# sThalham/PyraPose

Hardware: AMD Instinct MI355X
Metric: images/sec 640x480 fwd+bwd (train step: fwd + losses + bwd + clipnorm-Adam) (higher is better)
Workload: dtype bf16x3+f16c8

## Files before the change

### include/pyrapose_hip.h

```cpp
#ifndef PYRAPOSE_HIP_H
#define PYRAPOSE_HIP_H

#include <stddef.h>
#include <stdint.h>

#ifdef __cplusplus
extern "C" {
#endif

#define PP_OK 0
#define PP_ERR_ARG (-1)
#define PP_ERR_SHAPE (-2)
#define PP_ERR_ALIGN (-3)
#define PP_ERR_NOCTX (-4)
#define PP_ERR_UNSUPPORTED (-5)
#define PP_ERR_COMM (-6)

#define PP_MAX_SEG 5

typedef struct pp_ctx pp_ctx;

int pp_ctx_create(pp_ctx** out, int device, void* hip_stream);
void pp_ctx_destroy(pp_ctx* ctx);
int pp_ctx_set_stream(pp_ctx* ctx, void* hip_stream);
int pp_ctx_set_workspace(pp_ctx* ctx, void* device_buffer, size_t bytes);
int pp_row_block_list(pp_ctx* ctx, const float* x, int rows, int ld, int cols, unsigned char* flags, int* list);
int pp_row_block_list_planes(pp_ctx* ctx, const void* x_hi, const void* x_lo, int rows, int ld, int cols, unsigned char* flags, int* list);
int pp_row_block_list_planes_within(pp_ctx* ctx, const void* x_hi, const void* x_lo, int rows, int ld, int cols, const unsigned char* within,
                                    unsigned char* flags, int* list);
const char* pp_last_error_string(pp_ctx* ctx);
const char* pp_version(void);
int pp_device_info(pp_ctx* ctx, int* n_cu, char* name_host, int name_len);

typedef struct {
  int n_img;
  int n_seg;
  int h[PP_MAX_SEG];
  int w[PP_MAX_SEG];
} pp_rowspace;

typedef struct {
  pp_rowspace in;
  pp_rowspace out;
  int cin, cout;
  int kh, kw, stride;
  int pad_t, pad_l;
  int ld_x, ld_y, ld_w;
} pp_conv_desc;

int pp_conv2d_nhwc_fwd(pp_ctx* ctx, const pp_conv_desc* d, const float* x, const float* w,
                       const float* bias, const float* residual, int ld_res, int relu, float* y);

int pp_conv2d_nhwc_bwd_data(pp_ctx* ctx, const pp_conv_desc* d, const float* dy, const float* w,
                            const float* addend, int ld_add, const float* relu_src, int ld_rs, float* dx);

int pp_conv2d_nhwc_bwd_weight(pp_ctx* ctx, const pp_conv_desc* d, const float* x, const float* dy,
                              float* dw, float* dbias);

int pp_conv_split_weights_bf16x3(pp_ctx* ctx, const pp_conv_desc* d, const float* w, void* fwd_hi, void* fwd_lo,
                                 void* dgrad_hi, void* dgrad_lo);
typedef struct pp_split_job {
  const float* w;
  void* fwd_hi; void* fwd_lo; void* dg_hi; void* dg_lo;
  int taps, cin, cout, ld_w;
  int tile_begin, reserved;
} pp_split_job;
int pp_conv_split_weights_bf16x3_batch(pp_ctx* ctx, int n_jobs, const pp_split_job* jobs_dev, int total_tiles);
int pp_positive_row_blocks(pp_ctx* ctx, const pp_rowspace* rs, int A, int stride, const float* y_true, unsigned char* flags);
int pp_row_block_dilate(pp_ctx* ctx, const pp_conv_desc* d, const unsigned char* in_flags, unsigned char* out_flags);
int pp_split_planes_bf16x3(pp_ctx* ctx, size_t n, const float* src, void* hi, void* lo);
int pp_ctx_set_planes_format(pp_ctx* ctx, int fmt);
int pp_convert_planes(pp_ctx* ctx, size_t n, const void* src_hi, const void* src_lo, int src_fmt, void* dst_hi, void* dst_lo, int dst_fmt,
                      const float* scale2_dev, int scale_index, const void* relu_src_hi);
int pp_grad_scale_from_counts(pp_ctx* ctx, const int* counts_dev, int n_counts, float* scale2_dev);
int pp_grad_scale_from_counts_adj(pp_ctx* ctx, const int* counts_dev, int n_counts, float* scale2_dev, int log2_adjust);
int pp_split_planes_scaled_bf16x3(pp_ctx* ctx, size_t n, const float* src, void* hi, void* lo, const float* scale_dev);
int pp_ctx_set_grad_scale(pp_ctx* ctx, const float* scale2_dev);

typedef struct pp_conv_opts {
  void* capture_hi;
  void* capture_lo;
  const void* add_hi;
  const void* add_lo;
  const void* mask_hi;
  unsigned char* skip_flags;
  int* skip_list;
  const unsigned char* out_flags;
  int* out_list;
  int lazy_out;
  int lazy_in;
} pp_conv_opts;
#ifdef __cplusplus
static_assert(sizeof(pp_conv_opts) == 9 * sizeof(void*) + 2 * sizeof(int), "pp_conv_opts: pointers, then ints, no padding");
#else
_Static_assert(sizeof(pp_conv_opts) == 9 * sizeof(void*) + 2 * sizeof(int), "pp_conv_opts: pointers, then ints, no padding");
#endif

int pp_conv2d_nhwc_fwd_bf16x3(pp_ctx* ctx, const pp_conv_desc* d, const float* x, const void* x_hi, const void* x_lo,
                              const void* w_fwd_hi, const void* w_fwd_lo, const float* bias, const float* residual,
                              int ld_res, int relu, float* y, void* y_hi, void* y_lo, const pp_conv_opts* opts);
int pp_conv2d_nhwc_bwd_data_bf16x3(pp_ctx* ctx, const pp_conv_desc* d, const float* dy, const void* dy_hi,
                                   const void* dy_lo, const void* w_dgrad_hi, const void* w_dgrad_lo,
                                   const float* addend, int ld_add, const float* relu_src, int ld_rs, float* dx,
                                   void* dx_hi, void* dx_lo, const pp_conv_opts* opts);
int pp_conv2d_nhwc_bwd_data_s2_bf16x3(pp_ctx* ctx, const pp_conv_desc* d, const float* dy, const void* dy_hi,
                                      const void* dy_lo, const void* w_dgrad_hi, const void* w_dgrad_lo,
                                      const float* addend, int ld_add, const float* relu_src, int ld_rs, float* dx,
                                      void* dx_hi, void* dx_lo, const pp_conv_opts* opts);
int pp_conv_s2_merged(void);
int pp_conv2d_nhwc_bwd_weight_bf16x3(pp_ctx* ctx, const pp_conv_desc* d, const float* x, const float* dy,
                                     const void* x_hi, const void* x_lo, const void* dy_hi, const void* dy_lo,
                                     float* dw, float* dbias, const pp_conv_opts* opts);

#define PP_PLAN_FWD 0
#define PP_PLAN_BWD_DATA 1
#define PP_PLAN_BWD_WEIGHT 2
#define PP_PLAN_BWD_DATA_S2 3
#define PP_PLAN_PLANES_IN 1u
#define PP_PLAN_PLANES_OUT 2u
#define PP_PLAN_F32_OUT 4u
#define PP_PLAN_CAPTURE 8u
#define PP_PLAN_LIST 16u
#define PP_PLAN_LAZY_IN 32u
#define PP_PLAN_LAZY_OUT 64u
int pp_conv_plan_text(const pp_conv_desc* d, int pass, unsigned forms, int planes_fmt, int n_cu, size_t ws_bytes, char* buf,
                      int buf_bytes);

typedef struct pp_comm pp_comm;
int pp_comm_available(void);
int pp_comm_unique_id(pp_ctx* ctx, void* id128);
int pp_comm_init(pp_ctx* ctx, int world, int rank, const void* id128, pp_comm** out);
int pp_comm_destroy(pp_comm* comm);
int pp_allreduce_bucket(pp_ctx* ctx, pp_comm* comm, float* buf, size_t count);
int pp_allreduce_counts(pp_ctx* ctx, pp_comm* comm, int* counts, int n);

int pp_maxpool3x3s2_fwd(pp_ctx* ctx, int n_img, int h, int w, int c, const float* x, int oh, int ow, float* y);
int pp_upsample_nearest_add_fwd(pp_ctx* ctx, int n_img, int sh, int sw, int th, int tw, int c,
                                const float* src, const float* other, float* out);
int pp_upsample_nearest_add_bwd(pp_ctx* ctx, int n_img, int sh, int sw, int th, int tw, int c,
                                const float* dtarget, const float* base, float* dsrc);
int pp_add_n(pp_ctx* ctx, size_t n, const float* a, const float* b, const float* c, float* out);
int pp_relu_fwd(pp_ctx* ctx, size_t n, const float* x, float* y);
typedef struct pp_tview {
  const float* f32;
  const void* hi;
  const void* lo;
} pp_tview;
int pp_add_n_v(pp_ctx* ctx, size_t n, const pp_tview* a, const pp_tview* b, const pp_tview* c, const pp_tview* out);
int pp_relu_fwd_v(pp_ctx* ctx, size_t n, const pp_tview* x, const pp_tview* y);
int pp_upsample_nearest_add_fwd_v(pp_ctx* ctx, int n_img, int sh, int sw, int th, int tw, int c, const pp_tview* src,
                                  const pp_tview* other, const pp_tview* out);
int pp_upsample_nearest_add_bwd_v(pp_ctx* ctx, int n_img, int sh, int sw, int th, int tw, int c, const pp_tview* dtarget,
                                  const pp_tview* base, const pp_tview* dsrc);
int pp_merge_planes_bf16x3(pp_ctx* ctx, size_t n, const void* hi, const void* lo, float* dst);
int pp_planes_stats(pp_ctx* ctx, const void* hi, const void* lo, long long rows, int ld, int cols, const unsigned char* within,
                    unsigned long long* stats5_dev);
int pp_pack_rgb_to_4(pp_ctx* ctx, size_t n_pixels, const float* x3, float* x4);
int pp_preprocess_caffe_u8(pp_ctx* ctx, int n_img, int H, int W, const int* sizes_hw_host, const unsigned char* images_u8,
                           float* x4);
int pp_warp_affine_u8(pp_ctx* ctx, int n_img, int H, int W, int channels, const double* mats_host, int interpolation, int border,
                      int cval, const unsigned char* src, unsigned char* dst);
int pp_resize_scale(int rows, int cols, int min_side, int max_side, double* scale);
int pp_resize_linear_u8(pp_ctx* ctx, int n_img, int SH, int SW, int channels, double scale, int DH, int DW, const unsigned char* src,
                        unsigned char* dst);
enum { PP_PHOTO_NONE = 0, PP_PHOTO_LUT = 1, PP_PHOTO_GRAY = 2, PP_PHOTO_HUESAT = 3, PP_PHOTO_BLEND = 4, PP_PHOTO_CONV = 5, PP_PHOTO_MEDIAN = 6,
       PP_PHOTO_BILATERAL = 7 };
typedef struct pp_photo_op {
  int kind;
  int k;
  int off0, off1;
  float f0, f1;
} pp_photo_op;
size_t pp_photo_workspace_bytes(int n_img, int H, int W);
int pp_photo_augment_u8(pp_ctx* ctx, int n_img, int H, int W, int channels, const int* op_offsets_host, const pp_photo_op* ops_host,
                        const unsigned char* pool_host, size_t pool_bytes, const unsigned char* pool_dev, const unsigned char* src,
                        unsigned char* dst, void* workspace, size_t workspace_bytes);
int pp_pack_rgb_to_4_padded(pp_ctx* ctx, int n_img, int H, int W, int Hp, int Wp, int pad, const float* x3, float* x4p);
int pp_preprocess_caffe_u8_padded(pp_ctx* ctx, int n_img, int H, int W, int Hp, int Wp, int pad, const int* sizes_hw_host,
                                  const unsigned char* images_u8, float* x4p);
int pp_stem7x7s2_fwd_bf16x3(pp_ctx* ctx, int n_img, int H, int W, int Hp, int Wp, const float* x4p, const void* w_hi,
                            const void* w_lo, int cout, const float* bias, int relu, float* y, int ld_y);

int pp_export_head(pp_ctx* ctx, const pp_rowspace* rs, int n_anchor, int n_val, const float* src, int ld,
                   int apply_sigmoid, float* out);

int pp_count_positives(pp_ctx* ctx, size_t rows_box, const float* y_box, size_t rows_cls, int c_cls,
                       const float* y_cls, size_t rows_mask, int c_mask, const float* y_mask, int* counts);
int pp_sigmoid_focal_fwd_bwd(pp_ctx* ctx, const pp_rowspace* rs, int n_anchor, int n_class,
                             const float* logits, int ld, const float* y_true, float alpha, float gamma,
                             const int* count, float loss_weight, float* loss_sum, float* dlogits);
int pp_orth_smoothl1_fwd_bwd(pp_ctx* ctx, const pp_rowspace* rs, int n_anchor, const float* pred, int ld,
                             const float* y_true, float weight, float sigma, const int* count,
                             float loss_weight, float* loss_sum, float* dpred);

typedef struct {
  long long offset;
  long long count;
  int ld;
  int trainable;
  long long scale_off;
  float l2;
} pp_param_desc;

typedef struct pp_optimizer pp_optimizer;
int pp_optimizer_create(pp_ctx* ctx, pp_optimizer** out, const pp_param_desc* descs_host, int n_desc,
                        long long total);
void pp_optimizer_destroy(pp_optimizer* opt);
int pp_grad_global_norm(pp_ctx* ctx, pp_optimizer* opt, const float* w_master, const float* g_eff,
                        const float* scales, float* gnorm_sq, float* l2_loss);
int pp_adam_step_clipnorm(pp_ctx* ctx, pp_optimizer* opt, float* w_master, float* w_eff, const float* g_eff,
                          const float* scales, float* m, float* v, const float* gnorm_sq, float lr,
                          float beta1, float beta2, float eps, float clipnorm, long long step);

int pp_generate_base_anchors_host(int base_size, const float* ratios_host, int n_ratios,
                                  const float* scales_host, int n_scales, double* out_host);
int pp_anchors_shift_f64(pp_ctx* ctx, int n_levels, const int* feat_h_host, const int* feat_w_host,
                         const int* strides_host, int n_anchor, const double* base_anchors_host,
                         double* anchors_out);
int pp_anchors_shift_f32(pp_ctx* ctx, int n_levels, const int* feat_h_host, const int* feat_w_host,
                         const int* strides_host, int n_anchor, const double* base_anchors_host,
                         float* anchors_out);
int pp_compute_overlap_f64(pp_ctx* ctx, int n, const double* boxes, int k, const double* query, double* overlaps);
int pp_compute_gt_annotations(pp_ctx* ctx, int n, const double* anchors, int k, const double* gt_boxes,
                              double negative_overlap, double positive_overlap, int* argmax, signed char* state);

int pp_anchor_targets(pp_ctx* ctx, int n_anchor_total, const double* anchors, int batch,
                      const int* gt_offset_host, const double* gt_boxes, const int* gt_labels,
                      const double* gt_box3d, const int* gt_mask_ids, const unsigned char* id_masks,
                      int mask_h, int mask_w, const int* mask_hw_host, const int* image_hw_host, int num_classes,
                      double negative_overlap, double positive_overlap, int out_mh, int out_mw,
                      float* regression, float* labels, float* mask);
int pp_project_box3d_host(const double* pose7_host, const double* box8x3_host, const double* cam4_host,
                          double* out16_host);
int pp_pil_nearest_index_host(int n_in, int n_out, int* out_host);

int pp_box3d_decode(pp_ctx* ctx, int batch, int n, const float* anchors, const float* regression, float* boxes3d);
int pp_score_threshold_compact(pp_ctx* ctx, int batch, int n, int n_class, const float* scores, float thr,
                               int cap, int* idx_out, int* counts);
size_t pp_filter_workspace_bytes(int n, int n_class, int max_det);
int pp_filter_detections(pp_ctx* ctx, int n, int n_class, const float* boxes, const float* boxes3d,
                         const float* scores, float score_thr, float iou_thr, int max_det, void* workspace,
                         float* out_boxes, float* out_boxes3d, float* out_scores, int* out_labels);
int pp_filter_detections_batch(pp_ctx* ctx, int n_img, int n, int n_class, const float* boxes, const float* boxes3d,
                               const float* scores, float score_thr, float iou_thr, int max_det, void* workspace,
                               float* out_boxes, float* out_boxes3d, float* out_scores, int* out_labels);

size_t pp_pose_error_workspace_bytes(int n_pose, int n_pts);
int pp_pose_add_f64(pp_ctx* ctx, int n_pose, int n_pts, const double* pts, const double* R_est, const double* t_est,
                    const double* R_gt, const double* t_gt, void* workspace, double* out);
int pp_pose_adi_f64(pp_ctx* ctx, int n_pose, int n_pts, const double* pts, const double* R_est, const double* t_est,
                    const double* R_gt, const double* t_gt, void* workspace, double* out);

size_t pp_render_workspace_bytes(int n_pose, int n_vert, int n_tri, int width, int height);
int pp_render_depth_f32(pp_ctx* ctx, int n_pose, int n_vert, const double* verts, int n_tri, const int* faces, const double* R,
                        const double* t, const double* K4, int width, int height, double clip_near, double clip_far, void* workspace,
                        size_t workspace_bytes, float* depth);
size_t pp_render_rgbd_workspace_bytes(int n_pose, int n_vert, int n_tri, int width, int height);
int pp_render_rgbd(pp_ctx* ctx, int n_pose, int n_vert, const double* verts, const double* colors, const double* normals, int n_tri,
                   const int* faces, const double* R, const double* t, const double* K4, int width, int height, double clip_near,
                   double clip_far, int shading, double ambient_weight, const double* light_cam_pos, const double* bg_color,
                   void* workspace, size_t workspace_bytes, float* depth, int* tri_id, float* rgb_f32, unsigned char* rgb_u8);
size_t pp_render_rgbd_tex_workspace_bytes(int n_pose, int n_vert, int n_tri, int width, int height, int tex_w, int tex_h);
int pp_render_rgbd_tex(pp_ctx* ctx, int n_pose, int n_vert, const double* verts, const double* uv, const unsigned char* tex, int tex_w,
                       int tex_h, int filter, int wrap, const double* normals, int n_tri, const int* faces, const double* R,
                       const double* t, const double* K4, int width, int height, double clip_near, double clip_far, int shading,
                       double ambient_weight, const double* light_cam_pos, const double* bg_color, void* workspace,
                       size_t workspace_bytes, float* depth, int* tri_id, float* rgb_f32, unsigned char* rgb_u8);
size_t pp_vsd_workspace_bytes(int n, int width, int height);
int pp_vsd_f64(pp_ctx* ctx, int n, int width, int height, const float* depth_test, long long test_stride, const float* depth_est,
               const float* depth_gt, const double* K4, double delta, double tau, int cost_type, void* workspace, double* e,
               long long* inter, long long* uni);
size_t pp_vsd_multi_workspace_bytes(int n, int width, int height, int n_tau);
int pp_vsd_multi_f64(pp_ctx* ctx, int n, int width, int height, const float* depth_test, long long test_stride,
                     const float* depth_est, const float* depth_gt, const double* K4, double delta, int n_tau, const double* taus,
                     int cost_type, int visib_mode, void* workspace, double* e, long long* inter, long long* uni,
                     long long* visib_gt, long long* px_gt);
size_t pp_scene_gt_workspace_bytes(int n_inst, int canvas_w, int canvas_h);
// ... 163 lines not shown
```

### pyrapose_amd/_lib.py

```python
import ctypes as C
import os

_HERE = os.path.dirname(os.path.abspath(__file__))
LIB_PATH = os.path.join(_HERE, os.environ.get("PP_LIB") or "libpyrapose_hip.so")

PP_MAX_SEG = 5


class RowSpace(C.Structure):
    _fields_ = [("n_img", C.c_int), ("n_seg", C.c_int), ("h", C.c_int * PP_MAX_SEG), ("w", C.c_int * PP_MAX_SEG)]

    @classmethod
    def make(cls, n_img, shapes):
        rs = cls()
        rs.n_img = int(n_img)
        rs.n_seg = len(shapes)
        for i, (h, w) in enumerate(shapes):
            rs.h[i] = int(h)
            rs.w[i] = int(w)
        return rs

    def rows(self):
        return sum(self.n_img * self.h[i] * self.w[i] for i in range(self.n_seg))

    def shapes(self):
        return [(self.h[i], self.w[i]) for i in range(self.n_seg)]


class ConvDesc(C.Structure):
    _fields_ = [("in_", RowSpace), ("out", RowSpace), ("cin", C.c_int), ("cout", C.c_int), ("kh", C.c_int),
                ("kw", C.c_int), ("stride", C.c_int), ("pad_t", C.c_int), ("pad_l", C.c_int), ("ld_x", C.c_int),
                ("ld_y", C.c_int), ("ld_w", C.c_int)]


class ParamDesc(C.Structure):
    _fields_ = [("offset", C.c_longlong), ("count", C.c_longlong), ("ld", C.c_int), ("trainable", C.c_int),
                ("scale_off", C.c_longlong), ("l2", C.c_float)]


class SplitJob(C.Structure):
    _fields_ = [("w", C.c_void_p), ("fwd_hi", C.c_void_p), ("fwd_lo", C.c_void_p), ("dg_hi", C.c_void_p), ("dg_lo", C.c_void_p),
                ("taps", C.c_int), ("cin", C.c_int), ("cout", C.c_int), ("ld_w", C.c_int), ("tile_begin", C.c_int), ("reserved", C.c_int)]


class TView(C.Structure):
    _fields_ = [("f32", C.c_void_p), ("hi", C.c_void_p), ("lo", C.c_void_p)]


class ConvOpts(C.Structure):
    _fields_ = [("capture_hi", C.c_void_p), ("capture_lo", C.c_void_p), ("add_hi", C.c_void_p), ("add_lo", C.c_void_p),
                ("mask_hi", C.c_void_p), ("skip_flags", C.c_void_p), ("skip_list", C.c_void_p), ("out_flags", C.c_void_p),
                ("out_list", C.c_void_p), ("lazy_out", C.c_int), ("lazy_in", C.c_int)]


def _load():
    if not os.path.exists(LIB_PATH):
        raise ImportError(
            "pyrapose_amd: %s not found. Build it with `python -c 'import __graft_entry__ as g; g.build()'` "
            "or `make -C pyrapose_amd/csrc`. There is no CPU fallback." % LIB_PATH)
    try:
        return C.CDLL(LIB_PATH)
    except OSError as e:
        raise ImportError("pyrapose_amd: cannot load %s: %s" % (LIB_PATH, e))


lib = _load()
if hasattr(lib, "pp_ctx_set_split_capture"):
    raise ImportError("pyrapose_amd: %s predates pp_conv_opts (it still exports pp_ctx_set_split_capture): rebuild it" % LIB_PATH)

_p = C.c_void_p
_i = C.c_int
_f = C.c_float
_d = C.c_double
_ll = C.c_longlong
_sz = C.c_size_t

_SIGS = {
    "pp_ctx_create": (_i, [C.POINTER(_p), _i, _p]),
    "pp_ctx_destroy": (None, [_p]),
    "pp_ctx_set_stream": (_i, [_p, _p]),
    "pp_last_error_string": (C.c_char_p, [_p]),
    "pp_version": (C.c_char_p, []),
    "pp_device_info": (_i, [_p, C.POINTER(_i), C.c_char_p, _i]),
    "pp_conv2d_nhwc_fwd": (_i, [_p, C.POINTER(ConvDesc), _p, _p, _p, _p, _i, _i, _p]),
    "pp_conv2d_nhwc_bwd_data": (_i, [_p, C.POINTER(ConvDesc), _p, _p, _p, _i, _p, _i, _p]),
    "pp_conv2d_nhwc_bwd_weight": (_i, [_p, C.POINTER(ConvDesc), _p, _p, _p, _p]),
    "pp_conv_split_weights_bf16x3": (_i, [_p, C.POINTER(ConvDesc), _p, _p, _p, _p, _p]),
    "pp_split_planes_bf16x3": (_i, [_p, _sz, _p, _p, _p]),
    "pp_ctx_set_planes_format": (_i, [_p, _i]),
    "pp_convert_planes": (_i, [_p, _sz, _p, _p, _i, _p, _p, _i, _p, _i, _p]),
    "pp_split_planes_scaled_bf16x3": (_i, [_p, _sz, _p, _p, _p, _p]),
    "pp_grad_scale_from_counts": (_i, [_p, _p, _i, _p]),
    "pp_grad_scale_from_counts_adj": (_i, [_p, _p, _i, _p, _i]),
    "pp_ctx_set_grad_scale": (_i, [_p, _p]),
    "pp_planes_stats": (_i, [_p, _p, _p, _ll, _i, _i, _p, _p]),
    "pp_comm_available": (_i, []),
    "pp_comm_unique_id": (_i, [_p, _p]),
    "pp_comm_init": (_i, [_p, _i, _i, _p, C.POINTER(_p)]),
    "pp_comm_destroy": (_i, [_p]),
    "pp_allreduce_bucket": (_i, [_p, _p, _p, C.c_size_t]),
    "pp_allreduce_counts": (_i, [_p, _p, _p, _i]),
    "pp_ctx_set_workspace": (_i, [_p, _p, C.c_size_t]),
    "pp_row_block_list": (_i, [_p, _p, _i, _i, _i, _p, _p]),
    "pp_positive_row_blocks": (_i, [_p, _p, _i, _i, _p, _p]),
    "pp_row_block_dilate": (_i, [_p, _p, _p, _p]),
    "pp_row_block_list_planes": (_i, [_p, _p, _p, _i, _i, _i, _p, _p]),
    "pp_row_block_list_planes_within": (_i, [_p, _p, _p, _i, _i, _i, _p, _p, _p]),
    "pp_add_n_v": (_i, [_p, _sz, C.POINTER(TView), C.POINTER(TView), C.POINTER(TView), C.POINTER(TView)]),
    "pp_relu_fwd_v": (_i, [_p, _sz, C.POINTER(TView), C.POINTER(TView)]),
    "pp_upsample_nearest_add_fwd_v": (_i, [_p, _i, _i, _i, _i, _i, _i, C.POINTER(TView), C.POINTER(TView), C.POINTER(TView)]),
    "pp_upsample_nearest_add_bwd_v": (_i, [_p, _i, _i, _i, _i, _i, _i, C.POINTER(TView), C.POINTER(TView), C.POINTER(TView)]),
    "pp_merge_planes_bf16x3": (_i, [_p, _sz, _p, _p, _p]),
    "pp_warp_affine_u8": (_i, [_p, _i, _i, _i, _i, C.POINTER(_d), _i, _i, _i, _p, _p]),
    "pp_photo_workspace_bytes": (_sz, [_i, _i, _i]),
    "pp_photo_augment_u8": (_i, [_p, _i, _i, _i, _i, _p, _p, _p, _sz, _p, _p, _p, _p, _sz]),
    "pp_resize_scale": (_i, [_i, _i, _i, _i, C.POINTER(_d)]),
    "pp_resize_linear_u8": (_i, [_p, _i, _i, _i, _i, _d, _i, _i, _p, _p]),
    "pp_conv_split_weights_bf16x3_batch": (_i, [_p, _i, _p, _i]),
    "pp_conv2d_nhwc_fwd_bf16x3": (_i, [_p, C.POINTER(ConvDesc), _p, _p, _p, _p, _p, _p, _p, _i, _i, _p, _p, _p, C.POINTER(ConvOpts)]),
    "pp_conv2d_nhwc_bwd_data_bf16x3": (_i, [_p, C.POINTER(ConvDesc), _p, _p, _p, _p, _p, _p, _i, _p, _i, _p, _p, _p, C.POINTER(ConvOpts)]),
    "pp_conv2d_nhwc_bwd_data_s2_bf16x3": (_i, [_p, C.POINTER(ConvDesc), _p, _p, _p, _p, _p, _p, _i, _p, _i, _p, _p, _p, C.POINTER(ConvOpts)]),
    "pp_conv_s2_merged": (_i, []),
    "pp_conv2d_nhwc_bwd_weight_bf16x3": (_i, [_p, C.POINTER(ConvDesc), _p, _p, _p, _p, _p, _p, _p, _p, C.POINTER(ConvOpts)]),
    "pp_conv_plan_text": (_i, [C.POINTER(ConvDesc), _i, C.c_uint, _i, _i, _sz, C.c_char_p, _i]),
    "pp_maxpool3x3s2_fwd": (_i, [_p, _i, _i, _i, _i, _p, _i, _i, _p]),
    "pp_upsample_nearest_add_fwd": (_i, [_p, _i, _i, _i, _i, _i, _i, _p, _p, _p]),
    "pp_upsample_nearest_add_bwd": (_i, [_p, _i, _i, _i, _i, _i, _i, _p, _p, _p]),
    "pp_add_n": (_i, [_p, _sz, _p, _p, _p, _p]),
    "pp_relu_fwd": (_i, [_p, C.c_size_t, _p, _p]),
    "pp_preprocess_caffe_u8": (_i, [_p, _i, _i, _i, C.POINTER(C.c_int), _p, _p]),
    "pp_preprocess_caffe_u8_padded": (_i, [_p, _i, _i, _i, _i, _i, _i, C.POINTER(C.c_int), _p, _p]),
    "pp_pack_rgb_to_4_padded": (_i, [_p, _i, _i, _i, _i, _i, _i, _p, _p]),
    "pp_stem7x7s2_fwd_bf16x3": (_i, [_p, _i, _i, _i, _i, _i, _p, _p, _p, _i, _p, _i, _p, _i]),
    "pp_pack_rgb_to_4": (_i, [_p, _sz, _p, _p]),
    "pp_export_head": (_i, [_p, C.POINTER(RowSpace), _i, _i, _p, _i, _i, _p]),
    "pp_count_positives": (_i, [_p, _sz, _p, _sz, _i, _p, _sz, _i, _p, _p]),
    "pp_sigmoid_focal_fwd_bwd": (_i, [_p, C.POINTER(RowSpace), _i, _i, _p, _i, _p, _f, _f, _p, _f, _p, _p]),
    "pp_orth_smoothl1_fwd_bwd": (_i, [_p, C.POINTER(RowSpace), _i, _p, _i, _p, _f, _f, _p, _f, _p, _p]),
    "pp_optimizer_create": (_i, [_p, C.POINTER(_p), C.POINTER(ParamDesc), _i, _ll]),
    "pp_optimizer_destroy": (None, [_p]),
    "pp_grad_global_norm": (_i, [_p, _p, _p, _p, _p, _p, _p]),
    "pp_adam_step_clipnorm": (_i, [_p, _p, _p, _p, _p, _p, _p, _p, _p, _f, _f, _f, _f, _f, _ll]),
    "pp_generate_base_anchors_host": (_i, [_i, C.POINTER(_f), _i, C.POINTER(_f), _i, C.POINTER(_d)]),
    "pp_anchors_shift_f64": (_i, [_p, _i, C.POINTER(_i), C.POINTER(_i), C.POINTER(_i), _i, C.POINTER(_d), _p]),
    "pp_anchors_shift_f32": (_i, [_p, _i, C.POINTER(_i), C.POINTER(_i), C.POINTER(_i), _i, C.POINTER(_d), _p]),
    "pp_compute_overlap_f64": (_i, [_p, _i, _p, _i, _p, _p]),
    "pp_compute_gt_annotations": (_i, [_p, _i, _p, _i, _p, _d, _d, _p, _p]),
    "pp_anchor_targets": (_i, [_p, _i, _p, _i, C.POINTER(_i), _p, _p, _p, _p, _p, _i, _i, C.POINTER(_i), C.POINTER(_i), _i, _d, _d,
                               _i, _i, _p, _p, _p]),
    "pp_project_box3d_host": (_i, [C.POINTER(_d), C.POINTER(_d), C.POINTER(_d), C.POINTER(_d)]),
    "pp_pil_nearest_index_host": (_i, [_i, _i, C.POINTER(_i)]),
    "pp_box3d_decode": (_i, [_p, _i, _i, _p, _p, _p]),
    "pp_score_threshold_compact": (_i, [_p, _i, _i, _i, _p, _f, _i, _p, _p]),
    "pp_filter_workspace_bytes": (_sz, [_i, _i, _i]),
    "pp_pose_error_workspace_bytes": (_sz, [_i, _i]),
    "pp_filter_detections": (_i, [_p, _i, _i, _p, _p, _p, _f, _f, _i, _p, _p, _p, _p, _p]),
    "pp_pose_add_f64": (_i, [_p, _i, _i, _p, _p, _p, _p, _p, _p, _p]),
    "pp_pose_adi_f64": (_i, [_p, _i, _i, _p, _p, _p, _p, _p, _p, _p]),
    "pp_filter_detections_batch": (_i, [_p, _i, _i, _i, _p, _p, _p, _f, _f, _i, _p, _p, _p, _p, _p]),
    "pp_render_workspace_bytes": (_sz, [_i, _i, _i, _i, _i]),
    "pp_render_depth_f32": (_i, [_p, _i, _i, _p, _i, _p, _p, _p, _p, _i, _i, _d, _d, _p, _sz, _p]),
    "pp_render_rgbd_workspace_bytes": (_sz, [_i, _i, _i, _i, _i]),
    "pp_render_rgbd": (_i, [_p, _i, _i, _p, _p, _p, _i, _p, _p, _p, _p, _i, _i, _d, _d, _i, _d, C.POINTER(_d), C.POINTER(_d), _p, _sz,
                            _p, _p, _p, _p]),
    "pp_render_rgbd_tex_workspace_bytes": (_sz, [_i, _i, _i, _i, _i, _i, _i]),
    "pp_render_rgbd_tex": (_i, [_p, _i, _i, _p, _p, _p, _i, _i, _i, _i, _p, _i, _p, _p, _p, _p, _i, _i, _d, _d, _i, _d, C.POINTER(_d),
                                C.POINTER(_d), _p, _sz, _p, _p, _p, _p]),
    "pp_scene_compose_u8": (_i, [_p, _i, _i, C.POINTER(_i), _p, _i, _i, _p, _p, _p, C.POINTER(C.c_ubyte), _i, _p]),
    "pp_vsd_workspace_bytes": (_sz, [_i, _i, _i]),
    "pp_vsd_f64": (_i, [_p, _i, _i, _i, _p, _ll, _p, _p, _p, _d, _d, _i, _p, _p, _p, _p]),
    "pp_vsd_multi_workspace_bytes": (_sz, [_i, _i, _i, _i]),
    "pp_vsd_multi_f64": (_i, [_p, _i, _i, _i, _p, _ll, _p, _p, _p, _d, _i, C.POINTER(_d), _i, _i, _p, _p, _p, _p, _p, _p]),
    "pp_scene_gt_workspace_bytes": (_sz, [_i, _i, _i]),
    "pp_scene_gt_info": (_i, [_p, _i, _i, C.POINTER(_i), _p, _i, _i, _i, _i, _i, _i, _p, _p, _p, _ll, _d, _p, _sz, _p, _p, _p, _p, _p,
                              _p, _p]),
    "pp_pose_reproj_f64": (_i, [_p, _i, _i, _p, _p, _p, _p, _p, _p, _p, _p]),
    "pp_pose_sym_workspace_bytes": (_sz, [_i, _i, _i]),
    "pp_pose_mssd_f64": (_i, [_p, _i, _i, _i, _p, _p, _p, _p, _p, _p, _p, _p, _p, _p]),
    "pp_pose_mspd_f64": (_i, [_p, _i, _i, _i, _p, _p, _p, _p, _p, _p, _p, _p, _p, _p, _p]),
    "pp_pnp_ransac_workspace_bytes": (_sz, [_i, _i]),
    "pp_pnp_ransac_f64": (_i, [_p, _i, _p, _i, _p, _p, _p, _i, _d, C.c_ulonglong, _i, _p, _p, _p, _p, _p, _p]),
    "pp_cloud_from_depth_workspace_bytes": (_sz, [_i, _i]),
    "pp_cloud_from_depth_f64": (_i, [_p, _i, _i, _p, _p, _i, _i, _p, _p, _d, _d, _d, _d, _d, _i, _p, _p, _p]),
    "pp_voxel_workspace_bytes": (_sz, [_i]),
    "pp_voxel_keys_f64": (_i, [_p, _i, _p, _d, _p, _p]),
    "pp_voxel_means_f64": (_i, [_p, _i, _p, _p, _p, _i, _p, _p, _p]),
    "pp_estimate_normals_workspace_bytes": (_sz, [_i, _i]),
    "pp_estimate_normals_f64": (_i, [_p, _i, _p, _d, _i, _p, _p, _p]),
    "pp_icp_workspace_bytes": (_sz, [_i, _i]),
    "pp_icp_f64": (_i, [_p, _i, _p, _p, _i, _p, _p, _p, _p, _d, _i, _d, _d, _i, _p, _sz, _p, _p, _p, _p, _p, _p, _p]),
    "pp_vote_stats_workspace_bytes": (_sz, [_i, _i]),
    "pp_vote_stats_f64": (_i, [_p, _i, _p, _i, _p, _i, _p, _p, _i, _d, _p, _p, _p, _p, _p, _p, _p]),
    "pp_pnp_refine_weighted_workspace_bytes": (_sz, [_i, _i]),
    "pp_pnp_refine_weighted_f64": (_i, [_p, _i, _p, _i, _p, _p, _p, _p, _p, _p, _i, _d, _d, _d, _p, _p, _p, _p, _p, _p, _p, _p, _p]),
    "pp_vote_cluster_workspace_bytes": (_sz, [_i, _i, _i, _i]),
    "pp_vote_cluster": (_i, [_p, _i, _i, _i, _i, _p, _p, _p, _p, _d, _i, _i, _i, _p, _p, _p, _p, _p, _p, _p]),
    "pp_pts_diameter_workspace_bytes": (_sz, [_i]),
    "pp_pts_diameter_f64": (_i, [_p, _i, _p, _p, _sz, _p, _p]),
    "pp_farthest_points_workspace_bytes": (_sz, [_i]),
    "pp_farthest_points_f64": (_i, [_p, _i, _i, _p, C.POINTER(_i), _p, _i, _i, _p, _p, _p, _sz, _p]),
    "pp_sym_hausdorff_workspace_bytes": (_sz, [_i, _i]),
    "pp_sym_hausdorff_f64": (_i, [_p, _i, _p, _i, _p, _i, _p, _p, _p, _sz, _p, _p]),
    "pp_det_match": (_i, [_p, _i, _i, _i, _i, _p, _p, _p, _p, _p, _p, C.POINTER(_i), _p, _i, C.POINTER(_d), _i, _p, _p, _p]),
    "pp_det_pr_curve": (_i, [_p, _i, _i, _i, _ll, _p, _p, _p, _p, _p, _p, _p, _p, _p]),
    "pp_det_ap": (_i, [_p, _i, _i, _i, _p, _p, _p, _p, _i, _p, _p]),
    "pp_mask_confusion": (_i, [_p, _i, _i, _i, _p, _p, _i, C.POINTER(_d), _p]),
    "pp_mask_pack": (_i, [_p, _i, _i, _i, _p, _p, _p, _p]),
    "pp_mask_iou_pairs": (_i, [_p, _i, _i, _i, _i, _i, _p, _p, _p, _p, _p, _p, _p, C.POINTER(_i), _p, _p, _p]),
    "pp_det_match_iou": (_i, [_p, _i, _i, _i, _i, _p, _p, _p, _p, _p, C.POINTER(_i), _p, _i, C.POINTER(_d), _i, _p, _p, _p]),
    "pp_mask_rle_workspace_bytes": (_sz, [_i]),
    "pp_mask_rle": (_i, [_p, _i, _i, _i, _i, _p, _p, _sz, _ll, _p, C.POINTER(_i), _p]),
    "pp_mask_from_rle": (_i, [_p, _i, _i, _i, _i, C.POINTER(_i), C.POINTER(_i), _p, _p, _p]),
    "pp_depth_normals_workspace_bytes": (_sz, [_i, _i, _i]),
    "pp_depth_normals_f64": (_i, [_p, _i, _i, _i, _p, _p, C.POINTER(_d), _i, _p, _sz, _p, _p, _p, _p]),
    "pp_depth_augment_workspace_bytes": (_sz, [_i, _i, _i]),
    "pp_depth_augment": (_i, [_p, _i, _i, _i, _p, _p, _p, C.POINTER(_d), _p, _p, _sz, _p, _p, _p, _p, _p]),
    "pp_depth_inpaint_workspace_bytes": (_sz, [_i, _i, _i]),
    "pp_depth_inpaint": (_i, [_p, _i, _i, _i, _p, _p, _i, _i, _i, _p, _sz, _p, _p, _p, _p]),
    "pp_draw_overlay_u8": (_i, [_p, _i, _i, _i, _p, _p, _p, _p, _i, _p, _p, _i, _i]),
}

EXPORTS = sorted(_SIGS)

MISSING = []
for _name, (_res, _args) in _SIGS.items():
    try:
        _fn = getattr(lib, _name)
    except AttributeError:
        if not os.environ.get("PP_LIB"):
            raise
        MISSING.append(_name)
        continue
    _fn.restype = _res
    _fn.argtypes = _args


def check(rc, ctx=None, what=""):
    if rc == 0:
        return
    msg = ""
    if ctx is not None:
        s = lib.pp_last_error_string(ctx)
        msg = s.decode("utf-8", "replace") if s else ""
    if rc < 0:
        raise ValueError("%s failed (%d): %s" % (what or "pyrapose_hip", rc, msg))
    raise RuntimeError("%s failed (hipError %d): %s" % (what or "pyrapose_hip", rc, msg))
```

### pyrapose_amd/csrc/conv3.h

```cpp
#pragma once
#include "conv_common.h"

struct Igemm3Args {
  const void *ahi, *alo, *whi, *wlo;
  int w_rows, w_ld8;
  void *ohi, *olo;
  void *chi, *clo;
  const unsigned char* flags;
  float* ws;
};

void PP_API(pp3_launch_igemm)(hipStream_t st, IgemmParams& p, const Igemm3Args& a, const PpIgemmPlan& pl);
void PP_API(pp3_launch_igemm_s2)(hipStream_t st, IgemmParams& p, const Igemm3Args& a, const DgradS2Route& r);
void PP_API(pp3_launch_igemm_rowlist)(hipStream_t st, IgemmParams& p, const Igemm3Args& a, const PpIgemmPlan& pl, const unsigned char* dy_flags,
                                      unsigned char* out_flags, int* out_list, bool fill);
void PP_API(pp3_launch_class_fill)(hipStream_t st, const IgemmParams& p, unsigned blocks, const float* addend, const float* mask, float* out, void* ohi,
                                   void* olo);
void PP_API(pp3_launch_rl_dilate)(hipStream_t st, const IgemmParams& p, const unsigned char* in_flags, unsigned char* out_flags, int n_blocks);

void PP_API(pp3_launch_igemm4x)(hipStream_t st, const IgemmParams& p, const Igemm3Args& a, const PpIgemmPlan& pl);

void PP_API(pp3_launch_wgrad)(hipStream_t st, const Wgrad3Params& p, const PpWgradPlan& pl, const float* x, const float* dy, const void* xhi,
                              const void* xlo, const void* dhi, const void* dlo, float* dw, float* dbias, const int* list, float* ctx_ws);

void PP_API(pp3_split_capture_pass)(hipStream_t st, const IgemmParams& p, void* chi, void* clo);
void PP_API(pp3_launch_row_block_compact)(hipStream_t st, const unsigned char* flags, int n_blocks, int* list);
```

### pyrapose_amd/csrc/conv3.hip

```cpp
#include "conv3_unit.h"
#include "conv3.h"
#include "conv4.h"

namespace {

static PpIgemmFacts igemm3_facts(const pp_ctx* ctx, const IgemmParams& p, const Igemm3Args& a) {
  return igemm_facts(p, a.w_rows, a.w_ld8, a.ahi != nullptr, p.src != nullptr, a.ohi != nullptr, p.out != nullptr, a.chi != nullptr,
                     a.flags != nullptr, ctx->n_cu, ctx->ws != nullptr, (long long)ctx->ws_bytes);
}

static void dispatch3(pp_ctx* ctx, IgemmParams& p, const Igemm3Args& a) {
  const PpIgemmFacts f = igemm3_facts(ctx, p, a);
  const PpIgemmPlan pl = pp_plan_igemm(f);
  pp_plan_debug(f, pl);
  PP_API(pp3_launch_igemm)(ctx->stream, p, a, pl);
}

static void dispatch3m(pp_ctx* ctx, IgemmParams& p, const Igemm3Args& a, const DgradS2Route& r) {
  pp_plan_debug(r.f, r.pl, r.g);
  PP_API(pp3_launch_igemm_s2)(ctx->stream, p, a, r);
}

static void dispatch3_rowlist(pp_ctx* ctx, IgemmParams& p, const Igemm3Args& a, int tm, const unsigned char* dy_flags, unsigned char* out_flags,
                              int* out_list, bool fill) {
  PpIgemmFacts f = igemm3_facts(ctx, p, a);
  f.listed = true;
  f.listed_tm = tm;
  const PpIgemmPlan pl = pp_plan_igemm(f);
  PP_API(pp3_launch_igemm_rowlist)(ctx->stream, p, a, pl, dy_flags, out_flags, out_list, fill);
}

static int bwd_data_impl(pp_ctx* ctx, const char* who, bool merged, const pp_conv_desc* d, const float* dy, const void* dy_hi, const void* dy_lo,
                         const void* w_hi, const void* w_lo, const float* addend, int ld_add, const float* relu_src, int ld_rs, float* dx,
                         void* dx_hi, void* dx_lo, const pp_conv_opts* opts) {
  PP_REQUIRE_CTX(ctx);
  int rc = pp_conv_opts_take(ctx, opts,
                             merged ? (PP_OPT_ADD | PP_OPT_MASK)
                                    : (PP_OPT_CAPTURE | PP_OPT_ADD | PP_OPT_MASK | PP_OPT_SKIP | PP_OPT_LAZY_OUT | PP_OPT_LAZY_IN),
                             who);
  if (rc) return rc;
  void *const chi = opts->capture_hi, *const clo = opts->capture_lo;
  unsigned char* const skip_flags = opts->skip_flags;
  const bool skip_scratch_ok = skip_flags != nullptr && opts->skip_list != nullptr;
  const void *const ep_ah = opts->add_hi, *const ep_al = opts->add_lo, *const ep_mh = opts->mask_hi;
  rc = check_desc(ctx, d, who);
  PP_CHECK_ARG(ctx, !(ep_ah && addend) && !(ep_mh && relu_src), PP_ERR_ARG,
               "%s: addend / relu_src given both as f32 and as planes", who);
  PP_CHECK_ARG(ctx, (!ep_ah || (ld_add >= d->cin && ld_add % 4 == 0)) && (!ep_mh || (ld_rs >= d->cin && ld_rs % 4 == 0)), PP_ERR_SHAPE,
               "%s: addend / relu_src planes", who);
  if (rc) return rc;
  PP_CHECK_ARG(ctx, !chi || (dy && !dy_hi && pp_is_packed(chi, clo)), PP_ERR_ARG, "%s: split capture needs the f32 operand", who);
  PP_CHECK_ARG(ctx, (dy || (dy_hi && dy_lo)) && w_hi && w_lo && (dx || (dx_hi && dx_lo)), PP_ERR_ARG, "%s: null tensor", who);
  PP_CHECK_ARG(ctx, (dy_hi == nullptr) == (dy_lo == nullptr) && d->ld_y % 8 == 0, PP_ERR_ARG, "%s: planes / ld_y", who);
  PP_CHECK_ARG(ctx, pp_is_packed(dy_hi, dy_lo) && pp_is_packed(dx_hi, dx_lo), PP_ERR_ALIGN,
               "%s: planes must be packed (lo = hi + 16 bytes, 16-byte aligned)", who);
  PP_CHECK_ARG(ctx, (!dx_hi || (d->cin % 8 == 0 && d->ld_x % 8 == 0)) && (!ep_ah || ld_add % 8 == 0) && (!ep_mh || ld_rs % 8 == 0), PP_ERR_SHAPE,
               "%s: planes need channel counts and leading dimensions %% 8 == 0", who);
  const int cred = (d->cout + 31) / 32 * 32;
  PP_CHECK_ARG(ctx, d->cin % 16 == 0 && d->ld_y >= cred && d->ld_y % 4 == 0, PP_ERR_SHAPE,
               "%s: dy needs ld_y >= %d (cout rounded up to 32, zero padded)", who, cred);
  PP_CHECK_ARG(ctx, (!dy || pp_is_aligned16(dy)) && pp_is_aligned16(w_hi) && pp_is_aligned16(w_lo) && (!dx || pp_is_aligned16(dx)), PP_ERR_ALIGN,
               "%s: tensors must be 16-byte aligned", who);
  PP_CHECK_ARG(ctx, (!addend || (ld_add >= d->cin && ld_add % 4 == 0 && pp_is_aligned16(addend))) &&
                        (!relu_src || (ld_rs >= d->cin && ld_rs % 4 == 0 && pp_is_aligned16(relu_src))),
               PP_ERR_SHAPE, "%s: addend / relu_src", who);
  IgemmParams p;
  memset(&p, 0, sizeof(p));
  p.src = dy; p.out = dx; p.bias = nullptr; p.addend = addend; p.mask_src = relu_src;
  p.add_hi = ep_ah; p.add_lo = ep_al; p.mask_hi = ep_mh;
  igemm_geometry_bwd_data(ctx, d, p);
  p.ld_add = ld_add; p.ld_mask = ld_rs;
  p.relu = 0;
  PP_CHECK_ARG(ctx, (dx_hi == nullptr) == (dx_lo == nullptr) && (!dx_hi || (d->ld_x % 4 == 0 && pp_is_aligned16(dx_hi) && pp_is_aligned16(dx_lo))),
               PP_ERR_ARG, "%s: output planes", who);
  const Igemm3Args a = {dy_hi, dy_lo, w_hi, w_lo, d->cin, cred / 8, dx_hi, dx_lo, chi, clo, skip_flags, ctx->ws};
  if (merged) {
    DgradS2Route s2;
    dgrad_s2_route(d, p, igemm3_facts(ctx, p, a), &s2);
    PP_CHECK_ARG(ctx, s2.ok, PP_ERR_ARG,
                 "%s: needs stride 2, one level, operands all float32 or all planes, and classes the branch-free loop can run "
                 "(pp_conv2d_nhwc_bwd_data_bf16x3 takes every other call)", who);
    IgemmParams q = s2.cls[0];
    dispatch3m(ctx, q, a, s2);
    PP_CHECK_LAUNCH(ctx, who);
    return PP_OK;
  }
  DgradRoute route;
  dgrad_route(d, p, igemm3_facts(ctx, p, a), skip_scratch_ok, &route);
  PP_CHECK_ARG(ctx, !opts->lazy_in || route.listed, PP_ERR_ARG,
               "%s: dy was declared lazy (unwritten outside its flagged blocks) but the listed-block launch "
               "does not apply to this call", who);
  const int nb = (p.M + 31) / 32;
  if (skip_scratch_ok && !route.listed) PP_HIP(ctx, hipMemsetAsync(skip_flags + nb, 1, (size_t)nb, ctx->stream));
  const Igemm3Args ac = {dy_hi, dy_lo, w_hi, w_lo, d->cin, cred / 8, dx_hi, dx_lo, nullptr, nullptr, nullptr, ctx->ws};
  if (route.classes && chi) PP_API(pp3_split_capture_pass)(ctx->stream, p, chi, clo);
  dgrad_launches(
      route, p,
      [&](IgemmParams& q, bool is_class, bool listed) {
        if (listed) dispatch3_rowlist(ctx, q, a, route.listed_tm, skip_flags, skip_flags + nb, opts->skip_list + nb + 1, !opts->lazy_out);
        else dispatch3(ctx, q, is_class ? ac : a);
      },
      [&](IgemmParams& q) {
        PP_API(pp3_launch_class_fill)(ctx->stream, q, pp_finish_blocks(q.M, q.Nout, pp_cus(ctx->n_cu)), addend, relu_src, dx, dx_hi, dx_lo);
      });
  PP_CHECK_LAUNCH(ctx, who);
  return PP_OK;
}

}

extern "C" {

int PP_API(pp_conv2d_nhwc_fwd_bf16x3)(pp_ctx* ctx, const pp_conv_desc* d, const float* x, const void* x_hi, const void* x_lo,
                                         const void* w_hi, const void* w_lo, const float* bias, const float* residual, int ld_res,
                                         int relu, float* y, void* y_hi, void* y_lo, const pp_conv_opts* opts) {
  PP_REQUIRE_CTX(ctx);
  int rc = pp_conv_opts_take(ctx, opts, PP_OPT_CAPTURE | PP_OPT_ADD | PP_OPT_OUT, "pp_conv2d_nhwc_fwd_bf16x3");
  if (rc) return rc;
  void *const chi = opts->capture_hi, *const clo = opts->capture_lo;
  const void *const ep_ah = opts->add_hi, *const ep_al = opts->add_lo;
  rc = check_desc(ctx, d, "pp_conv2d_nhwc_fwd_bf16x3");
  PP_CHECK_ARG(ctx, !(ep_ah && residual), PP_ERR_ARG, "pp_conv2d_nhwc_fwd_bf16x3: residual given both as f32 and as planes");
  PP_CHECK_ARG(ctx, !ep_ah || (ld_res % 4 == 0 && ld_res >= ((d->cout + 3) & ~3)), PP_ERR_SHAPE, "pp_conv2d_nhwc_fwd_bf16x3: residual planes");
  if (rc) return rc;
  PP_CHECK_ARG(ctx, !chi || (x && !x_hi && pp_is_packed(chi, clo)), PP_ERR_ARG, "pp_conv2d_nhwc_fwd_bf16x3: split capture needs the f32 operand");
  PP_CHECK_ARG(ctx, (x || (x_hi && x_lo)) && w_hi && w_lo && (y || (y_hi && y_lo)), PP_ERR_ARG, "pp_conv2d_nhwc_fwd_bf16x3: null tensor");
  PP_CHECK_ARG(ctx, (x_hi == nullptr) == (x_lo == nullptr), PP_ERR_ARG, "pp_conv2d_nhwc_fwd_bf16x3: x_hi and x_lo go together");
  PP_CHECK_ARG(ctx, d->cin % 32 == 0 && d->ld_x % 8 == 0, PP_ERR_SHAPE, "pp_conv2d_nhwc_fwd_bf16x3: cin %d must be a multiple of 32, ld_x of 8", d->cin);
  PP_CHECK_ARG(ctx, pp_is_packed(x_hi, x_lo) && pp_is_packed(y_hi, y_lo), PP_ERR_ALIGN,
               "pp_conv2d_nhwc_fwd_bf16x3: planes must be packed (lo = hi + 16 bytes, 16-byte aligned)");
  PP_CHECK_ARG(ctx, !y_hi || (d->cout % 8 == 0 && d->ld_y % 8 == 0), PP_ERR_SHAPE, "pp_conv2d_nhwc_fwd_bf16x3: output planes need cout, ld_y %% 8 == 0");
  PP_CHECK_ARG(ctx, !ep_ah || (ld_res % 8 == 0 && d->cout % 8 == 0), PP_ERR_SHAPE, "pp_conv2d_nhwc_fwd_bf16x3: residual planes need cout, ld_res %% 8 == 0");
  PP_CHECK_ARG(ctx, (!x || pp_is_aligned16(x)) && pp_is_aligned16(w_hi) && pp_is_aligned16(w_lo) && (!y || pp_is_aligned16(y)), PP_ERR_ALIGN,
               "pp_conv2d_nhwc_fwd_bf16x3: tensors must be 16-byte aligned");
  PP_CHECK_ARG(ctx, !residual || (ld_res % 4 == 0 && ld_res >= ((d->cout + 3) & ~3) && pp_is_aligned16(residual)), PP_ERR_SHAPE,
               "pp_conv2d_nhwc_fwd_bf16x3: residual");
  PP_CHECK_ARG(ctx, !bias || pp_is_aligned16(bias), PP_ERR_ALIGN, "pp_conv2d_nhwc_fwd_bf16x3: bias alignment");
  IgemmParams p;
  memset(&p, 0, sizeof(p));
  p.src = x; p.out = y; p.bias = bias; p.addend = residual; p.mask_src = nullptr;
  p.add_hi = ep_ah; p.add_lo = ep_al;
  igemm_geometry_fwd(ctx, d, p);
  p.ld_add = ld_res; p.ld_mask = 0;
  p.relu = relu;
  PP_CHECK_ARG(ctx, (y_hi == nullptr) == (y_lo == nullptr) && (!y_hi || (d->ld_y % 4 == 0 && pp_is_aligned16(y_hi) && pp_is_aligned16(y_lo))),
               PP_ERR_ARG, "pp_conv2d_nhwc_fwd_bf16x3: output planes");
  const Igemm3Args a = {x_hi, x_lo, w_hi, w_lo, d->cout, d->cin / 8, y_hi, y_lo, chi, clo, nullptr, ctx->ws};
  if (opts->out_flags) {
    const bool ok = fwd_listed_ok(d, igemm3_facts(ctx, p, a), residual != nullptr || ep_ah != nullptr);
    PP_CHECK_ARG(ctx, ok, PP_ERR_SHAPE, "pp_conv2d_nhwc_fwd_bf16x3: out_flags needs a 3x3 stride-1 'same' conv on plane-stored input");
    dispatch3_rowlist(ctx, p, a, 2, nullptr, const_cast<unsigned char*>(opts->out_flags) ,
                      opts->out_list, false);
    PP_CHECK_LAUNCH(ctx, "pp_conv2d_nhwc_fwd_bf16x3");
    return PP_OK;
  }
  dispatch3(ctx, p, a);
  PP_CHECK_LAUNCH(ctx, "pp_conv2d_nhwc_fwd_bf16x3");
  return PP_OK;
}

int PP_API(pp_row_block_dilate)(pp_ctx* ctx, const pp_conv_desc* d, const unsigned char* in_flags, unsigned char* out_flags) {
  PP_REQUIRE_CTX(ctx);
  int rc = check_desc(ctx, d, "pp_row_block_dilate");
  if (rc) return rc;
  PP_CHECK_ARG(ctx, in_flags && out_flags && in_flags != out_flags, PP_ERR_ARG, "pp_row_block_dilate: two distinct flag buffers");
  IgemmParams p;
  memset(&p, 0, sizeof(p));
  p.n_seg = d->in.n_seg;
  fill_segs(ctx, d, true, p.seg, &p.M, &p.src_rows);
  const bool same = d->stride == 1 && d->kh == 3 && d->kw == 3 && segs_same_grid(p.seg, p.n_seg);
  PP_CHECK_ARG(ctx, same, PP_ERR_SHAPE, "pp_row_block_dilate: 3x3 stride-1 conv on an unchanged grid");
  const int nb = (p.M + 31) / 32;
  PP_API(pp3_launch_rl_dilate)(ctx->stream, p, in_flags, out_flags, nb);
  PP_CHECK_LAUNCH(ctx, "pp_row_block_dilate");
  return PP_OK;
}

int PP_API(pp_stem7x7s2_fwd_bf16x3)(pp_ctx* ctx, int n_img, int H, int W, int Hp, int Wp, const float* x4p, const void* w_hi,
                                       const void* w_lo, int cout, const float* bias, int relu, float* y, int ld_y) {
  PP_REQUIRE_CTX(ctx);
  PP_CHECK_ARG(ctx, x4p && w_hi && w_lo && y && pp_is_aligned16(x4p) && pp_is_aligned16(y) && pp_is_aligned16(w_hi) && pp_is_aligned16(w_lo),
               PP_ERR_ARG, "pp_stem7x7s2_fwd_bf16x3: null / unaligned tensor");
  PP_CHECK_ARG(ctx, n_img > 0 && H > 0 && W > 0 && Hp >= H + 6 && Wp >= W + 8 && Wp % 2 == 0 && cout > 0 && ld_y % 4 == 0 && ld_y >= ((cout + 3) & ~3),
               PP_ERR_SHAPE, "pp_stem7x7s2_fwd_bf16x3: bad geometry");
  const int OH = (H + 6 - 7) / 2 + 1, OW = (W + 6 - 7) / 2 + 1;
  IgemmParams p;
  memset(&p, 0, sizeof(p));
  p.src = x4p; p.out = y; p.bias = bias;
  p.ld_src = 4; p.ld_out = ld_y;
  p.relu = relu;
  p.n_seg = 1;
  p.seg[0].row_begin = 0; p.seg[0].src_row_begin = 0;
  p.seg[0].OH = OH; p.seg[0].OW = OW; p.seg[0].SH = Hp; p.seg[0].SW = Wp;
  p.M = n_img * OH * OW;
  p.src_rows = (long long)n_img * Hp * Wp;
  p.Cred = 32; p.Nout = cout; p.w_tap_rows = 32;
  p.kh = 7; p.kw = 1;
  p.mul = 2; p.tsign = 1; p.off_y = 0; p.off_x = 0; p.div = 1;
  p.w_ty0 = 0; p.w_tx0 = 0; p.w_tstep = 1; p.w_kw = 1; p.w_taps = 7;
  const Igemm3Args a = {nullptr, nullptr, w_hi, w_lo, cout, 4, nullptr, nullptr, nullptr, nullptr, nullptr, ctx->ws};
  PP_CHECK_ARG(ctx, pp_igemm_fast_ok(igemm3_facts(ctx, p, a)), PP_ERR_SHAPE, "pp_stem7x7s2_fwd_bf16x3: frame too large for 31-bit offsets");
  dispatch3(ctx, p, a);
  PP_CHECK_LAUNCH(ctx, "pp_stem7x7s2_fwd_bf16x3");
  return PP_OK;
}

int PP_API(pp_conv2d_nhwc_bwd_data_bf16x3)(pp_ctx* ctx, const pp_conv_desc* d, const float* dy, const void* dy_hi, const void* dy_lo,
                                              const void* w_hi, const void* w_lo, const float* addend, int ld_add,
                                              const float* relu_src, int ld_rs, float* dx, void* dx_hi, void* dx_lo,
                                              const pp_conv_opts* opts) {
  return bwd_data_impl(ctx, "pp_conv2d_nhwc_bwd_data_bf16x3", false, d, dy, dy_hi, dy_lo, w_hi, w_lo, addend, ld_add, relu_src, ld_rs, dx, dx_hi,
                       dx_lo, opts);
}
int PP_API(pp_conv2d_nhwc_bwd_data_s2_bf16x3)(pp_ctx* ctx, const pp_conv_desc* d, const float* dy, const void* dy_hi, const void* dy_lo,
                                                 const void* w_hi, const void* w_lo, const float* addend, int ld_add,
                                                 const float* relu_src, int ld_rs, float* dx, void* dx_hi, void* dx_lo,
                                                 const pp_conv_opts* opts) {
  return bwd_data_impl(ctx, "pp_conv2d_nhwc_bwd_data_s2_bf16x3", true, d, dy, dy_hi, dy_lo, w_hi, w_lo, addend, ld_add, relu_src, ld_rs, dx,
                       dx_hi, dx_lo, opts);
}

int PP_API(pp_conv2d_nhwc_bwd_weight_bf16x3)(pp_ctx* ctx, const pp_conv_desc* d, const float* x, const float* dy, const void* x_hi,
                                                const void* x_lo, const void* dy_hi, const void* dy_lo, float* dw, float* dbias,
                                                const pp_conv_opts* opts) {
  PP_REQUIRE_CTX(ctx);
  int rc = pp_conv_opts_take(ctx, opts, PP_OPT_SKIP | PP_OPT_LAZY_IN, "pp_conv2d_nhwc_bwd_weight_bf16x3");
  if (rc) return rc;
  const int* const skip_list = opts->skip_list;
  const bool lazy_in = opts->lazy_in != 0;
  rc = check_desc(ctx, d, "pp_conv2d_nhwc_bwd_weight_bf16x3");
  if (rc) return rc;
  const bool planes = x_hi && x_lo && dy_hi && dy_lo;
  PP_CHECK_ARG(ctx, ((x && dy) || planes) && dw, PP_ERR_ARG, "pp_conv2d_nhwc_bwd_weight_bf16x3: null tensor");
  PP_CHECK_ARG(ctx, planes || !(x_hi || x_lo || dy_hi || dy_lo), PP_ERR_ARG, "pp_conv2d_nhwc_bwd_weight_bf16x3: all four planes or none");
  PP_CHECK_ARG(ctx, !planes || (d->ld_x % 8 == 0 && d->ld_y % 8 == 0), PP_ERR_SHAPE, "pp_conv2d_nhwc_bwd_weight_bf16x3: planes need ld % 8 == 0");
  PP_CHECK_ARG(ctx, !planes || (pp_is_packed(x_hi, x_lo) && pp_is_packed(dy_hi, dy_lo)), PP_ERR_ALIGN,
               "pp_conv2d_nhwc_bwd_weight_bf16x3: planes must be packed (lo = hi + 16 bytes, 16-byte aligned)");
  PP_CHECK_ARG(ctx, d->cin % 64 == 0, PP_ERR_SHAPE, "pp_conv2d_nhwc_bwd_weight_bf16x3: cin %d must be a multiple of 64", d->cin);
  PP_CHECK_ARG(ctx, d->ld_y % 4 == 0 && d->ld_x % 4 == 0, PP_ERR_SHAPE, "pp_conv2d_nhwc_bwd_weight_bf16x3: leading dims must be multiples of 4");
  PP_CHECK_ARG(ctx, (!x || pp_is_aligned16(x)) && (!dy || pp_is_aligned16(dy)), PP_ERR_ALIGN,
               "pp_conv2d_nhwc_bwd_weight_bf16x3: tensors must be 16-byte aligned");
  Wgrad3Params p;
  memset(&p, 0, sizeof(p));
  wgrad_geometry(ctx, d, p);
  p.inv_scale = (planes && ctx->grad_scale) ? ctx->grad_scale + 1 : nullptr;
  const PpWgradFacts f = wgrad_facts(p, planes, skip_list != nullptr, lazy_in, PP_FMT, ctx->n_cu, ctx->ws != nullptr, (long long)ctx->ws_bytes,
                                     pp_is_aligned16(dw), pp_is_aligned16(dbias));
  const PpWgradPlan pl = pp_plan_wgrad(f);
  PP_CHECK_ARG(ctx, !pl.refused, PP_ERR_ARG,
               "pp_conv2d_nhwc_bwd_weight_bf16x3: dy was declared lazy (unwritten outside its listed blocks) but the listed-block reduction "
               "does not apply to this call");
  pp_plan_debug(f, pl);
  p.k_tiles_per_tap = pl.k_tiles_per_tap; p.n_tiles_k = pl.n_tiles_k; p.n_tiles_n = pl.n_tiles_n;
  p.splits = pl.splits; p.rows_per_split = pl.rows_per_split; p.max_wraps = pl.max_wraps; p.sp_min_steps = pl.sp_min_steps;
  const void* const xhi = planes ? x_hi : nullptr;
  if (pl.family == PP_WGRAD3R || pl.family == PP_WGRAD3W)
    PP_API(pp4_launch_wgrad3r)(ctx->stream, p, pl.grid, pl.family == PP_WGRAD3W, x_hi, x_lo, dy_hi, dy_lo, dw, dbias, skip_list);
  else
    PP_API(pp3_launch_wgrad)(ctx->stream, p, pl, x, dy, xhi, x_lo, dy_hi, dy_lo, dw, dbias, skip_list, ctx->ws);
  PP_CHECK_LAUNCH(ctx, "pp_conv2d_nhwc_bwd_weight_bf16x3");
  return PP_OK;
}

}
```

### pyrapose_amd/csrc/conv3_dispatch.hip

```cpp
#include "conv_common.h"

extern "C" int pp_row_block_list_fmt0(pp_ctx* ctx, const float* x, int rows, int ld, int cols, unsigned char* flags, int* list);
extern "C" int pp_row_block_list_fmt1(pp_ctx* ctx, const float* x, int rows, int ld, int cols, unsigned char* flags, int* list);
extern "C" int pp_row_block_list_planes_within_fmt0(pp_ctx* ctx, const void* x_hi, const void* x_lo, int rows, int ld, int cols, const unsigned char* within, unsigned char* flags, int* list);
extern "C" int pp_row_block_list_planes_within_fmt1(pp_ctx* ctx, const void* x_hi, const void* x_lo, int rows, int ld, int cols, const unsigned char* within, unsigned char* flags, int* list);
extern "C" int pp_row_block_list_planes_fmt0(pp_ctx* ctx, const void* x_hi, const void* x_lo, int rows, int ld, int cols, unsigned char* flags, int* list);
extern "C" int pp_row_block_list_planes_fmt1(pp_ctx* ctx, const void* x_hi, const void* x_lo, int rows, int ld, int cols, unsigned char* flags, int* list);
extern "C" int pp_split_planes_bf16x3_fmt0(pp_ctx* ctx, size_t n, const float* src, void* hi, void* lo);
extern "C" int pp_split_planes_bf16x3_fmt1(pp_ctx* ctx, size_t n, const float* src, void* hi, void* lo);
extern "C" int pp_split_planes_scaled_bf16x3_fmt0(pp_ctx* ctx, size_t n, const float* src, void* hi, void* lo, const float* scale_dev);
extern "C" int pp_split_planes_scaled_bf16x3_fmt1(pp_ctx* ctx, size_t n, const float* src, void* hi, void* lo, const float* scale_dev);
extern "C" int pp_grad_scale_from_counts_fmt0(pp_ctx* ctx, const int* counts_dev, int n_counts, float* scale2_dev);
extern "C" int pp_grad_scale_from_counts_adj_fmt0(pp_ctx* ctx, const int* counts_dev, int n_counts, float* scale2_dev, int log2_adjust);
extern "C" int pp_grad_scale_from_counts_adj_fmt1(pp_ctx* ctx, const int* counts_dev, int n_counts, float* scale2_dev, int log2_adjust);
extern "C" int pp_grad_scale_from_counts_fmt1(pp_ctx* ctx, const int* counts_dev, int n_counts, float* scale2_dev);
extern "C" int pp_conv_split_weights_bf16x3_batch_fmt0(pp_ctx* ctx, int n_jobs, const pp_split_job* jobs_dev, int total_tiles);
extern "C" int pp_conv_split_weights_bf16x3_batch_fmt1(pp_ctx* ctx, int n_jobs, const pp_split_job* jobs_dev, int total_tiles);
extern "C" int pp_conv_split_weights_bf16x3_fmt0(pp_ctx* ctx, const pp_conv_desc* d, const float* w, void* fwd_hi, void* fwd_lo, void* dgrad_hi, void* dgrad_lo);
extern "C" int pp_conv_split_weights_bf16x3_fmt1(pp_ctx* ctx, const pp_conv_desc* d, const float* w, void* fwd_hi, void* fwd_lo, void* dgrad_hi, void* dgrad_lo);
extern "C" int pp_conv2d_nhwc_fwd_bf16x3_fmt0(pp_ctx* ctx, const pp_conv_desc* d, const float* x, const void* x_hi, const void* x_lo, const void* w_fwd_hi, const void* w_fwd_lo, const float* bias, const float* residual, int ld_res, int relu, float* y, void* y_hi, void* y_lo, const pp_conv_opts* opts);
extern "C" int pp_conv2d_nhwc_fwd_bf16x3_fmt1(pp_ctx* ctx, const pp_conv_desc* d, const float* x, const void* x_hi, const void* x_lo, const void* w_fwd_hi, const void* w_fwd_lo, const float* bias, const float* residual, int ld_res, int relu, float* y, void* y_hi, void* y_lo, const pp_conv_opts* opts);
extern "C" int pp_row_block_dilate_fmt0(pp_ctx* ctx, const pp_conv_desc* d, const unsigned char* in_flags, unsigned char* out_flags);
extern "C" int pp_row_block_dilate_fmt1(pp_ctx* ctx, const pp_conv_desc* d, const unsigned char* in_flags, unsigned char* out_flags);
extern "C" int pp_stem7x7s2_fwd_bf16x3_fmt0(pp_ctx* ctx, int n_img, int H, int W, int Hp, int Wp, const float* x4p, const void* w_hi, const void* w_lo, int cout, const float* bias, int relu, float* y, int ld_y);
extern "C" int pp_stem7x7s2_fwd_bf16x3_fmt1(pp_ctx* ctx, int n_img, int H, int W, int Hp, int Wp, const float* x4p, const void* w_hi, const void* w_lo, int cout, const float* bias, int relu, float* y, int ld_y);
extern "C" int pp_conv2d_nhwc_bwd_data_bf16x3_fmt0(pp_ctx* ctx, const pp_conv_desc* d, const float* dy, const void* dy_hi, const void* dy_lo, const void* w_dgrad_hi, const void* w_dgrad_lo, const float* addend, int ld_add, const float* relu_src, int ld_rs, float* dx, void* dx_hi, void* dx_lo, const pp_conv_opts* opts);
extern "C" int pp_conv2d_nhwc_bwd_data_s2_bf16x3_fmt0(pp_ctx* ctx, const pp_conv_desc* d, const float* dy, const void* dy_hi, const void* dy_lo, const void* w_dgrad_hi, const void* w_dgrad_lo, const float* addend, int ld_add, const float* relu_src, int ld_rs, float* dx, void* dx_hi, void* dx_lo, const pp_conv_opts* opts);
extern "C" int pp_conv2d_nhwc_bwd_data_bf16x3_fmt1(pp_ctx* ctx, const pp_conv_desc* d, const float* dy, const void* dy_hi, const void* dy_lo, const void* w_dgrad_hi, const void* w_dgrad_lo, const float* addend, int ld_add, const float* relu_src, int ld_rs, float* dx, void* dx_hi, void* dx_lo, const pp_conv_opts* opts);
extern "C" int pp_conv2d_nhwc_bwd_data_s2_bf16x3_fmt1(pp_ctx* ctx, const pp_conv_desc* d, const float* dy, const void* dy_hi, const void* dy_lo, const void* w_dgrad_hi, const void* w_dgrad_lo, const float* addend, int ld_add, const float* relu_src, int ld_rs, float* dx, void* dx_hi, void* dx_lo, const pp_conv_opts* opts);
extern "C" int pp_conv2d_nhwc_bwd_weight_bf16x3_fmt0(pp_ctx* ctx, const pp_conv_desc* d, const float* x, const float* dy, const void* x_hi, const void* x_lo, const void* dy_hi, const void* dy_lo, float* dw, float* dbias, const pp_conv_opts* opts);
extern "C" int pp_conv2d_nhwc_bwd_weight_bf16x3_fmt1(pp_ctx* ctx, const pp_conv_desc* d, const float* x, const float* dy, const void* x_hi, const void* x_lo, const void* dy_hi, const void* dy_lo, float* dw, float* dbias, const pp_conv_opts* opts);

extern "C" int pp_row_block_list(pp_ctx* ctx, const float* x, int rows, int ld, int cols, unsigned char* flags, int* list) {
  return (ctx && ctx->planes_fmt == 1) ? pp_row_block_list_fmt1(ctx, x, rows, ld, cols, flags, list) : pp_row_block_list_fmt0(ctx, x, rows, ld, cols, flags, list);
}
extern "C" int pp_row_block_list_planes_within(pp_ctx* ctx, const void* x_hi, const void* x_lo, int rows, int ld, int cols, const unsigned char* within, unsigned char* flags, int* list) {
  return (ctx && ctx->planes_fmt == 1) ? pp_row_block_list_planes_within_fmt1(ctx, x_hi, x_lo, rows, ld, cols, within, flags, list) : pp_row_block_list_planes_within_fmt0(ctx, x_hi, x_lo, rows, ld, cols, within, flags, list);
}
extern "C" int pp_row_block_list_planes(pp_ctx* ctx, const void* x_hi, const void* x_lo, int rows, int ld, int cols, unsigned char* flags, int* list) {
  return (ctx && ctx->planes_fmt == 1) ? pp_row_block_list_planes_fmt1(ctx, x_hi, x_lo, rows, ld, cols, flags, list) : pp_row_block_list_planes_fmt0(ctx, x_hi, x_lo, rows, ld, cols, flags, list);
}
extern "C" int pp_split_planes_bf16x3(pp_ctx* ctx, size_t n, const float* src, void* hi, void* lo) {
  return (ctx && ctx->planes_fmt == 1) ? pp_split_planes_bf16x3_fmt1(ctx, n, src, hi, lo) : pp_split_planes_bf16x3_fmt0(ctx, n, src, hi, lo);
}
extern "C" int pp_split_planes_scaled_bf16x3(pp_ctx* ctx, size_t n, const float* src, void* hi, void* lo, const float* scale_dev) {
  return (ctx && ctx->planes_fmt == 1) ? pp_split_planes_scaled_bf16x3_fmt1(ctx, n, src, hi, lo, scale_dev) : pp_split_planes_scaled_bf16x3_fmt0(ctx, n, src, hi, lo, scale_dev);
}
extern "C" int pp_grad_scale_from_counts(pp_ctx* ctx, const int* counts_dev, int n_counts, float* scale2_dev) {
  return (ctx && ctx->planes_fmt == 1) ? pp_grad_scale_from_counts_fmt1(ctx, counts_dev, n_counts, scale2_dev) : pp_grad_scale_from_counts_fmt0(ctx, counts_dev, n_counts, scale2_dev);
}
extern "C" int pp_grad_scale_from_counts_adj(pp_ctx* ctx, const int* counts_dev, int n_counts, float* scale2_dev, int log2_adjust) {
  return (ctx && ctx->planes_fmt == 1) ? pp_grad_scale_from_counts_adj_fmt1(ctx, counts_dev, n_counts, scale2_dev, log2_adjust) : pp_grad_scale_from_counts_adj_fmt0(ctx, counts_dev, n_counts, scale2_dev, log2_adjust);
}
extern "C" int pp_conv_split_weights_bf16x3_batch(pp_ctx* ctx, int n_jobs, const pp_split_job* jobs_dev, int total_tiles) {
  return (ctx && ctx->planes_fmt == 1) ? pp_conv_split_weights_bf16x3_batch_fmt1(ctx, n_jobs, jobs_dev, total_tiles) : pp_conv_split_weights_bf16x3_batch_fmt0(ctx, n_jobs, jobs_dev, total_tiles);
}
extern "C" int pp_conv_split_weights_bf16x3(pp_ctx* ctx, const pp_conv_desc* d, const float* w, void* fwd_hi, void* fwd_lo, void* dgrad_hi, void* dgrad_lo) {
  return (ctx && ctx->planes_fmt == 1) ? pp_conv_split_weights_bf16x3_fmt1(ctx, d, w, fwd_hi, fwd_lo, dgrad_hi, dgrad_lo) : pp_conv_split_weights_bf16x3_fmt0(ctx, d, w, fwd_hi, fwd_lo, dgrad_hi, dgrad_lo);
}
extern "C" int pp_conv2d_nhwc_fwd_bf16x3(pp_ctx* ctx, const pp_conv_desc* d, const float* x, const void* x_hi, const void* x_lo, const void* w_fwd_hi, const void* w_fwd_lo, const float* bias, const float* residual, int ld_res, int relu, float* y, void* y_hi, void* y_lo, const pp_conv_opts* opts) {
  return (ctx && ctx->planes_fmt == 1) ? pp_conv2d_nhwc_fwd_bf16x3_fmt1(ctx, d, x, x_hi, x_lo, w_fwd_hi, w_fwd_lo, bias, residual, ld_res, relu, y, y_hi, y_lo, opts) : pp_conv2d_nhwc_fwd_bf16x3_fmt0(ctx, d, x, x_hi, x_lo, w_fwd_hi, w_fwd_lo, bias, residual, ld_res, relu, y, y_hi, y_lo, opts);
}
extern "C" int pp_row_block_dilate(pp_ctx* ctx, const pp_conv_desc* d, const unsigned char* in_flags, unsigned char* out_flags) {
  return (ctx && ctx->planes_fmt == 1) ? pp_row_block_dilate_fmt1(ctx, d, in_flags, out_flags) : pp_row_block_dilate_fmt0(ctx, d, in_flags, out_flags);
}
extern "C" int pp_stem7x7s2_fwd_bf16x3(pp_ctx* ctx, int n_img, int H, int W, int Hp, int Wp, const float* x4p, const void* w_hi, const void* w_lo, int cout, const float* bias, int relu, float* y, int ld_y) {
  return (ctx && ctx->planes_fmt == 1) ? pp_stem7x7s2_fwd_bf16x3_fmt1(ctx, n_img, H, W, Hp, Wp, x4p, w_hi, w_lo, cout, bias, relu, y, ld_y) : pp_stem7x7s2_fwd_bf16x3_fmt0(ctx, n_img, H, W, Hp, Wp, x4p, w_hi, w_lo, cout, bias, relu, y, ld_y);
}
extern "C" int pp_conv2d_nhwc_bwd_data_bf16x3(pp_ctx* ctx, const pp_conv_desc* d, const float* dy, const void* dy_hi, const void* dy_lo, const void* w_dgrad_hi, const void* w_dgrad_lo, const float* addend, int ld_add, const float* relu_src, int ld_rs, float* dx, void* dx_hi, void* dx_lo, const pp_conv_opts* opts) {
  return (ctx && ctx->planes_fmt == 1) ? pp_conv2d_nhwc_bwd_data_bf16x3_fmt1(ctx, d, dy, dy_hi, dy_lo, w_dgrad_hi, w_dgrad_lo, addend, ld_add, relu_src, ld_rs, dx, dx_hi, dx_lo, opts) : pp_conv2d_nhwc_bwd_data_bf16x3_fmt0(ctx, d, dy, dy_hi, dy_lo, w_dgrad_hi, w_dgrad_lo, addend, ld_add, relu_src, ld_rs, dx, dx_hi, dx_lo, opts);
}
extern "C" int pp_conv2d_nhwc_bwd_data_s2_bf16x3(pp_ctx* ctx, const pp_conv_desc* d, const float* dy, const void* dy_hi, const void* dy_lo, const void* w_dgrad_hi, const void* w_dgrad_lo, const float* addend, int ld_add, const float* relu_src, int ld_rs, float* dx, void* dx_hi, void* dx_lo, const pp_conv_opts* opts) {
  return (ctx && ctx->planes_fmt == 1) ? pp_conv2d_nhwc_bwd_data_s2_bf16x3_fmt1(ctx, d, dy, dy_hi, dy_lo, w_dgrad_hi, w_dgrad_lo, addend, ld_add, relu_src, ld_rs, dx, dx_hi, dx_lo, opts) : pp_conv2d_nhwc_bwd_data_s2_bf16x3_fmt0(ctx, d, dy, dy_hi, dy_lo, w_dgrad_hi, w_dgrad_lo, addend, ld_add, relu_src, ld_rs, dx, dx_hi, dx_lo, opts);
}
extern "C" int pp_conv2d_nhwc_bwd_weight_bf16x3(pp_ctx* ctx, const pp_conv_desc* d, const float* x, const float* dy, const void* x_hi, const void* x_lo, const void* dy_hi, const void* dy_lo, float* dw, float* dbias, const pp_conv_opts* opts) {
  return (ctx && ctx->planes_fmt == 1) ? pp_conv2d_nhwc_bwd_weight_bf16x3_fmt1(ctx, d, x, dy, x_hi, x_lo, dy_hi, dy_lo, dw, dbias, opts) : pp_conv2d_nhwc_bwd_weight_bf16x3_fmt0(ctx, d, x, dy, x_hi, x_lo, dy_hi, dy_lo, dw, dbias, opts);
}

extern "C" int pp_conv_s2_merged(void) { return pp_sw_s2_merged() ? 1 : 0; }

extern "C" int pp_conv_plan_text(const pp_conv_desc* d, int pass, unsigned forms, int planes_fmt, int n_cu, size_t ws_bytes, char* buf,
                                 int buf_bytes) {
  if (!buf || buf_bytes <= 0 || pass < PP_PLAN_FWD || pass > PP_PLAN_BWD_DATA_S2) return PP_ERR_ARG;
  const int rc = check_desc(nullptr, d, "pp_conv_plan_text");
  if (rc) return rc;
  const bool planes_in = forms & PP_PLAN_PLANES_IN, planes_out = forms & PP_PLAN_PLANES_OUT, f32_out = (forms & PP_PLAN_F32_OUT) || !planes_out,
             capture = forms & PP_PLAN_CAPTURE, list = forms & PP_PLAN_LIST, lazy_in = forms & PP_PLAN_LAZY_IN;
  const bool ws = ws_bytes > 0;
  int at = 0;
  buf[0] = 0;
  if (pass == PP_PLAN_BWD_WEIGHT) {
    if (d->cin % 64 != 0) return PP_ERR_SHAPE;
    Wgrad3Params p;
    memset(&p, 0, sizeof(p));
    wgrad_geometry(nullptr, d, p);
    const PpWgradFacts f = wgrad_facts(p, planes_in, list, lazy_in, planes_fmt, n_cu, ws, (long long)ws_bytes, true, true);
    return pp_plan_print(buf, buf_bytes, at, f, pp_plan_wgrad(f), true);
  }
  IgemmParams p;
  memset(&p, 0, sizeof(p));
  if (pass == PP_PLAN_FWD) {
    if (d->cin % 32 != 0) return PP_ERR_SHAPE;
    igemm_geometry_fwd(nullptr, d, p);
    PpIgemmFacts f = igemm_facts(p, d->cout, d->cin / 8, planes_in, !planes_in, planes_out, f32_out, capture, false, n_cu, ws, (long long)ws_bytes);
    if (list) {
      if (!fwd_listed_ok(d, f, false)) return PP_ERR_SHAPE;
      f.listed = true;
      f.listed_tm = 2;
    }
    return pp_plan_print(buf, buf_bytes, at, f, pp_plan_igemm(f), true);
  }
  if (d->cin % 16 != 0) return PP_ERR_SHAPE;
  igemm_geometry_bwd_data(nullptr, d, p);
  const int w_rows = d->cin, w_ld8 = p.Cred / 8;
  const PpIgemmFacts f = igemm_facts(p, w_rows, w_ld8, planes_in, !planes_in, planes_out, f32_out, capture, list, n_cu, ws, (long long)ws_bytes);
  if (pass == PP_PLAN_BWD_DATA_S2) {
    DgradS2Route s2;
    s2.ok = false;
    if (!(forms & (PP_PLAN_LIST | PP_PLAN_LAZY_IN | PP_PLAN_LAZY_OUT))) dgrad_s2_route(d, p, f, &s2);
    if (!s2.ok) return pp_plan_append(buf, buf_bytes, at, "igemm3 s2 refused: not a stride-2, one-level, all-f32 or all-planes data gradient\n");
    return pp_plan_print(buf, buf_bytes, at, s2.f, s2.pl, s2.g, true);
  }
  DgradRoute route;
  dgrad_route(d, p, f, list, &route);
  if (lazy_in && !route.listed) return pp_plan_append(buf, buf_bytes, at, "igemm3 refused: lazy dy without a listed-block launch\n");
  dgrad_launches(
      route, p,
      [&](IgemmParams& q, bool is_class, bool listed) {
        PpIgemmFacts fq = igemm_facts(q, w_rows, w_ld8, planes_in, !planes_in, planes_out, f32_out, capture && !is_class, list && !is_class, n_cu, ws,
                                      (long long)ws_bytes);
        fq.listed = listed;
        fq.listed_tm = route.listed_tm;
        at = pp_plan_print(buf, buf_bytes, at, fq, pp_plan_igemm(fq), true);
      },
      [&](IgemmParams& q) {
        at = pp_plan_append(buf, buf_bytes, at, "class M %d N %d: no taps class_fill | grid=%u\n", q.M, q.Nout,
                            pp_finish_blocks(q.M, q.Nout, pp_cus(n_cu)));
      });
  return at;
}
```

### pyrapose_amd/csrc/conv3_igemm.hip

```cpp
#include "conv3_unit.h"
#include "conv3.h"
#include "conv4.h"

#ifndef PP_EPI_GF
#define PP_EPI_GF 4
#endif

namespace {

template <int TM, int TN, bool AP, bool OP>
__global__ __launch_bounds__(256, (TM * TN >= 8) ? 2 : ((TM * TN == 4) ? 3 : 4)) void igemm3_kernel(
    const IgemmParams p, const float* __restrict__ g_src, const uint4* __restrict__ g_ahi, const uint4* __restrict__ g_alo,
    const uint4* __restrict__ g_whi, const uint4* __restrict__ g_wlo,
    const float* __restrict__ g_bias, const float* __restrict__ g_addend, const float* __restrict__ g_mask,
    float* __restrict__ g_out, uint2* __restrict__ g_ohi, uint2* __restrict__ g_olo, int w_rows, int w_ld8) {
  constexpr int BM = 64 * TM, BN = 64 * TN, BK = 32, NO = BK / 8;
  constexpr int SMEM_U4 = 2 * NO * (BM + BN);
  __shared__ __attribute__((aligned(16))) uint4 smem[SMEM_U4];
  uint4* Ahi = smem;
  uint4* Alo = Ahi + NO * BM;
  uint4* Bhi = Alo + NO * BM;
  uint4* Blo = Bhi + NO * BN;

  const int tid = threadIdx.x, lane = tid & 63, wave = tid >> 6;
  const int wm = wave >> 1, wn = wave & 1;
  const int lb = xcd_remap((int)blockIdx.x, (int)gridDim.x);
  const int tile_n = lb % p.n_tiles_n, tile_m = lb / p.n_tiles_n;
  const int m0 = tile_m * BM, n0 = tile_n * BN;

  const int oct = tid & 3, r0 = tid >> 2;
  RowPos rows[TM];
#pragma unroll
  for (int i = 0; i < TM; ++i) rows[i] = decode_row(p, m0 + r0 + 64 * i);
  long long a_off[TM];
  bool a_ok[TM];

  const int n_taps = p.kh * p.kw;
  const int n_steps = n_taps * (p.Cred / BK);

  float4 ra[TM][2];
  uint4 rah[TM], ral[TM];
  uint4 rbh[TN], rbl[TN];
  int tap = 0, ty = 0, tx = 0, red0 = 0;

  auto set_tap = [&]() {
#pragma unroll
    for (int i = 0; i < TM; ++i) a_ok[i] = tap_offset(p, rows[i], ty, tx, &a_off[i]);
  };
  auto load_step = [&]() {
#pragma unroll
    for (int i = 0; i < TM; ++i) {
      if (AP) {
        if (a_ok[i]) {
          const long long o8 = 2 * (((a_off[i] + red0) >> 3) + oct);
          rah[i] = g_ahi[o8];
          ral[i] = g_alo[o8];
        } else {
          rah[i] = make_uint4(0u, 0u, 0u, 0u);
          ral[i] = make_uint4(0u, 0u, 0u, 0u);
        }
      } else if (a_ok[i]) {
        const float4* s4 = reinterpret_cast<const float4*>(g_src + a_off[i] + red0 + 8 * oct);
        ra[i][0] = s4[0];
        ra[i][1] = s4[1];
      } else {
        ra[i][0] = make_float4(0.f, 0.f, 0.f, 0.f);
        ra[i][1] = make_float4(0.f, 0.f, 0.f, 0.f);
      }
    }
#pragma unroll
    for (int i = 0; i < TN; ++i) {
      const int n = n0 + r0 + 64 * i;
      if (n < w_rows) {
        const long long off = ((long long)tap * w_rows + n) * w_ld8 + (red0 >> 3) + oct;
        rbh[i] = g_whi[off];
        rbl[i] = g_wlo[off];
      } else {
        rbh[i] = make_uint4(0u, 0u, 0u, 0u);
        rbl[i] = make_uint4(0u, 0u, 0u, 0u);
      }
    }
  };
  auto advance = [&]() {
    red0 += BK;
    if (red0 >= p.Cred) {
      red0 = 0;
      ++tap;
      ++tx;
      if (tx == p.kw) { tx = 0; ++ty; }
      set_tap();
    }
  };
  auto store_step = [&]() {
#pragma unroll
    for (int i = 0; i < TM; ++i) {
      uint4 hi, lo;
      if (AP) {
        hi = rah[i];
        lo = ral[i];
      } else {
        split8(ra[i][0], ra[i][1], &hi, &lo);
      }
      const int slot = oct * BM + ((r0 + 64 * i + 2 * oct) & (BM - 1));
      Ahi[slot] = hi;
      Alo[slot] = lo;
    }
#pragma unroll
    for (int i = 0; i < TN; ++i) {
      const int slot = oct * BN + ((r0 + 64 * i + 2 * oct) & (BN - 1));
      Bhi[slot] = rbh[i];
      Blo[slot] = rbl[i];
    }
  };

  floatx16 acc[TM][TN];
#pragma unroll
  for (int a = 0; a < TM; ++a)
#pragma unroll
    for (int b = 0; b < TN; ++b)
#pragma unroll
      for (int r = 0; r < 16; ++r) acc[a][b][r] = 0.f;

  const int il = lane & 31, h = lane >> 5;

  set_tap();
  load_step();
  store_step();
  __syncthreads();

  for (int step = 0; step < n_steps; ++step) {
    const bool more = step + 1 < n_steps;
    if (more) {
      advance();
      load_step();
    }
    mma_step<TM, TN, BM, BN, 0>(acc, Ahi, Alo, Bhi, Blo, wm * 32 * TM + il, wn * 32 * TN + il, h);
    __syncthreads();
    if (more) {
      store_step();
      __syncthreads();
    }
  }

  epilogue3<TM, TN, OP>(p, acc, smem, m0, n0, tid, wm, wn, il, h, g_bias, g_addend, g_mask, g_out, g_ohi, g_olo);
}

template <int TM, int TN, bool AP, bool OP, bool SC, bool RL, bool MG>
__device__ __forceinline__ void igemm3f_body(
    const IgemmParams& p, const int bid, const int n_wg_in, const void* __restrict__ g_a0, const void* __restrict__ g_a1, unsigned a_bytes,
    const void* __restrict__ g_whi, const void* __restrict__ g_wlo, unsigned w_bytes,
    const float* __restrict__ g_bias, const float* __restrict__ g_addend, const float* __restrict__ g_mask,
    float* __restrict__ g_out, uint2* __restrict__ g_ohi, uint2* __restrict__ g_olo, int w_rows, int w_ld8, int splits,
    float* __restrict__ g_ws, const int* __restrict__ g_rl, const unsigned char* __restrict__ g_srcflags) {
  constexpr int BM = 64 * TM, BN = 64 * TN, BK = 32, NO = BK / 8;
  constexpr int SMEM_U4 = 2 * NO * (BM + BN);
  constexpr int ES = 4;
  __shared__ __attribute__((aligned(16))) uint4 smem[SMEM_U4];
  uint4* Ahi = smem;
  uint4* Alo = Ahi + NO * BM;
  uint4* Bhi = Alo + NO * BM;
  uint4* Blo = Bhi + NO * BN;

  const int tid = threadIdx.x, lane = tid & 63, wave = tid >> 6;
  const int wm = wave >> 1, wn = wave & 1;
  int n_wg = n_wg_in;
  if (RL) {
    n_wg = ((g_rl[0] + BM / 32 - 1) / (BM / 32)) * p.n_tiles_n * splits;
    if (bid >= n_wg) return;
  }
  const int lbs = xcd_remap(bid, n_wg);
  const int split = lbs % splits, lb = lbs / splits;
  const int tile_n = lb % p.n_tiles_n, tile_m = lb / p.n_tiles_n;
  const int m0 = tile_m * BM, n0 = tile_n * BN;
  int rl_blk[BM / 32];
  if (RL) {
    const int count = g_rl[0];
#pragma unroll
    for (int j = 0; j < BM / 32; ++j) {
      const int e = tile_m * (BM / 32) + j;
      rl_blk[j] = e < count ? g_rl[1 + e] * 32 : ((p.M + 31) & ~31);
    }
  }
  const int oct = tid & 3, r0 = tid >> 2;
  const int n_taps = p.kh * p.kw;
  const int steps_per_tap = p.Cred / BK;
  const int all_steps = n_taps * steps_per_tap;
  const int s_begin = (int)((long long)all_steps * split / splits), s_end = (int)((long long)all_steps * (split + 1) / splits);

  const __amdgpu_buffer_rsrc_t rs_a0 = __builtin_amdgcn_make_buffer_rsrc(const_cast<void*>(g_a0), 0, a_bytes, 0x00020000);
  const __amdgpu_buffer_rsrc_t rs_a1 = __builtin_amdgcn_make_buffer_rsrc(const_cast<void*>(AP ? g_a1 : g_a0), 0, AP ? a_bytes - 16 : a_bytes, 0x00020000);
  const __amdgpu_buffer_rsrc_t rs_wh = __builtin_amdgcn_make_buffer_rsrc(const_cast<void*>(g_whi), 0, w_bytes, 0x00020000);
  const __amdgpu_buffer_rsrc_t rs_wl = __builtin_amdgcn_make_buffer_rsrc(const_cast<void*>(g_wlo), 0, w_bytes, 0x00020000);

  int a_base[TM], a_pitch[TM];
  unsigned a_valid[TM];
#pragma unroll
  for (int i = 0; i < TM; ++i) {
    const int t_row = r0 + 64 * i;
    const RowPos r = decode_row(p, RL ? rl_blk[t_row >> 5] + (t_row & 31) : m0 + t_row);
    a_base[i] = ((r.rowbase + r.ybase * r.SW + r.xbase) * p.ld_src + 8 * oct) * ES;
    a_pitch[i] = p.tsign * r.SW * p.ld_src * ES;
    unsigned v = 0;
    int t = 0;
    for (int ty = 0; ty < p.kh; ++ty)
      for (int tx = 0; tx < p.kw; ++tx, ++t) {
        const int sy = r.ybase + ty * p.tsign, sx = r.xbase + tx * p.tsign;
        bool ok = r.ok && (unsigned)sy < (unsigned)r.SH && (unsigned)sx < (unsigned)r.SW;
        if (RL && g_srcflags && ok) ok = g_srcflags[(r.rowbase + sy * r.SW + sx) >> 5] != 0;
        if (ok) v |= 1u << t;
      }
    a_valid[i] = v;
  }
  const int x_pitch = p.tsign * p.ld_src * ES;
  int b_base[TN];
#pragma unroll
  for (int i = 0; i < TN; ++i) {
    const int n = n0 + r0 + 64 * i;
    b_base[i] = n < w_rows ? (n * w_ld8 + oct) * 16 : PP_BUF_OOB;
  }
  const int b_tap = w_rows * w_ld8 * 16;

  float4 ra[TM][2];
  uint4 rah[TM], ral[TM];
  uint4 rbh[TN], rbl[TN];
  int tap = s_begin / steps_per_tap, red0 = (s_begin - tap * steps_per_tap) * BK;
  int ty = tap / (MG ? max(p.kw, 1) : p.kw), tx = tap - ty * p.kw;

  auto load_step = [&]() {
    const int a_uni = tx * x_pitch + red0 * ES;
#pragma unroll
    for (int i = 0; i < TM; ++i) {
      int vo = a_base[i] + __mul24(ty, a_pitch[i]) + a_uni;
      vo = ((a_valid[i] >> tap) & 1u) ? vo : PP_BUF_OOB;
      if (AP) {
        rah[i] = buf_load16(rs_a0, vo, 0);
        ral[i] = buf_load16(rs_a1, vo, 0);
      } else {
        const uint4 q0 = buf_load16(rs_a0, vo, 0), q1 = buf_load16(rs_a0, vo + 16, 0);
        ra[i][0] = *reinterpret_cast<const float4*>(&q0);
        ra[i][1] = *reinterpret_cast<const float4*>(&q1);
      }
    }
    const int b_uni = ((p.w_ty0 + p.w_tstep * ty) * p.w_kw + p.w_tx0 + p.w_tstep * tx) * b_tap + (red0 >> 3) * 16;
#pragma unroll
    for (int i = 0; i < TN; ++i) {
      rbh[i] = buf_load16(rs_wh, b_base[i], b_uni);
      rbl[i] = buf_load16(rs_wl, b_base[i], b_uni);
    }
  };
  auto advance = [&](bool more) {
    red0 += BK;
    const bool wrap = red0 >= p.Cred;
    red0 = wrap ? 0 : red0;
    tap += wrap ? 1 : 0;
    tx += wrap ? 1 : 0;
    const bool wx = tx == p.kw;
    tx = wx ? 0 : tx;
    ty += wx ? 1 : 0;
    red0 = more ? red0 : 0;
    tap = more ? tap : 0;
    tx = more ? tx : 0;
    ty = more ? ty : 0;
  };
  auto split_step = [&]() {
    if (!AP) {
#pragma unroll
      for (int i = 0; i < TM; ++i) split8(ra[i][0], ra[i][1], &rah[i], &ral[i]);
    }
  };
  auto store_step = [&]() {
#pragma unroll
    for (int i = 0; i < TM; ++i) {
      const int slot = oct * BM + ((r0 + 64 * i + 2 * oct) & (BM - 1));
      Ahi[slot] = rah[i];
      Alo[slot] = ral[i];
    }
#pragma unroll
    for (int i = 0; i < TN; ++i) {
      const int slot = oct * BN + ((r0 + 64 * i + 2 * oct) & (BN - 1));
      Bhi[slot] = rbh[i];
      Blo[slot] = rbl[i];
    }
  };

  floatx16 acc[TM][TN];
#pragma unroll
  for (int a = 0; a < TM; ++a)
#pragma unroll
    for (int b = 0; b < TN; ++b)
#pragma unroll
      for (int r = 0; r < 16; ++r) acc[a][b][r] = 0.f;

  const int il = lane & 31, h = lane >> 5;

  if (!MG || s_begin < s_end) {
    load_step();
    split_step();
    store_step();
  }
  __syncthreads();

  for (int step = s_begin; step < s_end; ++step) {
    advance(step + 1 < s_end);
    load_step();
    __builtin_amdgcn_sched_barrier(0);
    mma_step<TM, TN, BM, BN, 2>(acc, Ahi, Alo, Bhi, Blo, wm * 32 * TM + il, wn * 32 * TN + il, h);
    split_step();
    __syncthreads();
    store_step();
    __syncthreads();
  }
  if (splits > 1) {
    float* slice = g_ws + (long long)split * (RL ? (((long long)p.M + 31) & ~31ll) : (long long)p.M) * p.ld_out;
#pragma unroll
    for (int a = 0; a < TM; ++a)
#pragma unroll
      for (int r = 0; r < 16; ++r) {
        const int trow = wm * 32 * TM + a * 32 + (r & 3) + 8 * (r >> 2) + 4 * h;
        const int m = m0 + trow;
        const bool row_ok = RL ? (rl_blk[trow >> 5] < p.M) : (m < p.M);
#pragma unroll
        for (int b = 0; b < TN; ++b) {
          const int co = n0 + wn * 32 * TN + b * 32 + il;
          if (row_ok && co < ((p.Nout + 3) & ~3)) slice[(long long)m * p.ld_out + co] = acc[a][b][r];
        }
      }
    return;
  }
  epilogue3<TM, TN, OP, PP_EPI_GF, SC, false, RL>(p, acc, smem, m0, n0, tid, wm, wn, il, h, g_bias, g_addend, g_mask, g_out, g_ohi, g_olo, rl_blk);
}

template <int TM, int TN, bool AP, bool OP, bool SC = false, bool RL = false>
__global__ __launch_bounds__(256, (TM * TN >= 8) ? 2 : ((TM * TN == 4) ? 3 : 4)) void igemm3f_kernel(
    const IgemmParams p, const void* __restrict__ g_a0, const void* __restrict__ g_a1, unsigned a_bytes,
    const void* __restrict__ g_whi, const void* __restrict__ g_wlo, unsigned w_bytes,
    const float* __restrict__ g_bias, const float* __restrict__ g_addend, const float* __restrict__ g_mask,
    float* __restrict__ g_out, uint2* __restrict__ g_ohi, uint2* __restrict__ g_olo, int w_rows, int w_ld8, int splits,
    float* __restrict__ g_ws, const int* __restrict__ g_rl = nullptr, const unsigned char* __restrict__ g_srcflags = nullptr) {
  igemm3f_body<TM, TN, AP, OP, SC, RL, false>(p, (int)blockIdx.x, (int)gridDim.x, g_a0, g_a1, a_bytes, g_whi, g_wlo, w_bytes, g_bias, g_addend,
                                              g_mask, g_out, g_ohi, g_olo, w_rows, w_ld8, splits, g_ws, g_rl, g_srcflags);
}

template <int TM, int TN, bool AP, bool OP>
__global__ __launch_bounds__(256, (TM * TN >= 8) ? 2 : ((TM * TN == 4) ? 3 : 4)) void igemm3m_kernel(
    const IgemmParams p0, const PpS2Merged g, const void* __restrict__ g_a0, const void* __restrict__ g_a1, unsigned a_bytes,
    const void* __restrict__ g_whi, const void* __restrict__ g_wlo, unsigned w_bytes, const float* __restrict__ g_addend,
    const float* __restrict__ g_mask, float* __restrict__ g_out, uint2* __restrict__ g_ohi, uint2* __restrict__ g_olo, int w_rows, int w_ld8) {
  const int bid = (int)blockIdx.x;
  PpS2Class c = g.c[0];
#pragma unroll
  for (int j = 1; j < 4; ++j)
    if (j < g.n_cls && bid >= g.c[j].blk_begin) c = g.c[j];
  IgemmParams p = p0;
  p.n_seg = 1;
  igemm_set_class(p, c);
  igemm3f_body<TM, TN, AP, OP, true, false, true>(p, bid - c.blk_begin, c.tiles, g_a0, g_a1, a_bytes, g_whi, g_wlo, w_bytes, nullptr, g_addend, g_mask,
                                                  g_out, g_ohi, g_olo, w_rows, w_ld8, 1, nullptr, nullptr, nullptr);
}

template <int TM, int TN, bool CAP, bool AP = false, bool OP = false>
__global__ __launch_bounds__(256, (TM * TN >= 8) ? 2 : ((TM * TN == 4) ? 3 : 4)) void igemm3x_kernel(
    const IgemmParams p, const void* __restrict__ g_a, const void* __restrict__ g_a1, unsigned a_bytes, const void* __restrict__ g_whi,
    const void* __restrict__ g_wlo, unsigned w_bytes, const float* __restrict__ g_bias, const float* __restrict__ g_addend,
    const float* __restrict__ g_mask, float* __restrict__ g_out, uint2* __restrict__ g_ohi, uint2* __restrict__ g_olo, int w_rows, int w_ld8,
    int splits, float* __restrict__ g_ws, void* __restrict__ g_chi, void* __restrict__ g_clo, const unsigned char* __restrict__ g_flags,
    int skip_halo) {
  static_assert(!(CAP && AP), "split capture is for f32 operands");
  constexpr int ES = 4;
  constexpr int BM = 64 * TM, BN = 64 * TN, BK = 32, NO = BK / 8;
  constexpr int AP1 = NO * BM + 1;
  constexpr int SMEM_U4 = 2 * AP1 + 2 * NO * BN;
  __shared__ __attribute__((aligned(16))) uint4 smem[SMEM_U4];
  uint4* Ahi = smem;
  uint4* Alo = Ahi + AP1;
  uint4* Bhi = Alo + AP1;
  uint4* Blo = Bhi + NO * BN;

  const int tid = threadIdx.x, lane = tid & 63, wave = tid >> 6;
  const int wm = wave >> 1, wn = wave & 1;
  const int lbs = xcd_remap((int)blockIdx.x, (int)gridDim.x);
  const int split = lbs % splits, lb = lbs / splits;
  const int tile_n = lb % p.n_tiles_n, tile_m = lb / p.n_tiles_n;
  const int m0 = p.m_off + tile_m * (BM - 2) - 1, n0 = tile_n * BN;
  const int oct = tid & 3, r0 = tid >> 2;
  const int il = lane & 31, h = lane >> 5;
  const int n_chunks = p.Cred / BK;
  const int all_groups = p.kh * n_chunks;
  const int g_begin = (int)((long long)all_groups * split / splits);
  int g_end = (int)((long long)all_groups * (split + 1) / splits);
  if (g_flags) {
    int lo = m0 - skip_halo, hi = m0 + BM - 1 + skip_halo;
    lo = lo < 0 ? 0 : lo;
    hi = hi > p.M - 1 ? p.M - 1 : hi;
    int any = 0;
    for (int b = lo >> 5; b <= (hi >> 5); ++b) any |= g_flags[b];
    g_end = any ? g_end : g_begin;
  }

  const __amdgpu_buffer_rsrc_t rs_a = __builtin_amdgcn_make_buffer_rsrc(const_cast<void*>(g_a), 0, a_bytes, 0x00020000);
  const __amdgpu_buffer_rsrc_t rs_a1 = __builtin_amdgcn_make_buffer_rsrc(const_cast<void*>(AP ? g_a1 : g_a), 0, AP ? a_bytes - 16 : a_bytes, 0x00020000);
  const __amdgpu_buffer_rsrc_t rs_wh = __builtin_amdgcn_make_buffer_rsrc(const_cast<void*>(g_whi), 0, w_bytes, 0x00020000);
  const __amdgpu_buffer_rsrc_t rs_wl = __builtin_amdgcn_make_buffer_rsrc(const_cast<void*>(g_wlo), 0, w_bytes, 0x00020000);

  int s_base[TM], s_pitch[TM];
#pragma unroll
  for (int i = 0; i < TM; ++i) {
    const int q = m0 + r0 + 64 * i;
    const RowPos r = decode_row(p, q < 0 ? 0 : q);
    const bool ok = q >= 0 && r.ok;
    const int x = r.xbase - p.off_x;
    s_base[i] = ((r.rowbase + r.ybase * r.SW + x) * p.ld_src + 8 * oct) * ES;
    int v = 0;
    for (int ty = 0; ty < p.kh; ++ty)
      if (ok && (unsigned)(r.ybase + ty * p.tsign) < (unsigned)r.SH) v |= 1 << ty;
    s_pitch[i] = (p.tsign * r.SW * p.ld_src * ES) | v;
  }
  unsigned f_valid[(TM + 1) / 2];
#pragma unroll
  for (int a = 0; a < (TM + 1) / 2; ++a) f_valid[a] = 0;
#pragma unroll
  for (int a = 0; a < TM; ++a) {
    const int q = m0 + wm * 32 * TM + a * 32 + il;
    const RowPos r = decode_row(p, q < 0 ? 0 : q);
    unsigned v = 0;
    int t = 0;
    for (int ty = 0; ty < p.kh; ++ty)
      for (int tx = 0; tx < 3; ++tx, ++t) {
        const int sy = r.ybase + ty * p.tsign, sx = r.xbase + tx * p.tsign;
        if (q >= 0 && r.ok && (unsigned)sy < (unsigned)r.SH && (unsigned)sx < (unsigned)r.SW) v |= 1u << t;
      }
    f_valid[a >> 1] |= v << (16 * (a & 1));
  }
  int b_base[TN];
#pragma unroll
  for (int i = 0; i < TN; ++i) {
    const int n = n0 + r0 + 64 * i;
    b_base[i] = n < w_rows ? (n * w_ld8 + oct) * 16 : PP_BUF_OOB;
  }
  const int b_tap = w_rows * w_ld8 * 16;

  float4 ra[TM][2];
  uint4 rah[TM], ral[TM];
  uint4 rbh[TN], rbl[TN];
  const bool ty_inner = p.x_ty_inner != 0;
  int ty = ty_inner ? g_begin % p.kh : g_begin / n_chunks;
  int chunk = ty_inner ? g_begin / p.kh : g_begin - ty * n_chunks;

  auto load_a = [&]() {
#pragma unroll
    for (int i = 0; i < TM; ++i) {
      int vo = s_base[i] + __mul24(ty, s_pitch[i] & ~15) + chunk * (BK * ES);
      vo = ((s_pitch[i] >> ty) & 1) ? vo : PP_BUF_OOB;
      if (AP) {
        rah[i] = buf_load16(rs_a, vo, 0);
        ral[i] = buf_load16(rs_a1, vo, 0);
      } else {
        const uint4 q0 = buf_load16(rs_a, vo, 0), q1 = buf_load16(rs_a, vo + 16, 0);
        ra[i][0] = *reinterpret_cast<const float4*>(&q0);
        ra[i][1] = *reinterpret_cast<const float4*>(&q1);
      }
    }
  };
  auto load_b = [&](int tx) {
    const int b_uni = ((p.w_ty0 + ty) * p.w_kw + tx) * b_tap + chunk * (BK / 8 * 16);
#pragma unroll
    for (int i = 0; i < TN; ++i) {
      rbh[i] = buf_load16(rs_wh, b_base[i], b_uni);
      rbl[i] = buf_load16(rs_wl, b_base[i], b_uni);
    }
  };
  auto split_a = [&]() {
    if (!AP) {
#pragma unroll
      for (int i = 0; i < TM; ++i) split8(ra[i][0], ra[i][1], &rah[i], &ral[i]);
    }
  };
  auto store_a = [&]() {
#pragma unroll
    for (int i = 0; i < TM; ++i) {
      const int slot = oct * BM + ((r0 + 64 * i + 2 * oct) & (BM - 1));
      Ahi[slot] = rah[i];
      Alo[slot] = ral[i];
    }
  };
  const int ty_c = -p.off_y * p.tsign;
  auto capture = [&]() {
    if constexpr (CAP) {
      const __amdgpu_buffer_rsrc_t rs_ch = __builtin_amdgcn_make_buffer_rsrc(g_chi, 0, a_bytes, 0x00020000);
      const __amdgpu_buffer_rsrc_t rs_cl = __builtin_amdgcn_make_buffer_rsrc(g_clo, 0, a_bytes - 16, 0x00020000);
      if (ty == ty_c && chunk % p.n_tiles_n == tile_n) {
#pragma unroll
        for (int i = 0; i < TM; ++i) {
          const int row = r0 + 64 * i;
          const int vo = s_base[i] + __mul24(ty, s_pitch[i] & ~15) + chunk * (BK * 4);
          const bool ok = ((s_pitch[i] >> ty) & 1) && row >= 1 && row <= BM - 2;
          const int co = ok ? vo : PP_BUF_OOB;
          buf_store16(rs_ch, rah[i], co);
          buf_store16(rs_cl, ral[i], co);
        }
      }
    }
  };
  auto store_b = [&]() {
#pragma unroll
    for (int i = 0; i < TN; ++i) {
      const int slot = oct * BN + ((r0 + 64 * i + 2 * oct) & (BN - 1));
      Bhi[slot] = rbh[i];
      Blo[slot] = rbl[i];
    }
  };

  floatx16 acc[TM][TN];
#pragma unroll
  for (int a = 0; a < TM; ++a)
#pragma unroll
    for (int b = 0; b < TN; ++b)
#pragma unroll
      for (int r = 0; r < 16; ++r) acc[a][b][r] = 0.f;

  auto mma_tile = [&](int c_ty, auto tx_c) {
    constexpr int TX = decltype(tx_c)::value;
    const int dx = p.off_x + TX * p.tsign;
    const unsigned tap_bits = (1u << (c_ty * 3 + TX)) * 0x10001u;
    unsigned okm[(TM + 1) / 2];
#pragma unroll
    for (int a = 0; a < (TM + 1) / 2; ++a) okm[a] = f_valid[a] & tap_bits;
    unsigned a_ok = 0;
#pragma unroll
    for (int a = 0; a < TM; ++a) a_ok |= (((okm[a >> 1] >> (16 * (a & 1))) & 0xffffu) != 0 ? 1u : 0u) << a;
    mma_step<TM, TN, BM, BN, 1>(acc, Ahi, Alo, Bhi, Blo, wm * 32 * TM + il + dx, wn * 32 * TN + il, h, a_ok, NO * BM);
  };

  std::integral_constant<int, 0> t0;
  std::integral_constant<int, 1> t1;
  std::integral_constant<int, 2> t2;
  if (threadIdx.x == 0) {
    Ahi[NO * BM] = make_uint4(0u, 0u, 0u, 0u);
    Alo[NO * BM] = make_uint4(0u, 0u, 0u, 0u);
  }
  load_a();
  load_b(0);
  split_a();
  store_a();
  store_b();
  __syncthreads();
  for (int g = g_begin; g < g_end; ++g) {
    const int c_ty = ty;
    capture();
    load_b(1);
    __builtin_amdgcn_sched_barrier(0);
    mma_tile(c_ty, t0);
    __syncthreads();
    store_b();
    __syncthreads();
    load_b(2);
    __builtin_amdgcn_sched_barrier(0);
    mma_tile(c_ty, t1);
    __syncthreads();
    store_b();
    __syncthreads();
    {
      const bool more = g + 1 < g_end;
      if (ty_inner) {
        ty += 1;
        const bool wt = ty == p.kh;
        ty = wt ? 0 : ty;
        chunk += wt ? 1 : 0;
      } else {
        chunk += 1;
        const bool wc = chunk == n_chunks;
        chunk = wc ? 0 : chunk;
        ty += wc ? 1 : 0;
      }
      chunk = more ? chunk : 0;
      ty = more ? ty : 0;
    }
    load_b(0);
    load_a();
    __builtin_amdgcn_sched_barrier(0);
    mma_tile(c_ty, t2);
    split_a();
    __syncthreads();
    store_b();
    store_a();
    __syncthreads();
  }
  if (splits > 1) {
    float* slice = g_ws + (long long)split * (p.M - p.m_off) * p.ld_out;
#pragma unroll
    for (int a = 0; a < TM; ++a)
#pragma unroll
      for (int r = 0; r < 16; ++r) {
        const int row = wm * 32 * TM + a * 32 + (r & 3) + 8 * (r >> 2) + 4 * h;
        const int m = m0 + row;
#pragma unroll
        for (int b = 0; b < TN; ++b) {
          const int co = n0 + wn * 32 * TN + b * 32 + il;
          if (row >= 1 && row <= BM - 2 && m < p.M && co < ((p.Nout + 3) & ~3)) slice[(long long)(m - p.m_off) * p.ld_out + co] = acc[a][b][r];
        }
      }
    return;
  }
  epilogue3<TM, TN, OP, 4, false, true>(p, acc, smem, m0, n0, tid, wm, wn, il, h, g_bias, g_addend, g_mask, g_out, g_ohi, g_olo);
}

__device__ __forceinline__ void finish4(const IgemmParams& p, float4 v, long long mo, int co, bool with_addend, const float* __restrict__ g_addend,
                                        const float* __restrict__ g_mask, float* __restrict__ g_out, void* __restrict__ g_ohi,
                                        void* __restrict__ g_olo) {
  if (with_addend) {
    if (p.add_hi) {
      const float4 a = planes_ld4(p.add_hi, p.add_lo, (mo * p.ld_add + co) >> 2);
      v.x += a.x; v.y += a.y; v.z += a.z; v.w += a.w;
    } else if (g_addend) {
      const float4 a = *reinterpret_cast<const float4*>(g_addend + mo * p.ld_add + co);
      v.x += a.x; v.y += a.y; v.z += a.z; v.w += a.w;
    }
  }
  if (p.mask_hi || g_mask) {
    const float4 k = p.mask_hi ? hi_ld4(p.mask_hi, (mo * p.ld_mask + co) >> 2) : *reinterpret_cast<const float4*>(g_mask + mo * p.ld_mask + co);
    v.x = k.x > 0.f ? v.x : 0.f; v.y = k.y > 0.f ? v.y : 0.f; v.z = k.z > 0.f ? v.z : 0.f; v.w = k.w > 0.f ? v.w : 0.f;
  }
  if (p.relu) { v.x = fmaxf(v.x, 0.f); v.y = fmaxf(v.y, 0.f); v.z = fmaxf(v.z, 0.f); v.w = fmaxf(v.w, 0.f); }
  if (g_out) *reinterpret_cast<float4*>(g_out + mo * p.ld_out + co) = v;
  if (g_ohi) planes_st4(g_ohi, g_olo, (mo * p.ld_out + co) >> 2, v);
}

__global__ void class_fill_kernel(const IgemmParams p, const float* __restrict__ g_addend, const float* __restrict__ g_mask,
                                  float* __restrict__ g_out, void* __restrict__ g_ohi, void* __restrict__ g_olo) {
  const int n4 = (p.Nout + 3) >> 2;
  const long long total = (long long)p.M * n4;
  const int hw = p.seg[0].OH * p.seg[0].OW;
  for (long long i = blockIdx.x * (long long)blockDim.x + threadIdx.x; i < total; i += (long long)gridDim.x * blockDim.x) {
    const int m = (int)(i / n4), co = 4 * (int)(i - (long long)m * n4);
    const int n = m / hw, rem = m - n * hw, yq = rem / p.seg[0].OW, xq = rem - yq * p.seg[0].OW;
    const long long mo = (long long)(n * p.sc_H + 2 * yq + p.sc_cy) * p.sc_W + 2 * xq + p.sc_cx;
    finish4(p, make_float4(0.f, 0.f, 0.f, 0.f), mo, co, true, g_addend, g_mask, g_out, g_ohi, g_olo);
  }
}

__global__ void splitk_finish_kernel(const IgemmParams p, int splits, const float* __restrict__ ws, const float* __restrict__ g_bias,
                                     const float* __restrict__ g_addend, const float* __restrict__ g_mask, float* __restrict__ g_out,
                                     void* __restrict__ g_ohi, void* __restrict__ g_olo) {
  const int n4 = (p.Nout + 3) >> 2;
  const int rows = p.M - p.m_off;
  const long long total = (long long)rows * n4, slice = (long long)rows * p.ld_out;
  for (long long i = blockIdx.x * (long long)blockDim.x + threadIdx.x; i < total; i += (long long)gridDim.x * blockDim.x) {
    const int mr = (int)(i / n4), co = 4 * (int)(i - (long long)mr * n4);
    const int m = p.m_off + mr;
    const float* w = ws + (long long)mr * p.ld_out + co;
    float4 v = *reinterpret_cast<const float4*>(w);
    for (int s = 1; s < splits; ++s) {
      const float4 q = *reinterpret_cast<const float4*>(w + s * slice);
      v.x += q.x; v.y += q.y; v.z += q.z; v.w += q.w;
    }
    if (g_bias) { const float4 b = *reinterpret_cast<const float4*>(g_bias + co); v.x += b.x; v.y += b.y; v.z += b.z; v.w += b.w; }
    finish4(p, v, (long long)m, co, true, g_addend, g_mask, g_out, g_ohi, g_olo);
  }
}

__global__ void rl_splitk_finish_kernel(const IgemmParams p, int splits, const float* __restrict__ ws, const int* __restrict__ g_rl,
                                        const float* __restrict__ g_bias, const float* __restrict__ g_addend, const float* __restrict__ g_mask,
                                        float* __restrict__ g_out, void* __restrict__ g_ohi, void* __restrict__ g_olo) {
  const int j = blockIdx.x;
  if (j >= g_rl[0]) return;
  const int n4 = (p.Nout + 3) >> 2;
  const long long slice = (((long long)p.M + 31) & ~31ll) * p.ld_out;
  const int m0 = g_rl[1 + j] * 32, nr = min(32, p.M - m0);
  for (int i = threadIdx.x; i < nr * n4; i += blockDim.x) {
    const int r = i / n4, co = 4 * (i - r * n4);
    const float* w = ws + ((long long)j * 32 + r) * p.ld_out + co;
    float4 v = *reinterpret_cast<const float4*>(w);
    for (int s = 1; s < splits; ++s) {
      const float4 q = *reinterpret_cast<const float4*>(w + s * slice);
      v.x += q.x; v.y += q.y; v.z += q.z; v.w += q.w;
    }
    if (g_bias) { const float4 b = *reinterpret_cast<const float4*>(g_bias + co); v.x += b.x; v.y += b.y; v.z += b.z; v.w += b.w; }
    finish4(p, v, (long long)(m0 + r), co, true, g_addend, g_mask, g_out, g_ohi, g_olo);
  }
}

__global__ void rl_dilate_kernel(const IgemmParams p, const unsigned char* __restrict__ in_flags, unsigned char* __restrict__ out_flags,
                                 int n_blocks) {
  const int b = blockIdx.x * blockDim.x + threadIdx.x;
  if (b >= n_blocks) return;
  const int r_lo = 32 * b, r_hi = min(32 * b + 31, p.M - 1);
  int any = 0;
  for (int s = 0; s < p.n_seg; ++s) {
    const int seg_lo = p.seg[s].row_begin, seg_hi = (s + 1 < p.n_seg ? p.seg[s + 1].row_begin : p.M) - 1;
    if (r_hi < seg_lo || r_lo > seg_hi) continue;
    const int W = p.seg[s].OW;
    for (int j = -1; j <= 1; ++j) {
      int lo = r_lo - 1 + j * W, hi = r_hi + 1 + j * W;
      lo = lo < 0 ? 0 : lo;
      hi = hi > p.M - 1 ? p.M - 1 : hi;
      for (int q = lo >> 5; q <= (hi >> 5); ++q) any |= in_flags[q];
    }
  }
  out_flags[b] = any ? 1 : 0;
}

__global__ void rl_fill_kernel(const IgemmParams p, const unsigned char* __restrict__ live, const float* __restrict__ g_addend,
                               const float* __restrict__ g_mask, float* __restrict__ g_out, void* __restrict__ g_ohi, void* __restrict__ g_olo) {
  const int b = blockIdx.x;
  if (live[b]) return;
  const int n4 = (p.Nout + 3) >> 2;
  const int r0 = 32 * b, nr = min(32, p.M - r0);
  if (g_ohi && !g_out && !g_addend && p.Nout == p.ld_out && (p.ld_out & 7) == 0 && (p.add_hi == nullptr || (p.ld_add & 7) == 0) &&
      (p.mask_hi == nullptr || (p.ld_mask & 7) == 0)) {
    const int n8 = nr * (p.ld_out >> 3);
    uint4* dst = reinterpret_cast<uint4*>(g_ohi) + 2 * (long long)r0 * (p.ld_out >> 3);
    const uint4 z4 = make_uint4(0u, 0u, 0u, 0u);
    for (int i = threadIdx.x; i < n8; i += blockDim.x) {
      uint4 oh = z4, ol = z4;
      if (p.add_hi) {
        const int r = i / (p.ld_out >> 3), g8 = i - r * (p.ld_out >> 3);
        const uint4* a = reinterpret_cast<const uint4*>(p.add_hi) + 2 * ((long long)(r0 + r) * (p.ld_add >> 3) + g8);
        oh = a[0];
        ol = a[1];
        if (p.mask_hi) {
          const uint4 k = reinterpret_cast<const uint4*>(p.mask_hi)[2 * ((long long)(r0 + r) * (p.ld_mask >> 3) + g8)];
          const unsigned kk[4] = {k.x, k.y, k.z, k.w};
          unsigned hh[4] = {oh.x, oh.y, oh.z, oh.w}, ll[4] = {ol.x, ol.y, ol.z, ol.w};
#pragma unroll
          for (int j = 0; j < 4; ++j) {
            const unsigned lo_ok = ((kk[j] & 0x8000u) == 0u && (kk[j] & 0x7fffu) != 0u) ? 0x0000ffffu : 0u;
            const unsigned hi_ok = ((kk[j] & 0x80000000u) == 0u && (kk[j] & 0x7fff0000u) != 0u) ? 0xffff0000u : 0u;
            hh[j] &= (lo_ok | hi_ok);
            ll[j] &= (lo_ok | hi_ok);
          }
          oh = make_uint4(hh[0], hh[1], hh[2], hh[3]);
          ol = make_uint4(ll[0], ll[1], ll[2], ll[3]);
        }
      }
      dst[2 * i] = oh;
      dst[2 * i + 1] = ol;
    }
    return;
  }
  for (int i = threadIdx.x; i < nr * n4; i += blockDim.x) {
    const int r = i / n4, co = 4 * (i - r * n4);
    const long long m = r0 + r;
    const float4 z = make_float4(0.f, 0.f, 0.f, 0.f);
    if (g_addend || p.add_hi) {
      finish4(p, z, m, co, true, g_addend, g_mask, g_out, g_ohi, g_olo);
    } else {
      if (g_out) *reinterpret_cast<float4*>(g_out + m * p.ld_out + co) = z;
      if (g_ohi) {
        reinterpret_cast<uint2*>(g_ohi)[pk4((m * p.ld_out + co) >> 2)] = make_uint2(0u, 0u);
        reinterpret_cast<uint2*>(g_olo)[pk4((m * p.ld_out + co) >> 2)] = make_uint2(0u, 0u);
      }
    }
  }
}

static void launch_splitk_finish(hipStream_t st, const IgemmParams& p, int splits, const float* ws, unsigned blocks, void* ohi, void* olo) {
  hipLaunchKernelGGL(splitk_finish_kernel, dim3(blocks), dim3(256), 0, st, p, splits, ws, p.bias, p.addend, p.mask_src, p.out, ohi, olo);
}

template <int TM, int TN, bool AP, bool OP, bool SC, bool RL>
static void launch_igemm3f(hipStream_t st, unsigned grid, const IgemmParams& p, const Igemm3Args& a, void* ohi, void* olo, int splits, float* ws,
                           const int* list, const unsigned char* srcflags) {
  const unsigned a_bytes = (unsigned)(p.src_rows * (long long)p.ld_src * 4), w_bytes = (unsigned)((long long)p.w_taps * a.w_rows * a.w_ld8 * 16);
  hipLaunchKernelGGL((igemm3f_kernel<TM, TN, AP, OP, SC, RL>), dim3(grid), dim3(256), 0, st, p, AP ? a.ahi : (const void*)p.src, AP ? a.alo : nullptr,
                     a_bytes, a.whi, a.wlo, w_bytes, p.bias, p.addend, p.mask_src, p.out, (uint2*)(OP ? ohi : nullptr), (uint2*)(OP ? olo : nullptr),
                     a.w_rows, a.w_ld8, splits, ws, list, srcflags);
}

template <int TM, int TN>
static void launch_igemm3_rowlist(hipStream_t st, IgemmParams& p, const Igemm3Args& a, const PpIgemmPlan& pl, const unsigned char* dy_flags,
                                  unsigned char* out_flags, int* out_list, bool fill) {
  const int nb = (p.M + 31) / 32, splits = pl.splits;
  float* const ws = splits > 1 ? a.ws : nullptr;
  const dim3 wg(256);
  p.n_tiles_n = pl.n_tiles_n;
  if (dy_flags) hipLaunchKernelGGL(rl_dilate_kernel, dim3((unsigned)((nb + 255) / 256)), wg, 0, st, p, dy_flags, out_flags, nb);
  PP_API(pp3_launch_row_block_compact)(st, out_flags, nb, out_list);
  if (a.ahi && !a.ohi)
    launch_igemm3f<TM, TN, true, false, false, true>(st, pl.grid, p, a, nullptr, nullptr, splits, ws, out_list, dy_flags);
  else if (a.ahi)
    launch_igemm3f<TM, TN, true, true, false, true>(st, pl.grid, p, a, a.ohi, a.olo, splits, ws, out_list, dy_flags);
  else
    launch_igemm3f<TM, TN, false, false, false, true>(st, pl.grid, p, a, nullptr, nullptr, splits, ws, out_list, dy_flags);
  if (pl.finish_blocks)
    hipLaunchKernelGGL(rl_splitk_finish_kernel, dim3(pl.finish_blocks), wg, 0, st, p, splits, (const float*)a.ws, (const int*)out_list, p.bias,
                       p.addend, p.mask_src, p.out, a.ohi, a.olo);
  const bool in_place = (a.ohi != nullptr && p.add_hi == (const void*)a.ohi && p.ld_add == p.ld_out && !p.out && !p.addend && !p.mask_hi &&
                         !p.mask_src && !p.relu) ||
                        (p.out != nullptr && p.addend == p.out && p.ld_add == p.ld_out && !a.ohi && !p.add_hi && !p.mask_hi && !p.mask_src && !p.relu);
  if (fill && !in_place)
    hipLaunchKernelGGL(rl_fill_kernel, dim3((unsigned)nb), wg, 0, st, p, (const unsigned char*)out_flags, p.addend, p.mask_src, p.out, a.ohi, a.olo);
}

template <int TM, int TN>
static void launch_igemm3(hipStream_t st, IgemmParams& p, const Igemm3Args& a, const PpIgemmPlan& pl) {
  const dim3 wg(256);
  const unsigned a_bytes = (unsigned)(p.src_rows * (long long)p.ld_src * 4), w_bytes = (unsigned)((long long)p.w_taps * a.w_rows * a.w_ld8 * 16);
  const int splits = pl.splits;
  float* const ws = splits > 1 ? a.ws : nullptr;
  uint2 *const no_hi = nullptr, *const no_lo = nullptr;
  const std::true_type yes{};
  const std::false_type no{};
  p.n_tiles_n = pl.n_tiles_n;
  p.x_ty_inner = pl.x_ty_inner;
  if (pl.capture_first) PP_API(pp3_split_capture_pass)(st, p, a.chi, a.clo);
  auto go_x = [&](auto cap, auto ap, auto op, const IgemmParams& q, unsigned grid, int q_splits, float* q_ws, const unsigned char* flags) {
    constexpr bool CAP = decltype(cap)::value, AP = decltype(ap)::value, OP = decltype(op)::value;
    if constexpr (AP || TM <= 2)
      hipLaunchKernelGGL((igemm3x_kernel<TM, TN, CAP, AP, OP>), dim3(grid), wg, 0, st, q, AP ? a.ahi : (const void*)q.src, AP ? a.alo : nullptr, a_bytes,
                         a.whi, a.wlo, w_bytes, q.bias, q.addend, q.mask_src, q.out, OP ? (uint2*)a.ohi : no_hi, OP ? (uint2*)a.olo : no_lo, a.w_rows,
                         a.w_ld8, q_splits, q_ws, CAP ? a.chi : nullptr, CAP ? a.clo : nullptr, flags, pl.skip_halo);
  };
  switch (pl.family) {
    case PP_IGEMM3F_CLASS:
      if (a.ahi) launch_igemm3f<TM, TN, true, true, true, false>(st, pl.grid, p, a, a.ohi, a.olo, 1, nullptr, nullptr, nullptr);
      else launch_igemm3f<TM, TN, false, false, true, false>(st, pl.grid, p, a, nullptr, nullptr, 1, nullptr, nullptr, nullptr);
      return;
    case PP_IGEMM4X:
      if constexpr (TM == 2 && TN == 2) {
        PP_API(pp3_launch_igemm4x)(st, p, a, pl);
        if (pl.tail_splits > 1) {
          IgemmParams q = p;
          q.m_off = pl.tail_m_off;
          go_x(no, yes, no, q, pl.tail_grid, pl.tail_splits, a.ws, nullptr);
          launch_splitk_finish(st, q, pl.tail_splits, a.ws, pl.finish_blocks, a.ohi, a.olo);
        }
      }
      return;
    case PP_IGEMM4X2:
      if constexpr (TM == 2 && TN == 2) PP_API(pp3_launch_igemm4x)(st, p, a, pl);
      return;
    case PP_IGEMM4P:
      if constexpr (TM == 2 && TN == 2)
        PP_API(pp4_launch_igemm4p)(st, p, a.ahi, a.whi, a.wlo, a.w_rows, a.w_ld8, a.ohi, a.olo, splits, ws, pl.grid, pl.stages);
      break;
    case PP_IGEMM3X_CAPTURE: go_x(yes, no, no, p, pl.grid, splits, ws, a.flags); break;
    case PP_IGEMM3X_PP: go_x(no, yes, yes, p, pl.grid, splits, ws, a.flags); break;
    case PP_IGEMM3X_PF: go_x(no, yes, no, p, pl.grid, splits, ws, a.flags); break;
    case PP_IGEMM3X_FP: go_x(no, no, yes, p, pl.grid, splits, ws, a.flags); break;
    case PP_IGEMM3X_FF: go_x(no, no, no, p, pl.grid, splits, ws, a.flags); break;
    default: {
      void *const ohi = splits > 1 ? nullptr : a.ohi, *const olo = splits > 1 ? nullptr : a.olo;
      auto go = [&](auto ap, auto op) {
        constexpr bool AP = decltype(ap)::value, OP = decltype(op)::value;
        if (pl.family == PP_IGEMM3F)
          launch_igemm3f<TM, TN, AP, OP, false, false>(st, pl.grid, p, a, ohi, olo, splits, ws, nullptr, nullptr);
        else
          hipLaunchKernelGGL((igemm3_kernel<TM, TN, AP, OP>), dim3(pl.grid), wg, 0, st, p, p.src, (const uint4*)(AP ? a.ahi : nullptr),
                             (const uint4*)(AP ? a.alo : nullptr), (const uint4*)a.whi, (const uint4*)a.wlo, p.bias, p.addend, p.mask_src, p.out,
                             (uint2*)ohi, (uint2*)olo, a.w_rows, a.w_ld8);
      };
      if (a.ahi && ohi) go(yes, yes);
      else if (a.ahi) go(yes, no);
      else if (ohi) go(no, yes);
      else go(no, no);
    }
  }
  if (pl.finish_blocks) launch_splitk_finish(st, p, splits, a.ws, pl.finish_blocks, a.ohi, a.olo);
}

template <int TM, int TN>
static void launch_igemm3m(hipStream_t st, IgemmParams& p, const Igemm3Args& a, const DgradS2Route& r) {
  const dim3 grid(r.g.grid), wg(256);
  const unsigned a_bytes = (unsigned)(p.src_rows * (long long)p.ld_src * 4), w_bytes = (unsigned)((long long)p.w_taps * a.w_rows * a.w_ld8 * 16);
  p.n_tiles_n = r.pl.n_tiles_n;
  auto go = [&](auto planes) {
    constexpr bool P = decltype(planes)::value;
    hipLaunchKernelGGL((igemm3m_kernel<TM, TN, P, P>), grid, wg, 0, st, p, r.g, P ? a.ahi : (const void*)p.src, P ? a.alo : nullptr, a_bytes, a.whi, a.wlo,
                       w_bytes, p.addend, p.mask_src, p.out, (uint2*)(P ? a.ohi : nullptr), (uint2*)(P ? a.olo : nullptr), a.w_rows, a.w_ld8);
  };
  if (a.ahi) go(std::true_type{});
  else go(std::false_type{});
}

}

void PP_API(pp3_launch_igemm)(hipStream_t st, IgemmParams& p, const Igemm3Args& a, const PpIgemmPlan& pl) {
  if (pl.tm == 4) launch_igemm3<4, 2>(st, p, a, pl);
  else if (pl.tm == 2 && pl.tn == 2) launch_igemm3<2, 2>(st, p, a, pl);
  else if (pl.tm == 1 && pl.tn == 2) launch_igemm3<1, 2>(st, p, a, pl);
  else if (pl.tm == 2 && pl.tn == 1) launch_igemm3<2, 1>(st, p, a, pl);
  else launch_igemm3<1, 1>(st, p, a, pl);
}

void PP_API(pp3_launch_igemm_s2)(hipStream_t st, IgemmParams& p, const Igemm3Args& a, const DgradS2Route& r) {
  if (r.pl.tm == 4) launch_igemm3m<4, 2>(st, p, a, r);
  else if (r.pl.tm == 2 && r.pl.tn == 2) launch_igemm3m<2, 2>(st, p, a, r);
  else if (r.pl.tm == 1 && r.pl.tn == 2) launch_igemm3m<1, 2>(st, p, a, r);
  else if (r.pl.tm == 2 && r.pl.tn == 1) launch_igemm3m<2, 1>(st, p, a, r);
  else launch_igemm3m<1, 1>(st, p, a, r);
}

void PP_API(pp3_launch_igemm_rowlist)(hipStream_t st, IgemmParams& p, const Igemm3Args& a, const PpIgemmPlan& pl, const unsigned char* dy_flags,
                                      unsigned char* out_flags, int* out_list, bool fill) {
  if (pl.tm == 2) launch_igemm3_rowlist<2, 2>(st, p, a, pl, dy_flags, out_flags, out_list, fill);
  else launch_igemm3_rowlist<1, 2>(st, p, a, pl, dy_flags, out_flags, out_list, fill);
}

void PP_API(pp3_launch_class_fill)(hipStream_t st, const IgemmParams& p, unsigned blocks, const float* addend, const float* mask, float* out, void* ohi,
                                   void* olo) {
  hipLaunchKernelGGL(class_fill_kernel, dim3(blocks), dim3(256), 0, st, p, addend, mask, out, ohi, olo);
}

void PP_API(pp3_launch_rl_dilate)(hipStream_t st, const IgemmParams& p, const unsigned char* in_flags, unsigned char* out_flags, int n_blocks) {
  hipLaunchKernelGGL(rl_dilate_kernel, dim3((unsigned)((n_blocks + 255) / 256)), dim3(256), 0, st, p, in_flags, out_flags, n_blocks);
}
```

### pyrapose_amd/csrc/conv_plan.h

```cpp
#pragma once
#include <stdarg.h>
#include <stdio.h>
#include <stdlib.h>

struct PpConvSwitches {
  int gscale_log2;
  bool fast;
  bool xreuse;
  int sparse_dgrad_splits;
  int sparse_dgrad;
  int x_order;
  int dma_min;
  int dma_frac;
  bool dma_tail;
  int dma_tail_frac;
  bool x4;
  bool s2_classes;
  int wgrad3w_min;
  int wgrad3_sp_steps;
};
inline int pp_env_int(const char* name, int dflt) { const char* e = getenv(name); return e ? atoi(e) : dflt; }
inline bool pp_env_not0(const char* name) { const char* e = getenv(name); return !(e && e[0] == '0'); }
inline bool pp_env_is1(const char* name) { const char* e = getenv(name); return e && e[0] == '1'; }
inline const PpConvSwitches& pp_conv_switches() {
  static const PpConvSwitches s = []() {
    PpConvSwitches v;
    const int g = pp_env_int("PP_GSCALE_LOG2", 8);
    v.gscale_log2 = g < -20 ? -20 : (g > 30 ? 30 : g);
    v.fast = pp_env_not0("PP_CONV3_FAST");
    v.xreuse = pp_env_not0("PP_CONV3_XREUSE");
    v.sparse_dgrad_splits = pp_env_int("PP_SPARSE_DGRAD_SPLITS", 2);
    v.sparse_dgrad = pp_env_int("PP_SPARSE_DGRAD", 22);
    v.x_order = pp_env_int("PP_CONV3_X_ORDER", 1);
    v.dma_min = pp_env_int("PP_CONV3_DMA_MIN", 512);
    v.dma_frac = pp_env_int("PP_CONV3_DMA_FRAC", 1000);
    v.dma_tail = pp_env_not0("PP_CONV3_DMA_TAIL");
    v.dma_tail_frac = pp_env_int("PP_CONV3_DMA_TAIL_FRAC", 60);
    v.x4 = pp_env_is1("PP_CONV3_X4");
    v.s2_classes = pp_env_not0("PP_CONV3_S2CLASSES");
    const int wm = pp_env_int("PP_WGRAD3W_MIN", 0);
    v.wgrad3w_min = wm > 0 ? wm : 512;
    const int ss = pp_env_int("PP_WGRAD3_SP_STEPS", 0);
    v.wgrad3_sp_steps = ss > 0 ? ss : 1;
    return v;
  }();
  return s;
}
inline bool pp_sw_debug() { return getenv("PP_CONV_DEBUG") != nullptr; }
inline bool pp_sw_dma() { return pp_env_not0("PP_CONV3_DMA"); }
inline int pp_sw_dma_var() { return pp_env_int("PP_CONV3_DMA_VAR", 1); }
inline bool pp_sw_dma2() { return pp_env_is1("PP_CONV3_DMA2"); }
inline int pp_sw_dma2_min() { return pp_env_int("PP_CONV3_DMA2_MIN", 512); }
inline bool pp_sw_conv4p() { return pp_env_is1("PP_CONV4P"); }
inline int pp_sw_conv4p_nst() { const char* e = getenv("PP_CONV4P_NST"); return e && atoi(e) == 3 ? 3 : 4; }
inline int pp_sw_conv4p_splits() { return pp_env_int("PP_CONV4P_SPLITS", 0); }
inline bool pp_sw_wgrad_det() { return pp_env_is1("PP_WGRAD3_DETERMINISTIC"); }
inline bool pp_sw_s2_merged() { return pp_env_not0("PP_CONV3_S2MERGED"); }
inline int pp_sw_wgrad3r() { const char* e = getenv("PP_WGRAD3R"); return !e ? -1 : ((e[0] == '1' || e[0] == '2') ? e[0] - '0' : 0); }
inline bool pp_sw_tile(const char* name, char* a, char* b) {
  const char* e = getenv(name);
  if (!(e && e[0] && e[1] == ',' && e[2])) return false;
  *a = e[0];
  *b = e[2];
  return true;
}
inline int pp_sw_splits(const char* name) { const char* e = getenv(name); return e ? atoi(e) : 0; }

inline int pp_cus(int n_cu) { return n_cu > 0 ? n_cu : 256; }

inline double est_rounds(long long blocks, int slots, int cus) {
  static const double thr[5] = {1.0, 0.62, 0.78, 0.81, 0.82};
  const long long per_round = (long long)cus * slots;
  const long long full = blocks / per_round;
  const long long rem = blocks - full * per_round;
  const int s_idx = slots < 4 ? slots : 4;
  double t = (double)full * slots / thr[s_idx];
  if (rem > 0) {
    const int c = (int)((rem + cus - 1) / cus);
    t += (double)c / thr[c < 4 ? c : 4];
  }
  return t;
}

inline unsigned pp_finish_blocks(long long rows, int Nout, int n_cu) {
  const long long total = rows * ((Nout + 3) >> 2);
  long long blocks = (total + 255) / 256;
  if (blocks > (long long)n_cu * 8) blocks = (long long)n_cu * 8;
  return (unsigned)blocks;
}

struct PpIgemmFacts {
  int M, Nout, Cred, kh, kw, ld_out, ld_src, w_rows, w_ld8, w_taps, div, mul, sc_on, w_tstep, w_tx0;
  long long src_rows;
  int max_sw;
  bool same_grid;
  bool planes_in, f32_in, planes_out, f32_out, capture, flags;
  bool listed;
  int listed_tm;
  int n_cu;
  bool ws;
  long long ws_bytes;
};

enum PpIgemmFamily {
  PP_IGEMM3, PP_IGEMM3F, PP_IGEMM3F_CLASS, PP_IGEMM3X_CAPTURE, PP_IGEMM3X_PP, PP_IGEMM3X_PF, PP_IGEMM3X_FP, PP_IGEMM3X_FF, PP_IGEMM4X,
  PP_IGEMM4X2, PP_IGEMM4P, PP_IGEMM3F_LIST, PP_IGEMM3F_S2
};
static const char* const pp_igemm_family_name[] = {
    "igemm3", "igemm3f", "igemm3f[parity class]", "igemm3x[capture]", "igemm3x[planes->planes]", "igemm3x[planes->f32]",
    "igemm3x[f32->planes]", "igemm3x[f32->f32]", "igemm4x", "igemm4x<NWM=2>", "igemm4p", "igemm3f[row list]", "igemm3f[stride-2 merged]"};

struct PpIgemmPlan {
  int family;
  int tm, tn, splits;
  int n_tiles_n;
  unsigned grid;
  int x_ty_inner, skip_halo;
  int full_rt, tail_splits, variant;
  int tail_m_off;
  unsigned tail_grid;
  int stages;
  bool capture_first;
  unsigned finish_blocks;
  long long ws_need;
  int n_steps;
  bool may_split;
};

inline bool pp_igemm_fast_ok(const PpIgemmFacts& f) {
  const long long a_bytes = f.src_rows * (long long)f.ld_src * 4;
  const long long w_bytes = (long long)f.w_taps * f.w_rows * f.w_ld8 * 16;
  return pp_conv_switches().fast && f.div == 1 && f.kh * f.kw <= 31 && a_bytes < (1ll << 31) && w_bytes < (1ll << 31) &&
         (long long)f.max_sw * f.ld_src * 4 < (1ll << 23) && f.src_rows > 0;
}

inline bool pp_igemm_x_ok(const PpIgemmFacts& f) {
  return pp_conv_switches().xreuse && pp_igemm_fast_ok(f) && !f.sc_on && f.kw == 3 && f.mul == 1 && f.div == 1 && (f.f32_in || f.planes_in) &&
         (!f.planes_in || f.ld_src % 8 == 0) && f.w_tstep == 1 && f.w_tx0 == 0 && f.same_grid;
}

inline void pp_pick_tile3(const PpIgemmFacts& f, int n_steps, bool may_split, bool x_ok, int* tm, int* tn, int* splits) {
  static const int cand[5][2] = {{4, 2}, {2, 2}, {1, 2}, {2, 1}, {1, 1}};
  static const double eff[5] = {1.1, 1.0, 0.9, 0.9, 0.8};
  static const int slots[5] = {2, 3, 4, 4, 4};
  static const int split_cand[8] = {1, 2, 3, 4, 6, 8, 12, 16};
  const int M = f.M, Nout = f.Nout, ld_out = f.ld_out, cus = f.n_cu;
  const long long ws_bytes = f.ws_bytes;
  double best = 1e300;
  *splits = 1;
  for (int i = 0; i < 5; ++i) {
    const int bm = 64 * cand[i][0], bn = 64 * cand[i][1];
    const long long blocks = (long long)((M + bm - 1) / bm) * ((Nout + bn - 1) / bn);
    for (int si = 0; si < (may_split ? 8 : 1); ++si) {
      const int sp = split_cand[si];
      if (sp > 1 && (n_steps / sp < 8 || (long long)sp * M * ld_out * 4 > ws_bytes)) break;
      const double steps = (double)((n_steps + sp - 1) / sp) + 8.0;
      double t = est_rounds(blocks * sp, slots[i], cus) * steps * cand[i][0] * cand[i][1] / eff[i];
      if (sp > 1) {
        const double us = (double)M * Nout * (8.0 * sp + 12.0) / 4.0e6 + 4.0;
        t += us / 2.1 * 4.0;
      }
      if (t < best * 0.97) {
        best = t;
        *tm = cand[i][0];
        *tn = cand[i][1];
        *splits = sp;
      }
    }
  }
  if (x_ok && *tm == 4 && *splits == 1 && !pp_conv_switches().x4) {
    *tm = 2;
    *tn = 2;
  }
  char a, b;
  if (pp_sw_tile("PP_CONV3_TILE", &a, &b)) {
    *tm = a - '0';
    *tn = b - '0';
  }
  if (const int v = pp_sw_splits("PP_CONV3_SPLITS")) {
    if (v >= 1 && (v == 1 || (may_split && n_steps / v >= 1 && (long long)v * M * ld_out * 4 <= ws_bytes))) *splits = v;
  }
  if (*tm == 4) *tn = 2;
  else if (!((*tm == 2 || *tm == 1) && (*tn == 2 || *tn == 1))) *tm = *tn = 1;
}

inline void pp_plan_listed(const PpIgemmFacts& f, PpIgemmPlan* pl) {
  const int nb = (f.M + 31) / 32, BM = 64 * f.listed_tm, BN = 128;
  const int want_splits = pp_conv_switches().sparse_dgrad_splits;
  int splits = 1;
  if (f.ws && want_splits > 1 && (f.planes_out || f.f32_out)) {
    const long long slice_bytes = (long long)nb * 32 * f.ld_out * 4;
    splits = want_splits;
    while (splits > 1 && (pl->n_steps / splits < 24 || slice_bytes * splits > f.ws_bytes)) --splits;
  }
  pl->family = PP_IGEMM3F_LIST;
  pl->tm = f.listed_tm;
  pl->tn = 2;
  pl->splits = splits;
  pl->n_tiles_n = (f.Nout + BN - 1) / BN;
  pl->grid = (unsigned)(((nb + BM / 32 - 1) / (BM / 32)) * pl->n_tiles_n * splits);
  pl->finish_blocks = splits > 1 ? (unsigned)nb : 0u;
  pl->ws_need = splits > 1 ? (long long)nb * 32 * f.ld_out * 4 * splits : 0;
}

inline PpIgemmPlan pp_plan_igemm(const PpIgemmFacts& f) {
  const PpConvSwitches& sw = pp_conv_switches();
  PpIgemmPlan pl = {};
  const int n_steps = pl.n_steps = f.kh * f.kw * (f.Cred / 32);
  const int n_cu = f.n_cu;
  if (f.listed) {
    pp_plan_listed(f, &pl);
    return pl;
  }
  if (pp_sw_conv4p()) {
    const long long a_bytes = f.src_rows * (long long)f.ld_src * 4, w_bytes = (long long)f.w_taps * f.w_rows * f.w_ld8 * 16;
    if (f.kh == 1 && f.kw == 1 && f.planes_in && !f.capture && !f.flags && !f.sc_on && f.div == 1 && f.Cred % 32 == 0 && f.ld_src % 8 == 0 &&
        a_bytes < (1ll << 31) && w_bytes < (1ll << 31) && f.src_rows > 0 && (f.planes_out || f.f32_out)) {
      const int p_splits = pp_sw_conv4p_splits();
      const long long tiles = (long long)((f.M + 127) / 128) * ((f.Nout + 127) / 128);
      int sp = 1;
      if (tiles * 4 < (long long)n_cu * 3 && f.ws) {
        sp = (int)(n_cu / tiles);
        while (sp > 1 && (n_steps / sp < 4 || (long long)sp * f.M * f.ld_out * 4 > f.ws_bytes)) --sp;
      }
      if (p_splits >= 1 && (p_splits == 1 || (f.ws && n_steps / p_splits >= 1 && (long long)p_splits * f.M * f.ld_out * 4 <= f.ws_bytes)))
        sp = p_splits;
      pl.family = PP_IGEMM4P;
      pl.tm = pl.tn = 2;
      pl.splits = sp;
      pl.stages = pp_sw_conv4p_nst();
      pl.n_tiles_n = (f.Nout + 127) / 128;
      const long long n_items = tiles * sp;
      pl.grid = (unsigned)(n_items < n_cu ? n_items : n_cu);
      pl.finish_blocks = sp > 1 ? pp_finish_blocks(f.M, f.Nout, n_cu) : 0u;
      pl.ws_need = sp > 1 ? (long long)sp * f.M * f.ld_out * 4 : 0;
      return pl;
    }
  }
  const bool fast = pp_igemm_fast_ok(f), x_ok = pp_igemm_x_ok(f);
  const bool may_split = pl.may_split = f.ws && (f.planes_out || f.f32_out) && !f.sc_on && fast;
  int tm = 1, tn = 1, splits = 1;
  pp_pick_tile3(f, n_steps, may_split, x_ok, &tm, &tn, &splits);
  pl.tm = tm;
  pl.tn = tn;
  pl.splits = splits;
  const int BM = 64 * tm, BN = 64 * tn;
  pl.n_tiles_n = (f.Nout + BN - 1) / BN;
  pl.grid = (unsigned)(((f.M + BM - 1) / BM) * pl.n_tiles_n * splits);
  pl.finish_blocks = splits > 1 ? pp_finish_blocks(f.M, f.Nout, n_cu) : 0u;
  pl.ws_need = splits > 1 ? (long long)splits * f.M * f.ld_out * 4 : 0;
  if (f.sc_on) {
    pl.family = PP_IGEMM3F_CLASS;
    return pl;
  }
  if (x_ok && (tm <= 2 || (f.planes_in && !f.capture))) {
    const int n_tiles_mx = (f.M + BM - 3) / (BM - 2);
    pl.skip_halo = f.max_sw + 1;
    pl.grid = (unsigned)(n_tiles_mx * pl.n_tiles_n * splits);
    pl.x_ty_inner = sw.x_order;
    const bool op = f.planes_out && splits == 1;
    if (tm <= 2 && f.capture) {
      pl.family = PP_IGEMM3X_CAPTURE;
      return pl;
    }
    if (tm == 2 && tn == 2 && pp_sw_dma() && f.planes_in && op && !f.flags && splits == 1 && f.kh == 3 && sw.x_order == 1 && f.w_rows % 128 == 0 &&
        f.Cred % 32 == 0) {
      const int BM4 = 256;
      const int n_tiles_m4 = (f.M + BM4 - 3) / (BM4 - 2);
      const int ntn = (f.Nout + 127) / 128;
      const int n_blk = n_tiles_m4 * ntn;
      const bool one_and_a_bit = n_blk > n_cu && n_blk < 2 * n_cu && (n_blk - n_cu) * 100 >= sw.dma_frac * n_cu;
      if (n_blk >= sw.dma_min || one_and_a_bit) {
        int full_rt = n_tiles_m4;
        const int rounds = (n_tiles_m4 * ntn) / n_cu;
        const int last = (n_tiles_m4 * ntn) % n_cu;
        if (sw.dma_tail && last != 0 && last * 100 < sw.dma_tail_frac * n_cu && rounds >= 2 && f.ws) full_rt = rounds * n_cu / ntn;
        const int m_split = full_rt * (BM4 - 2);
        int tail_splits = 0;
        if (full_rt < n_tiles_m4) {
          const int rem = f.M - m_split;
          const int n_rt = (rem + BM - 3) / (BM - 2);
          const int groups = f.kh * (f.Cred / 32);
          int sp = (3 * n_cu + n_rt * ntn - 1) / (n_rt * ntn);
          while (sp > 1 && (groups / sp < 4 || (long long)sp * rem * f.ld_out * 4 > f.ws_bytes)) --sp;
          if (sp > 1) tail_splits = sp;
          else full_rt = n_tiles_m4;
        }
        const int var = pp_sw_dma_var();
        pl.family = PP_IGEMM4X;
        pl.variant = (var == 0 || var == 2 || var == 3 || var == 4 || var == 9) ? var : 1;
        pl.n_tiles_n = ntn;
        pl.full_rt = full_rt;
        pl.grid = (unsigned)(full_rt * ntn);
        pl.tail_splits = tail_splits;
        if (tail_splits > 1) {
          const int rem = f.M - full_rt * (BM4 - 2);
          pl.tail_m_off = full_rt * (BM4 - 2);
          pl.tail_grid = (unsigned)(((rem + BM - 3) / (BM - 2)) * ntn * tail_splits);
          pl.finish_blocks = pp_finish_blocks(rem, f.Nout, n_cu);
          pl.ws_need = (long long)tail_splits * rem * f.ld_out * 4;
        }
        return pl;
      }
      if (pp_sw_dma2() && n_tiles_mx * ntn >= pp_sw_dma2_min()) {
        pl.family = PP_IGEMM4X2;
        pl.n_tiles_n = ntn;
        pl.grid = (unsigned)(n_tiles_mx * ntn);
        return pl;
      }
    }
    pl.family = f.planes_in ? (op ? PP_IGEMM3X_PP : PP_IGEMM3X_PF) : (op ? PP_IGEMM3X_FP : PP_IGEMM3X_FF);
    return pl;
  }
  pl.capture_first = f.capture;
  pl.family = fast ? PP_IGEMM3F : PP_IGEMM3;
  return pl;
}

struct PpDgradRouteFacts {
  int stride, kh, kw, pad_t, pad_l, n_seg;
  bool all_f32, all_planes, capture, bias, skip, skip_scratch, fast_ok, same_grid;
};
inline bool pp_dgrad_listed_ok(const PpDgradRouteFacts& r) {
  return r.skip && r.skip_scratch && pp_conv_switches().sparse_dgrad && (r.all_f32 || r.all_planes) && !r.capture && r.stride == 1 && r.kh == 3 &&
         r.kw == 3 && r.pad_t == 1 && r.pad_l == 1 && !r.bias && r.fast_ok && r.same_grid;
}
inline bool pp_dgrad_classes_ok(const PpDgradRouteFacts& r) {
  return r.stride == 2 && pp_conv_switches().s2_classes && (r.all_f32 || r.all_planes) && r.n_seg == 1;
}

struct PpS2Class {
  int cy, cx;
  int kh, kw;
  int off_y, off_x, w_ty0, w_tx0;
  int OH, OW, M;
  int tiles, blk_begin;
};
inline void pp_s2_classes(int n_img, int H, int W, int kh, int kw, int pad_t, int pad_l, PpS2Class cls[4]) {
  for (int c = 0; c < 4; ++c) {
    PpS2Class& r = cls[c];
    r.cy = c >> 1;
    r.cx = c & 1;
    const int ty0 = (r.cy + pad_t) & 1, tx0 = (r.cx + pad_l) & 1;
    r.kh = ty0 < kh ? (kh - ty0 + 1) / 2 : 0;
    r.kw = tx0 < kw ? (kw - tx0 + 1) / 2 : 0;
    r.off_y = (r.cy + pad_t - ty0) / 2;
    r.off_x = (r.cx + pad_l - tx0) / 2;
    r.w_ty0 = ty0;
    r.w_tx0 = tx0;
    if (r.kh == 0 || r.kw == 0) r.kh = r.kw = 0;
    r.OH = (H - r.cy + 1) / 2;
    r.OW = (W - r.cx + 1) / 2;
    r.M = n_img * r.OH * r.OW;
    r.tiles = r.blk_begin = 0;
  }
}
struct PpS2Merged {
  int n_cls;
  unsigned grid;
  PpS2Class c[4];
};
inline PpS2Merged pp_s2_merge(const PpS2Class cls[4], int BM, int BN, int Nout) {
  PpS2Merged g = {};
  for (int c = 0; c < 4; ++c) {
    if (cls[c].M <= 0) continue;
    int at = g.n_cls++;
    for (; at > 0 && g.c[at - 1].kh * g.c[at - 1].kw < cls[c].kh * cls[c].kw; --at) g.c[at] = g.c[at - 1];
    g.c[at] = cls[c];
  }
  const long long ntn = (Nout + BN - 1) / BN;
  long long at = 0;
  for (int i = 0; i < g.n_cls; ++i) {
    g.c[i].tiles = (int)(((g.c[i].M + BM - 1) / BM) * ntn);
    g.c[i].blk_begin = (int)at;
    at += g.c[i].tiles;
  }
  g.grid = (unsigned)at;
  return g;
}
inline bool pp_dgrad_s2_ok(const PpDgradRouteFacts& r) { return r.stride == 2 && (r.all_f32 || r.all_planes) && r.n_seg == 1; }

struct PpWgradFacts {
  int M, Cin, Cout, kh, kw, stride, pad_t, pad_l, ld_src, ld_dy, ld_w;
  long long src_rows;
  int min_ow, min_hw;
  bool same_grid;
  bool list_levels_aligned;
  long long Mp;
  bool planes, list, lazy_in;
  int fmt;
  int n_cu;
  bool ws;
  long long ws_bytes;
  bool dw_aligned, dbias_aligned;
};

enum PpWgradFamily { PP_WGRAD3, PP_WGRAD3F_PLANES_LIST, PP_WGRAD3F_PLANES, PP_WGRAD3F_F32_LIST, PP_WGRAD3F_F32, PP_WGRAD3R, PP_WGRAD3W };
static const char* const pp_wgrad_family_name[] = {"wgrad3", "wgrad3f[planes, list]", "wgrad3f[planes]", "wgrad3f[f32, list]", "wgrad3f[f32]",
                                                   "wgrad3r", "wgrad3w"};

struct PpWgradPlan {
  int family;
  bool refused;
  int tm, tn;
  bool fast;
  int k_tiles_per_tap, n_tiles_k, n_tiles_n, tiles;
  int model_splits;
  int splits, rows_per_split, max_wraps, sp_min_steps;
  bool use_ws;
  long long ws_slice;
  unsigned grid, finish_blocks;
  long long ws_need;
};

inline bool pp_plan_wgrad3r(const PpWgradFacts& f, int variant, PpWgradPlan* pl) {
  if (!(f.kh == 3 && f.kw == 3 && f.stride == 1 && f.pad_t == 1 && f.pad_l == 1 && f.Cin % 128 == 0 && f.planes)) return false;
  if (variant == 2 && f.list) return false;
  if (!f.same_grid) return false;
  if (f.list && !f.list_levels_aligned) return false;
  const long long x_bytes = f.src_rows * (long long)f.ld_src * 4, d_bytes = (long long)f.M * f.ld_dy * 4;
  if (!(f.min_ow >= (f.list ? 12 : 2) && x_bytes < (1ll << 31) && d_bytes < (1ll << 31) && f.Mp < (1 << 24) && f.src_rows > 0)) return false;
  pl->k_tiles_per_tap = f.Cin / 128;
  pl->n_tiles_k = 3 * pl->k_tiles_per_tap;
  pl->n_tiles_n = (f.Cout + 127) / 128;
  const int tiles = pl->tiles = pl->n_tiles_k * pl->n_tiles_n;
  const int R = f.list ? f.M : (int)f.Mp;
  int max_splits = (R + 255) / 256;
  if (max_splits > 128) max_splits = 128;
  if (max_splits < 1) max_splits = 1;
  const double atomic_steps_per_split = 0.5 * (double)tiles * 3.0 * 128.0 * 128.0 * 4.0 / 1.3e6 / 1.0;
  int splits = 1;
  double best = 1e300;
  for (int sp = 1; sp <= max_splits; ++sp) {
    const double steps = (double)((R + sp - 1) / sp + 31) / 32.0 + 6.0;
    const double rounds = (double)(((long long)tiles * sp + f.n_cu - 1) / f.n_cu);
    const double cost = rounds * steps + atomic_steps_per_split * sp;
    if (cost < best * 0.995) {
      best = cost;
      splits = sp;
    }
  }
  if (const int v = pp_sw_splits("PP_WGRAD3R_SPLITS")) {
    if (v >= 1 && v <= max_splits) splits = v;
  }
  int rps = (R + splits - 1) / splits;
  rps = (rps + 31) / 32 * 32;
  splits = (R + rps - 1) / rps;
  pl->family = variant == 2 ? PP_WGRAD3W : PP_WGRAD3R;
  pl->tm = pl->tn = 2;
  pl->fast = true;
  pl->model_splits = pl->splits = splits;
  pl->rows_per_split = rps;
  pl->grid = (unsigned)(tiles * splits);
  return true;
}

inline PpWgradPlan pp_plan_wgrad(const PpWgradFacts& f) {
  const PpConvSwitches& sw = pp_conv_switches();
  PpWgradPlan pl = {};
  pl.sp_min_steps = sw.wgrad3_sp_steps;
  const bool det = pp_sw_wgrad_det();
  {
    const int e_r = pp_sw_wgrad3r();
    int variant = 0;
    if (e_r > 0) variant = e_r;
    else if (e_r < 0 && f.fmt == 1 && !f.list && (f.Cin >= sw.wgrad3w_min || f.Cout >= sw.wgrad3w_min)) variant = 2;
    if (variant && f.planes && !(det && f.ws) && (!f.lazy_in || f.list) && pp_plan_wgrad3r(f, variant, &pl)) return pl;
  }
  bool big_k = (f.Cin % 128 == 0);
  bool big_n = ((f.Cout + 127) / 128 * 128) <= ((f.Cout + 63) / 64 * 64);
  char a, b;
  if (pp_sw_tile("PP_WGRAD3_TILE", &a, &b)) {
    big_k = big_k && a == '2';
    big_n = b == '2';
  }
  const int TM = pl.tm = big_k ? 2 : 1, TN = pl.tn = big_n ? 2 : 1;
  pl.max_wraps = (32 + f.min_ow - 1) / f.min_ow;
  const int BM = 64 * TM, BN = 64 * TN;
  pl.k_tiles_per_tap = f.Cin / BM;
  pl.n_tiles_k = f.kh * f.kw * pl.k_tiles_per_tap;
  pl.n_tiles_n = (f.Cout + BN - 1) / BN;
  const int tiles = pl.tiles = pl.n_tiles_k * pl.n_tiles_n;
  const int cus = f.n_cu;
  int max_splits = (f.M + 511) / 512;
  if (max_splits < 1) max_splits = 1;
  if (max_splits > 64) max_splits = 64;
  const long long x_bytes = f.src_rows * (long long)f.ld_src * 4, d_bytes = (long long)f.M * f.ld_dy * 4;
  const bool fast = pl.fast = sw.fast && x_bytes < (1ll << 31) && d_bytes < (1ll << 31) && f.M < (1 << 24) && f.src_rows > 0 && f.min_hw >= 32;
  if (f.lazy_in && !(fast && f.list)) {
    pl.refused = true;
    return pl;
  }
  const int slots = fast ? ((TM * TN == 4) ? 3 : 4) : ((TM * TN == 4) ? 2 : 3);
  const double tile_work = (double)(TM * TN) / 4.0;
  const long long ws_slice = pl.ws_slice = (long long)f.kh * f.kw * f.Cin * f.ld_w + f.ld_w;
  const bool use_ws = pl.use_ws = fast && f.ws && f.ws_bytes >= ws_slice * 4 && f.dw_aligned && f.dbias_aligned && det;
  if (use_ws) {
    const long long fit = f.ws_bytes / (ws_slice * 4);
    if (max_splits > fit) max_splits = (int)fit;
  }
  const double atomic_us_per_split = use_ws ? (double)tiles * BM * BN * 4.0 * 2.0 / 4.0e6 : 0.5 * (double)tiles * BM * BN * 4.0 / 1.3e6;
  int splits = 1;
  double best = 1e300;
  for (int sp = 1; sp <= max_splits; ++sp) {
    const double steps = (double)((f.M + sp - 1) / sp + 31) / 32.0;
    const double cost = est_rounds((long long)tiles * sp, slots, cus) * steps * tile_work * 0.8 + atomic_us_per_split * sp;
    if (cost < best * 0.995) {
      best = cost;
      splits = sp;
    }
  }
  if (const int v = pp_sw_splits("PP_WGRAD3_SPLITS")) {
    if (v >= 1 && v <= max_splits) splits = v;
  }
  pl.model_splits = splits;
  int rps = (f.M + splits - 1) / splits;
  rps = (rps + 31) / 32 * 32;
  splits = (f.M + rps - 1) / rps;
  pl.splits = splits;
  pl.rows_per_split = rps;
  pl.grid = (unsigned)(tiles * splits);
  pl.family = !fast ? PP_WGRAD3
                    : (f.planes ? (f.list ? PP_WGRAD3F_PLANES_LIST : PP_WGRAD3F_PLANES) : (f.list ? PP_WGRAD3F_F32_LIST : PP_WGRAD3F_F32));
  if (use_ws && splits > 1) {
    const long long n4 = (ws_slice - f.ld_w) / 4;
    long long blocks = (n4 + f.ld_w / 4 + 255) / 256;
    if (blocks > (long long)cus * 8) blocks = (long long)cus * 8;
    pl.finish_blocks = (unsigned)blocks;
    pl.ws_need = (long long)splits * ws_slice * 4;
  }
  return pl;
}

inline int pp_plan_append(char* buf, int cap, int at, const char* fmt, ...) {
  if (at >= cap) return at;
  va_list ap;
  va_start(ap, fmt);
  const int n = vsnprintf(buf + at, (size_t)(cap - at), fmt, ap);
  va_end(ap);
  return n < 0 ? at : (at + n < cap ? at + n : cap);
}
inline int pp_plan_print(char* buf, int cap, int at, const PpIgemmFacts& f, const PpIgemmPlan& pl, bool detail) {
  if (pl.family == PP_IGEMM4P)
    at = pp_plan_append(buf, cap, at, "igemm4p M %d N %d steps %d -> %lld tiles x %d splits on %d CUs, %d stages", f.M, f.Nout, pl.n_steps,
                        (long long)((f.M + 127) / 128) * ((f.Nout + 127) / 128), pl.splits, f.n_cu, pl.stages);
  else if (pl.family == PP_IGEMM3F_LIST)
    at = pp_plan_append(buf, cap, at, "igemm3 M %d N %d steps %d -> tile %dx%d splits %d (listed blocks)", f.M, f.Nout, pl.n_steps, 64 * pl.tm,
                        64 * pl.tn, pl.splits);
  else
    at = pp_plan_append(buf, cap, at, "igemm3 M %d N %d steps %d -> tile %dx%d splits %d (may_split %d: ws %d planes_out %d out %d)", f.M, f.Nout,
                        pl.n_steps, 64 * pl.tm, 64 * pl.tn, pl.splits, (int)pl.may_split, (int)f.ws, (int)f.planes_out, (int)f.f32_out);
  at = pp_plan_append(buf, cap, at, " %s", pp_igemm_family_name[pl.family]);
  if (detail)
    at = pp_plan_append(buf, cap, at, " | grid=%u n_tiles_n=%d x_ty_inner=%d skip_halo=%d full_rt=%d tail_splits=%d tail_grid=%u tail_m_off=%d "
                        "variant=%d stages=%d capture_first=%d finish_blocks=%u ws_need=%lld",
                        pl.grid, pl.n_tiles_n, pl.x_ty_inner, pl.skip_halo, pl.full_rt, pl.tail_splits, pl.tail_grid, pl.tail_m_off, pl.variant,
                        pl.stages, (int)pl.capture_first, pl.finish_blocks, pl.ws_need);
  return pp_plan_append(buf, cap, at, "\n");
}
inline int pp_plan_print(char* buf, int cap, int at, const PpWgradFacts& f, const PpWgradPlan& pl, bool detail) {
  if (pl.refused) return pp_plan_append(buf, cap, at, "wgrad3 refused: lazy dy without a listed-block reduction\n");
  if (pl.family == PP_WGRAD3R || pl.family == PP_WGRAD3W)
    at = pp_plan_append(buf, cap, at, "wgrad3r tiles %d (3 taps each) splits %d (M %d)%s", pl.tiles, pl.splits, f.M, f.list ? " listed blocks" : "");
  else
    at = pp_plan_append(buf, cap, at, "wgrad3 tile %dx%d tiles %d splits %d (M %d) fast %d", 64 * pl.tm, 64 * pl.tn, pl.tiles, pl.model_splits, f.M,
                        (int)pl.fast);
  at = pp_plan_append(buf, cap, at, " %s", pp_wgrad_family_name[pl.family]);
  if (detail)
    at = pp_plan_append(buf, cap, at, " | grid=%u tile=%dx%d splits=%d rows_per_split=%d max_wraps=%d sp_min_steps=%d use_ws=%d ws_slice=%lld "
                        "finish_blocks=%u ws_need=%lld",
                        pl.grid, 64 * pl.tm, 64 * pl.tn, pl.splits, pl.rows_per_split, pl.max_wraps, pl.sp_min_steps, (int)pl.use_ws, pl.ws_slice,
                        pl.finish_blocks, pl.ws_need);
  return pp_plan_append(buf, cap, at, "\n");
}
inline int pp_plan_print(char* buf, int cap, int at, const PpIgemmFacts& f, const PpIgemmPlan& pl, const PpS2Merged& g, bool detail) {
  at = pp_plan_append(buf, cap, at, "igemm3 s2 N %d -> tile %dx%d, %d classes:", f.Nout, 64 * pl.tm, 64 * pl.tn, g.n_cls);
  for (int i = 0; i < g.n_cls; ++i)
    at = pp_plan_append(buf, cap, at, " (%d,%d) M %d steps %d", g.c[i].cy, g.c[i].cx, g.c[i].M, g.c[i].kh * g.c[i].kw * (f.Cred / 32));
  at = pp_plan_append(buf, cap, at, " %s", pp_igemm_family_name[PP_IGEMM3F_S2]);
  if (detail) {
    at = pp_plan_append(buf, cap, at, " | grid=%u n_tiles_n=%d class_grids=", g.grid, pl.n_tiles_n);
    for (int i = 0; i < g.n_cls; ++i) at = pp_plan_append(buf, cap, at, i ? "+%d" : "%d", g.c[i].tiles);
  }
  return pp_plan_append(buf, cap, at, "\n");
}
template <class Facts, class Plan>
inline void pp_plan_debug(const Facts& f, const Plan& pl) {
  if (!pp_sw_debug()) return;
  char line[512];
  pp_plan_print(line, (int)sizeof(line), 0, f, pl, false);
  fputs(line, stderr);
}
inline void pp_plan_debug(const PpIgemmFacts& f, const PpIgemmPlan& pl, const PpS2Merged& g) {
  if (!pp_sw_debug()) return;
  char line[512];
  pp_plan_print(line, (int)sizeof(line), 0, f, pl, g, false);
  fputs(line, stderr);
}
```

### pyrapose_amd/csrc/ctx.hip

```cpp
#include <stdlib.h>

#include "pp_internal.h"

extern "C" const char* pp_version(void) { return "pyrapose_hip 0.7 (gfx950; convolutions on packed planes in two formats -- bf16 pairs / bf16x3 and P16 / f16c8 (f16 + block-scaled e5m2 MFMA) -- and exact f32 MFMA; sparse 3D-box backward, pose tail, device augmentation)"; }

extern "C" int pp_ctx_create(pp_ctx** out, int device, void* hip_stream) {
  if (!out) return PP_ERR_ARG;
  *out = nullptr;
  int n_dev = 0;
  hipError_t e = hipGetDeviceCount(&n_dev);
  if (e != hipSuccess) return (int)e;
  if (device < 0 || device >= n_dev) return PP_ERR_ARG;
  pp_ctx* c = (pp_ctx*)calloc(1, sizeof(pp_ctx));
  if (!c) return PP_ERR_ARG;
  c->device = device;
  c->stream = (hipStream_t)hip_stream;
  hipDeviceProp_t prop;
  e = hipGetDeviceProperties(&prop, device);
  if (e != hipSuccess) {
    free(c);
    return (int)e;
  }
  c->n_cu = prop.multiProcessorCount;
  snprintf(c->name, sizeof(c->name), "%s (%s)", prop.name, prop.gcnArchName);
  c->err[0] = 0;
  *out = c;
  return PP_OK;
}

extern "C" void pp_ctx_destroy(pp_ctx* ctx) { free(ctx); }

extern "C" int pp_ctx_set_stream(pp_ctx* ctx, void* hip_stream) {
  PP_REQUIRE_CTX(ctx);
  ctx->stream = (hipStream_t)hip_stream;
  return PP_OK;
}

extern "C" int pp_ctx_set_workspace(pp_ctx* ctx, void* zeroed, size_t bytes) {
  PP_REQUIRE_CTX(ctx);
  PP_CHECK_ARG(ctx, (zeroed == nullptr) == (bytes == 0) && pp_is_aligned16(zeroed), PP_ERR_ARG, "pp_ctx_set_workspace: bad buffer");
  ctx->ws = (float*)zeroed;
  ctx->ws_bytes = bytes;
  return PP_OK;
}

extern "C" int pp_ctx_set_planes_format(pp_ctx* ctx, int fmt) {
  PP_REQUIRE_CTX(ctx);
  PP_CHECK_ARG(ctx, fmt == 0 || fmt == 1, PP_ERR_ARG, "pp_ctx_set_planes_format: 0 (bf16 pairs) or 1 (P16)");
  ctx->planes_fmt = fmt;
  return PP_OK;
}

extern "C" int pp_ctx_set_grad_scale(pp_ctx* ctx, const float* scale2_dev) {
  PP_REQUIRE_CTX(ctx);
  ctx->grad_scale = scale2_dev;
  return PP_OK;
}

extern "C" const char* pp_last_error_string(pp_ctx* ctx) { return ctx ? ctx->err : "no context"; }

extern "C" int pp_device_info(pp_ctx* ctx, int* n_cu, char* name, int name_len) {
  PP_REQUIRE_CTX(ctx);
  if (n_cu) *n_cu = ctx->n_cu;
  if (name && name_len > 0) {
    strncpy(name, ctx->name, (size_t)name_len - 1);
    name[name_len - 1] = 0;
  }
  return PP_OK;
}
```

### pyrapose_amd/csrc/pp_internal.h

```cpp
#pragma once
#include <hip/hip_runtime.h>
#include <stdarg.h>
#include <stdio.h>
#include <string.h>

#include "pyrapose_hip.h"

struct pp_ctx {
  int device;
  hipStream_t stream;
  int n_cu;
  char name[128];
  char err[512];
  float* ws;
  size_t ws_bytes;
  int planes_fmt;
  const float* grad_scale;
};

static inline int pp_fail(pp_ctx* ctx, int code, const char* fmt, ...) {
  if (ctx) {
    va_list ap;
    va_start(ap, fmt);
    vsnprintf(ctx->err, sizeof(ctx->err), fmt, ap);
    va_end(ap);
  }
  return code;
}

#define PP_REQUIRE_CTX(ctx) \
  do {                      \
    if (!(ctx)) return PP_ERR_NOCTX; \
  } while (0)

#define PP_CHECK_ARG(ctx, cond, code, ...)            \
  do {                                                \
    if (!(cond)) return pp_fail(ctx, code, __VA_ARGS__); \
  } while (0)

#define PP_CHECK_LAUNCH(ctx, what)                                                   \
  do {                                                                               \
    hipError_t e__ = hipGetLastError();                                              \
    if (e__ != hipSuccess)                                                           \
      return pp_fail(ctx, (int)e__, "%s: launch failed: %s", what, hipGetErrorString(e__)); \
  } while (0)

#define PP_HIP(ctx, call)                                                                        \
  do {                                                                                           \
    hipError_t e__ = (call);                                                                     \
    if (e__ != hipSuccess) return pp_fail(ctx, (int)e__, "%s: %s", #call, hipGetErrorString(e__)); \
  } while (0)

static inline long long pp_rowspace_rows(const pp_rowspace* rs) {
  long long r = 0;
  for (int s = 0; s < rs->n_seg; ++s) r += (long long)rs->n_img * rs->h[s] * rs->w[s];
  return r;
}

static inline int pp_rowspace_ok(const pp_rowspace* rs) {
  if (rs->n_img <= 0 || rs->n_seg <= 0 || rs->n_seg > PP_MAX_SEG) return 0;
  for (int s = 0; s < rs->n_seg; ++s)
    if (rs->h[s] <= 0 || rs->w[s] <= 0) return 0;
  return pp_rowspace_rows(rs) < (1ll << 31);
}

static inline int pp_is_aligned16(const void* p) { return (((uintptr_t)p) & 15u) == 0; }
static inline int pp_is_packed(const void* hi, const void* lo) {
  return (hi == nullptr && lo == nullptr) || (hi != nullptr && (const char*)lo == (const char*)hi + 16 && pp_is_aligned16(hi));
}

enum { PP_OPT_CAPTURE = 1, PP_OPT_ADD = 2, PP_OPT_MASK = 4, PP_OPT_SKIP = 8, PP_OPT_LAZY_OUT = 16, PP_OPT_LAZY_IN = 32, PP_OPT_OUT = 64 };
static inline int pp_conv_opts_take(pp_ctx* ctx, const pp_conv_opts*& o, unsigned takes, const char* who) {
  static const pp_conv_opts none = {};
  if (!o) o = &none;
  const struct { unsigned group; bool set; const char* name; } fields[] = {
      {PP_OPT_CAPTURE, o->capture_hi != nullptr, "capture_hi"}, {PP_OPT_CAPTURE, o->capture_lo != nullptr, "capture_lo"},
      {PP_OPT_ADD, o->add_hi != nullptr, "add_hi"},             {PP_OPT_ADD, o->add_lo != nullptr, "add_lo"},
      {PP_OPT_MASK, o->mask_hi != nullptr, "mask_hi"},          {PP_OPT_SKIP, o->skip_flags != nullptr, "skip_flags"},
      {PP_OPT_SKIP, o->skip_list != nullptr, "skip_list"},      {PP_OPT_OUT, o->out_flags != nullptr, "out_flags"},
      {PP_OPT_OUT, o->out_list != nullptr, "out_list"},         {PP_OPT_LAZY_OUT, o->lazy_out != 0, "lazy_out"},
      {PP_OPT_LAZY_IN, o->lazy_in != 0, "lazy_in"}};
  for (const auto& f : fields) PP_CHECK_ARG(ctx, !f.set || (takes & f.group), PP_ERR_ARG, "%s: pp_conv_opts.%s is not an option of this call", who, f.name);
  PP_CHECK_ARG(ctx, (o->capture_hi == nullptr) == (o->capture_lo == nullptr) && pp_is_aligned16(o->capture_hi) && pp_is_aligned16(o->capture_lo),
               PP_ERR_ARG, "%s: pp_conv_opts.capture_hi and capture_lo go together, 16-byte aligned", who);
  PP_CHECK_ARG(ctx, (o->add_hi == nullptr) == (o->add_lo == nullptr), PP_ERR_ARG, "%s: pp_conv_opts.add_hi and add_lo go together", who);
  PP_CHECK_ARG(ctx, pp_is_packed(o->add_hi, o->add_lo) && pp_is_aligned16(o->mask_hi), PP_ERR_ALIGN,
               "%s: pp_conv_opts epilogue planes must be packed (lo = hi + 16 bytes) and 16-byte aligned", who);
  PP_CHECK_ARG(ctx, (o->out_flags == nullptr) == (o->out_list == nullptr), PP_ERR_ARG, "%s: pp_conv_opts.out_flags and out_list go together", who);
  PP_CHECK_ARG(ctx, !(o->lazy_out || o->lazy_in) || (o->skip_flags && o->skip_list), PP_ERR_ARG,
               "%s: pp_conv_opts.lazy_out / lazy_in go with skip_flags and skip_list", who);
  return PP_OK;
}
```

### pyrapose_amd/ops.py

```python
import collections
import ctypes as C

import numpy as np
import torch

from ._lib import ConvDesc, ConvOpts, ParamDesc, RowSpace, TView, check, lib
from ._lib import check as check_status


def _ptr(t):
    if t is None:
        return None
    assert t.is_cuda, "pyrapose_amd ops need device tensors"
    return C.c_void_p(t.data_ptr())


class Context:

    def __init__(self, device=0, stream=None):
        if not torch.cuda.is_available():
            raise RuntimeError("pyrapose_amd: no GPU visible (torch.cuda.is_available() is False); "
                               "the HIP path has no CPU fallback")
        self.device = int(device)
        torch.cuda.set_device(self.device)
        self.handle = C.c_void_p()
        s = stream if stream is not None else torch.cuda.current_stream(self.device)
        self.stream = s
        check(lib.pp_ctx_create(C.byref(self.handle), self.device, C.c_void_p(s.cuda_stream)), None, "pp_ctx_create")

        self.planes_fmt = 0
        self._twin = None

    def use_stream(self, stream):
        for c in (self, self._twin):
            if c is not None:
                c.stream = stream
                check(lib.pp_ctx_set_stream(c.handle, C.c_void_p(stream.cuda_stream)), c.handle, "pp_ctx_set_stream")

    def twin(self, fmt):
        if int(fmt) == self.planes_fmt:
            return self
        if self._twin is None:
            t = Context(self.device, self.stream)
            set_planes_format(t, fmt)
            t._twin = self
            ws = getattr(self, "workspace", None)
            t.workspace = ws
            if ws is not None:
                check(lib.pp_ctx_set_workspace(t.handle, _ptr(ws), ws.numel() * 4), t.handle, "pp_ctx_set_workspace")
            self._twin = t
        assert self._twin.planes_fmt == int(fmt)
        return self._twin

    def set_workspace(self, nbytes):
        self.workspace = torch.empty((int(nbytes) // 4,), dtype=torch.float32, device="cuda:%d" % self.device) if nbytes else None
        for c in (self, self._twin):
            if c is not None:
                c.workspace = self.workspace
                check(lib.pp_ctx_set_workspace(c.handle, _ptr(self.workspace), (int(nbytes) // 4) * 4 if nbytes else 0), c.handle,
                      "pp_ctx_set_workspace")

    def device_info(self):
        n = C.c_int(0)
        buf = C.create_string_buffer(128)
        check(lib.pp_device_info(self.handle, C.byref(n), buf, 128), self.handle)
        return n.value, buf.value.decode()

    def close(self):
        t, self._twin = self._twin, None
        if t is not None and t.handle:
            t._twin = None
            t.close()
        if self.handle:
            lib.pp_ctx_destroy(self.handle)
            self.handle = C.c_void_p()


def make_conv_desc(n_img, in_shapes, out_shapes, cin, cout, k, stride, pad_t, pad_l, ld_x, ld_y, ld_w):
    d = ConvDesc()
    d.in_ = RowSpace.make(n_img, in_shapes)
    d.out = RowSpace.make(n_img, out_shapes)
    d.cin, d.cout, d.kh, d.kw, d.stride = cin, cout, k, k, stride
    d.pad_t, d.pad_l, d.ld_x, d.ld_y, d.ld_w = pad_t, pad_l, ld_x, ld_y, ld_w
    return d


PLAN_FWD, PLAN_BWD_DATA, PLAN_BWD_WEIGHT, PLAN_BWD_DATA_S2 = 0, 1, 2, 3
PLAN_PLANES_IN, PLAN_PLANES_OUT, PLAN_F32_OUT, PLAN_CAPTURE, PLAN_LIST, PLAN_LAZY_IN, PLAN_LAZY_OUT = 1, 2, 4, 8, 16, 32, 64


def conv_plan_text(d, pass_, forms=0, planes_fmt=1, n_cu=256, ws_bytes=0):
    buf = C.create_string_buffer(4096)
    n = lib.pp_conv_plan_text(C.byref(d), int(pass_), int(forms), int(planes_fmt), int(n_cu), int(ws_bytes), buf, len(buf))
    check(min(n, 0), None, "pp_conv_plan_text")
    return buf.value.decode()


def conv_fwd(ctx, d, x, w, bias, residual, relu, y):
    ld_res = residual.stride(0) if residual is not None else 0
    check(lib.pp_conv2d_nhwc_fwd(ctx.handle, C.byref(d), _ptr(x), _ptr(w), _ptr(bias), _ptr(residual), ld_res,
                                 int(bool(relu)), _ptr(y)), ctx.handle, "pp_conv2d_nhwc_fwd")


def conv_bwd_data(ctx, d, dy, w, addend, relu_src, dx):
    ld_add = addend.stride(0) if addend is not None else 0
    ld_rs = relu_src.stride(0) if relu_src is not None else 0
    check(lib.pp_conv2d_nhwc_bwd_data(ctx.handle, C.byref(d), _ptr(dy), _ptr(w), _ptr(addend), ld_add, _ptr(relu_src),
                                      ld_rs, _ptr(dx)), ctx.handle, "pp_conv2d_nhwc_bwd_data")


def conv_bwd_weight(ctx, d, x, dy, dw, dbias):
    check(lib.pp_conv2d_nhwc_bwd_weight(ctx.handle, C.byref(d), _ptr(x), _ptr(dy), _ptr(dw), _ptr(dbias)), ctx.handle,
          "pp_conv2d_nhwc_bwd_weight")


def conv_split_weights3(ctx, d, w, fwd_hi, fwd_lo, dg_hi, dg_lo):
    check(lib.pp_conv_split_weights_bf16x3(ctx.handle, C.byref(d), _ptr(w), _ptr(fwd_hi), _ptr(fwd_lo), _ptr(dg_hi), _ptr(dg_lo)),
          ctx.handle, "pp_conv_split_weights_bf16x3")


class SplitWeightsBatch(object):

    def __init__(self, jobs):
        from ._lib import SplitJob
        jobs = list(jobs)
        arr = (SplitJob * max(len(jobs), 1))()
        tiles = 0
        self._keep = jobs
        for i, (d, w, fh, fl, dh, dl) in enumerate(jobs):
            if d.cin % 32:
                raise ValueError("SplitWeightsBatch: cin %d must be a multiple of 32" % d.cin)
            j = arr[i]
            j.w, j.fwd_hi, j.fwd_lo, j.dg_hi, j.dg_lo = [(t.data_ptr() if t is not None else None) for t in (w, fh, fl, dh, dl)]
            j.taps, j.cin, j.cout, j.ld_w, j.tile_begin = d.kh * d.kw, d.cin, d.cout, d.ld_w, tiles
            tiles += j.taps * (d.cin // 32) * ((d.cout + 31) // 32)
        self.n, self.tiles = len(jobs), tiles
        host = torch.frombuffer(bytearray(bytes(arr)), dtype=torch.uint8)
        self.table = host.cuda()

    def run(self, ctx):
        check(lib.pp_conv_split_weights_bf16x3_batch(ctx.handle, self.n, _ptr(self.table), self.tiles), ctx.handle,
              "pp_conv_split_weights_bf16x3_batch")


def new_planes(rows, ld, device="cuda", fill=0):
    assert ld % 8 == 0, ld
    base = torch.full((rows, ld // 8, 2, 8), fill, dtype=torch.int16, device=device)
    return base[:, :, 0, :], base[:, :, 1, :]


def planes_ld(planes):
    return planes[0].stride(0) // 2


def set_planes_format(ctx, fmt):
    check(lib.pp_ctx_set_planes_format(ctx.handle, int(fmt)), ctx.handle, "pp_ctx_set_planes_format")
    ctx.planes_fmt = int(fmt)


def convert_planes(ctx, src, src_fmt, dst, dst_fmt, scale2=None, scale_index=0, relu_src_hi=None):
    n = src[0].numel()
    check(lib.pp_convert_planes(ctx.handle, n, _ptr(src[0]), _ptr(src[1]), int(src_fmt), _ptr(dst[0]), _ptr(dst[1]), int(dst_fmt), _ptr(scale2),
                                int(scale_index), _ptr(relu_src_hi)), ctx.handle, "pp_convert_planes")


def planes_to_f32(planes, fmt=0):
    hi, lo = planes
    rows = hi.shape[0]
    if fmt == 0:
        return (hi.contiguous().view(torch.bfloat16).float() + lo.contiguous().view(torch.bfloat16).float()).reshape(rows, -1)
    rem = (lo.contiguous().to(torch.int32) & 0xff00).to(torch.int16).view(torch.float16).float() / 4096.0
    return (hi.contiguous().view(torch.float16).float() + rem).reshape(rows, -1)


def weight_planes_to_f32(hi, lo, fmt=0):
    if fmt == 0:
        return hi.contiguous().view(torch.bfloat16).float() + lo.contiguous().view(torch.bfloat16).float()
    rem = ((lo.contiguous().to(torch.int32) & 0xff) << 8).to(torch.int16).view(torch.float16).float() / 4096.0
    return hi.contiguous().view(torch.float16).float() + rem


def split_planes3(ctx, src, hi, lo, scale=None):
    if scale is None:
        check(lib.pp_split_planes_bf16x3(ctx.handle, src.numel(), _ptr(src), _ptr(hi), _ptr(lo)), ctx.handle, "pp_split_planes_bf16x3")
    else:
        check(lib.pp_split_planes_scaled_bf16x3(ctx.handle, src.numel(), _ptr(src), _ptr(hi), _ptr(lo), _ptr(scale)), ctx.handle,
              "pp_split_planes_scaled_bf16x3")


def grad_scale_from_counts(ctx, counts, scale2, log2_adjust=0):
    check(lib.pp_grad_scale_from_counts_adj(ctx.handle, _ptr(counts), int(counts.numel()), _ptr(scale2), int(log2_adjust)), ctx.handle,
          "pp_grad_scale_from_counts")


def set_grad_scale(ctx, scale2):
    ctx._grad_scale_keep = scale2
    check(lib.pp_ctx_set_grad_scale(ctx.handle, _ptr(scale2)), ctx.handle, "pp_ctx_set_grad_scale")


def row_block_list(ctx, x, cols, flags=None, blocks=None):
    rows, ld = x.shape
    nb = (rows + 31) // 32
    if flags is None:
        flags = torch.zeros((2 * nb,), dtype=torch.uint8, device=x.device)
    if blocks is None:
        blocks = torch.zeros((2 * (nb + 1),), dtype=torch.int32, device=x.device)
    check(lib.pp_row_block_list(ctx.handle, _ptr(x), rows, x.stride(0), int(cols), _ptr(flags), _ptr(blocks)), ctx.handle, "pp_row_block_list")
    return flags, blocks


def row_block_list_planes(ctx, planes, cols, flags, blocks, within=None):
    hi, lo = planes
    rows = hi.shape[0]
    if within is not None:
        assert within.dtype == torch.uint8 and within.is_contiguous() and within.numel() >= (rows + 31) // 32
        check(lib.pp_row_block_list_planes_within(ctx.handle, _ptr(hi), _ptr(lo), rows, planes_ld(planes), int(cols), _ptr(within), _ptr(flags),
                                                  _ptr(blocks)), ctx.handle, "pp_row_block_list_planes_within")
    else:
        check(lib.pp_row_block_list_planes(ctx.handle, _ptr(hi), _ptr(lo), rows, planes_ld(planes), int(cols), _ptr(flags), _ptr(blocks)),
              ctx.handle, "pp_row_block_list_planes")
    return flags, blocks


def tview(t=None, planes=None):
    v = TView()
    v.f32 = t.data_ptr() if t is not None else None
    v.hi = planes[0].data_ptr() if planes is not None else None
    v.lo = planes[1].data_ptr() if planes is not None else None
    v._keep = (t, planes)
    return v


def _numel(v):
    t, planes = v._keep
    return (t if t is not None else planes[0]).numel()


def add_n_v(ctx, a, b, c, out):
    null = TView()
    check(lib.pp_add_n_v(ctx.handle, _numel(a), C.byref(a), C.byref(b if b is not None else null), C.byref(c if c is not None else null),
                         C.byref(out)), ctx.handle, "pp_add_n_v")
# ... 1321 lines not shown
```

Measured before the change: 615.8.

## Fold split-K reduction into the GEMM launch using per-tile arrival tickets

Adds a device ticket buffer to the context. Split-K igemm3f/igemm3x kernels now atomically count arrivals per output tile, and the last arriving workgroup sums the workspace slices and runs the epilogue itself. This removes the separate split-K finish kernel launch and its extra pass over the workspace. In exchange it adds atomics, fences and a serialized tail reduction in the last CTA per tile, and it depends on the tickets being reset correctly between calls.

```diff
diff --git a/include/pyrapose_hip.h b/include/pyrapose_hip.h
--- a/include/pyrapose_hip.h
+++ b/include/pyrapose_hip.h
@@ -24,6 +24,8 @@
 void pp_ctx_destroy(pp_ctx* ctx);
 int pp_ctx_set_stream(pp_ctx* ctx, void* hip_stream);
 int pp_ctx_set_workspace(pp_ctx* ctx, void* device_buffer, size_t bytes);
+int pp_ctx_set_tickets(pp_ctx* ctx, int* device_buffer, size_t count, int zero);
+int pp_ctx_tickets_nonzero(pp_ctx* ctx, int* count);
 int pp_row_block_list(pp_ctx* ctx, const float* x, int rows, int ld, int cols, unsigned char* flags, int* list);
 int pp_row_block_list_planes(pp_ctx* ctx, const void* x_hi, const void* x_lo, int rows, int ld, int cols, unsigned char* flags, int* list);
 int pp_row_block_list_planes_within(pp_ctx* ctx, const void* x_hi, const void* x_lo, int rows, int ld, int cols, const unsigned char* within,
@@ -123,6 +125,7 @@
 #define PP_PLAN_LIST 16u
 #define PP_PLAN_LAZY_IN 32u
 #define PP_PLAN_LAZY_OUT 64u
+#define PP_PLAN_TICKETS 128u
 int pp_conv_plan_text(const pp_conv_desc* d, int pass, unsigned forms, int planes_fmt, int n_cu, size_t ws_bytes, char* buf,
                       int buf_bytes);
 
diff --git a/pyrapose_amd/_lib.py b/pyrapose_amd/_lib.py
--- a/pyrapose_amd/_lib.py
+++ b/pyrapose_amd/_lib.py
@@ -101,6 +101,8 @@
     "pp_allreduce_bucket": (_i, [_p, _p, _p, C.c_size_t]),
     "pp_allreduce_counts": (_i, [_p, _p, _p, _i]),
     "pp_ctx_set_workspace": (_i, [_p, _p, C.c_size_t]),
+    "pp_ctx_set_tickets": (_i, [_p, _p, C.c_size_t, _i]),
+    "pp_ctx_tickets_nonzero": (_i, [_p, C.POINTER(C.c_int)]),
     "pp_row_block_list": (_i, [_p, _p, _i, _i, _i, _p, _p]),
     "pp_positive_row_blocks": (_i, [_p, _p, _i, _i, _p, _p]),
     "pp_row_block_dilate": (_i, [_p, _p, _p, _p]),
diff --git a/pyrapose_amd/csrc/conv3.h b/pyrapose_amd/csrc/conv3.h
--- a/pyrapose_amd/csrc/conv3.h
+++ b/pyrapose_amd/csrc/conv3.h
@@ -8,6 +8,7 @@
   void *chi, *clo;
   const unsigned char* flags;
   float* ws;
+  int* tickets;
 };
 
 void PP_API(pp3_launch_igemm)(hipStream_t st, IgemmParams& p, const Igemm3Args& a, const PpIgemmPlan& pl);
diff --git a/pyrapose_amd/csrc/conv3.hip b/pyrapose_amd/csrc/conv3.hip
--- a/pyrapose_amd/csrc/conv3.hip
+++ b/pyrapose_amd/csrc/conv3.hip
@@ -5,8 +5,10 @@
 namespace {
 
 static PpIgemmFacts igemm3_facts(const pp_ctx* ctx, const IgemmParams& p, const Igemm3Args& a) {
-  return igemm_facts(p, a.w_rows, a.w_ld8, a.ahi != nullptr, p.src != nullptr, a.ohi != nullptr, p.out != nullptr, a.chi != nullptr,
-                     a.flags != nullptr, ctx->n_cu, ctx->ws != nullptr, (long long)ctx->ws_bytes);
+  PpIgemmFacts f = igemm_facts(p, a.w_rows, a.w_ld8, a.ahi != nullptr, p.src != nullptr, a.ohi != nullptr, p.out != nullptr, a.chi != nullptr,
+                               a.flags != nullptr, ctx->n_cu, ctx->ws != nullptr, (long long)ctx->ws_bytes);
+  f.tickets = (int)ctx->n_tickets;
+  return f;
 }
 
 static void dispatch3(pp_ctx* ctx, IgemmParams& p, const Igemm3Args& a) {
@@ -73,7 +75,7 @@
   p.relu = 0;
   PP_CHECK_ARG(ctx, (dx_hi == nullptr) == (dx_lo == nullptr) && (!dx_hi || (d->ld_x % 4 == 0 && pp_is_aligned16(dx_hi) && pp_is_aligned16(dx_lo))),
                PP_ERR_ARG, "%s: output planes", who);
-  const Igemm3Args a = {dy_hi, dy_lo, w_hi, w_lo, d->cin, cred / 8, dx_hi, dx_lo, chi, clo, skip_flags, ctx->ws};
+  const Igemm3Args a = {dy_hi, dy_lo, w_hi, w_lo, d->cin, cred / 8, dx_hi, dx_lo, chi, clo, skip_flags, ctx->ws, ctx->tickets};
   if (merged) {
     DgradS2Route s2;
     dgrad_s2_route(d, p, igemm3_facts(ctx, p, a), &s2);
@@ -92,7 +94,7 @@
                "does not apply to this call", who);
   const int nb = (p.M + 31) / 32;
   if (skip_scratch_ok && !route.listed) PP_HIP(ctx, hipMemsetAsync(skip_flags + nb, 1, (size_t)nb, ctx->stream));
-  const Igemm3Args ac = {dy_hi, dy_lo, w_hi, w_lo, d->cin, cred / 8, dx_hi, dx_lo, nullptr, nullptr, nullptr, ctx->ws};
+  const Igemm3Args ac = {dy_hi, dy_lo, w_hi, w_lo, d->cin, cred / 8, dx_hi, dx_lo, nullptr, nullptr, nullptr, ctx->ws, ctx->tickets};
   if (route.classes && chi) PP_API(pp3_split_capture_pass)(ctx->stream, p, chi, clo);
   dgrad_launches(
       route, p,
@@ -145,7 +147,7 @@
   p.relu = relu;
   PP_CHECK_ARG(ctx, (y_hi == nullptr) == (y_lo == nullptr) && (!y_hi || (d->ld_y % 4 == 0 && pp_is_aligned16(y_hi) && pp_is_aligned16(y_lo))),
                PP_ERR_ARG, "pp_conv2d_nhwc_fwd_bf16x3: output planes");
-  const Igemm3Args a = {x_hi, x_lo, w_hi, w_lo, d->cout, d->cin / 8, y_hi, y_lo, chi, clo, nullptr, ctx->ws};
+  const Igemm3Args a = {x_hi, x_lo, w_hi, w_lo, d->cout, d->cin / 8, y_hi, y_lo, chi, clo, nullptr, ctx->ws, ctx->tickets};
   if (opts->out_flags) {
     const bool ok = fwd_listed_ok(d, igemm3_facts(ctx, p, a), residual != nullptr || ep_ah != nullptr);
     PP_CHECK_ARG(ctx, ok, PP_ERR_SHAPE, "pp_conv2d_nhwc_fwd_bf16x3: out_flags needs a 3x3 stride-1 'same' conv on plane-stored input");
@@ -198,7 +200,7 @@
   p.kh = 7; p.kw = 1;
   p.mul = 2; p.tsign = 1; p.off_y = 0; p.off_x = 0; p.div = 1;
   p.w_ty0 = 0; p.w_tx0 = 0; p.w_tstep = 1; p.w_kw = 1; p.w_taps = 7;
-  const Igemm3Args a = {nullptr, nullptr, w_hi, w_lo, cout, 4, nullptr, nullptr, nullptr, nullptr, nullptr, ctx->ws};
+  const Igemm3Args a = {nullptr, nullptr, w_hi, w_lo, cout, 4, nullptr, nullptr, nullptr, nullptr, nullptr, ctx->ws, ctx->tickets};
   PP_CHECK_ARG(ctx, pp_igemm_fast_ok(igemm3_facts(ctx, p, a)), PP_ERR_SHAPE, "pp_stem7x7s2_fwd_bf16x3: frame too large for 31-bit offsets");
   dispatch3(ctx, p, a);
   PP_CHECK_LAUNCH(ctx, "pp_stem7x7s2_fwd_bf16x3");
diff --git a/pyrapose_amd/csrc/conv3_dispatch.hip b/pyrapose_amd/csrc/conv3_dispatch.hip
--- a/pyrapose_amd/csrc/conv3_dispatch.hip
+++ b/pyrapose_amd/csrc/conv3_dispatch.hip
@@ -87,6 +87,7 @@
   const bool planes_in = forms & PP_PLAN_PLANES_IN, planes_out = forms & PP_PLAN_PLANES_OUT, f32_out = (forms & PP_PLAN_F32_OUT) || !planes_out,
              capture = forms & PP_PLAN_CAPTURE, list = forms & PP_PLAN_LIST, lazy_in = forms & PP_PLAN_LAZY_IN;
   const bool ws = ws_bytes > 0;
+  const int tickets = (forms & PP_PLAN_TICKETS) ? (1 << 30) : 0;
   int at = 0;
   buf[0] = 0;
   if (pass == PP_PLAN_BWD_WEIGHT) {
@@ -103,6 +104,7 @@
     if (d->cin % 32 != 0) return PP_ERR_SHAPE;
     igemm_geometry_fwd(nullptr, d, p);
     PpIgemmFacts f = igemm_facts(p, d->cout, d->cin / 8, planes_in, !planes_in, planes_out, f32_out, capture, false, n_cu, ws, (long long)ws_bytes);
+    f.tickets = tickets;
     if (list) {
       if (!fwd_listed_ok(d, f, false)) return PP_ERR_SHAPE;
       f.listed = true;
@@ -131,6 +133,7 @@
                                       (long long)ws_bytes);
         fq.listed = listed;
         fq.listed_tm = route.listed_tm;
+        fq.tickets = tickets;
         at = pp_plan_print(buf, buf_bytes, at, fq, pp_plan_igemm(fq), true);
       },
       [&](IgemmParams& q) {
diff --git a/pyrapose_amd/csrc/conv3_igemm.hip b/pyrapose_amd/csrc/conv3_igemm.hip
--- a/pyrapose_amd/csrc/conv3_igemm.hip
+++ b/pyrapose_amd/csrc/conv3_igemm.hip
@@ -7,6 +7,42 @@
 #endif
 
 namespace {
+
+__device__ __forceinline__ void splitk_finish4(const IgemmParams& p, int splits, const float* ws, long long slice, int mr, int co,
+                                               const float* __restrict__ g_bias, const float* __restrict__ g_addend, const float* __restrict__ g_mask,
+                                               float* __restrict__ g_out, void* __restrict__ g_ohi, void* __restrict__ g_olo);
+
+__device__ __forceinline__ bool splitk_arrive(int* g_tickets, int tile, int splits, int tid, int* flag) {
+  asm volatile("s_waitcnt vmcnt(0)" ::: "memory");
+  __syncthreads();
+  if (tid == 0) {
+    __builtin_amdgcn_fence(__ATOMIC_RELEASE, "agent");
+    asm volatile("s_waitcnt vmcnt(0)" ::: "memory");
+    const bool last = __hip_atomic_fetch_add(g_tickets + tile, 1, __ATOMIC_RELAXED, __HIP_MEMORY_SCOPE_AGENT) == splits - 1;
+    if (last) {
+      __hip_atomic_store(g_tickets + tile, 0, __ATOMIC_RELAXED, __HIP_MEMORY_SCOPE_AGENT);
+      __builtin_amdgcn_fence(__ATOMIC_ACQUIRE, "agent");
+      asm volatile("s_waitcnt vmcnt(0)" ::: "memory");
+    }
+    *flag = last ? 1 : 0;
+  }
+  __syncthreads();
+  return *flag != 0;
+}
+
+template <int BM, int BN>
+__device__ __forceinline__ void splitk_finish_tile(const IgemmParams& p, int splits, const float* ws, int m0, int n0, int r_lo, int r_hi, int tid,
+                                                   const float* __restrict__ g_bias, const float* __restrict__ g_addend,
+                                                   const float* __restrict__ g_mask, float* __restrict__ g_out, void* __restrict__ g_ohi,
+                                                   void* __restrict__ g_olo) {
+  const int n_end = (p.Nout + 3) & ~3;
+  const long long slice = (long long)(p.M - p.m_off) * p.ld_out;
+  for (int i = tid; i < BM * (BN / 4); i += 256) {
+    const int r = i / (BN / 4), co = n0 + 4 * (i % (BN / 4));
+    const int m = m0 + r;
+    if (r >= r_lo && r <= r_hi && m < p.M && co < n_end) splitk_finish4(p, splits, ws, slice, m - p.m_off, co, g_bias, g_addend, g_mask, g_out, g_ohi, g_olo);
+  }
+}
 
 template <int TM, int TN, bool AP, bool OP>
 __global__ __launch_bounds__(256, (TM * TN >= 8) ? 2 : ((TM * TN == 4) ? 3 : 4)) void igemm3_kernel(
@@ -145,13 +181,14 @@
   epilogue3<TM, TN, OP>(p, acc, smem, m0, n0, tid, wm, wn, il, h, g_bias, g_addend, g_mask, g_out, g_ohi, g_olo);
 }
 
-template <int TM, int TN, bool AP, bool OP, bool SC, bool RL, bool MG>
+template <int TM, int TN, bool AP, bool OP, bool SC, bool RL, bool MG, bool FIN = false>
 __device__ __forceinline__ void igemm3f_body(
     const IgemmParams& p, const int bid, const int n_wg_in, const void* __restrict__ g_a0, const void* __restrict__ g_a1, unsigned a_bytes,
     const void* __restrict__ g_whi, const void* __restrict__ g_wlo, unsigned w_bytes,
     const float* __restrict__ g_bias, const float* __restrict__ g_addend, const float* __restrict__ g_mask,
     float* __restrict__ g_out, uint2* __restrict__ g_ohi, uint2* __restrict__ g_olo, int w_rows, int w_ld8, int splits,
-    float* __restrict__ g_ws, const int* __restrict__ g_rl, const unsigned char* __restrict__ g_srcflags) {
+    float* __restrict__ g_ws, const int* __restrict__ g_rl, const unsigned char* __restrict__ g_srcflags, int* g_tickets = nullptr) {
+  static_assert(!FIN || (!RL && !MG && !SC), "the in-launch finish is for the dense split launch");
   constexpr int BM = 64 * TM, BN = 64 * TN, BK = 32, NO = BK / 8;
   constexpr int SMEM_U4 = 2 * NO * (BM + BN);
   constexpr int ES = 4;
@@ -310,7 +347,7 @@
     store_step();
     __syncthreads();
   }
-  if (splits > 1) {
+  if (FIN || splits > 1) {
     float* slice = g_ws + (long long)split * (RL ? (((long long)p.M + 31) & ~31ll) : (long long)p.M) * p.ld_out;
 #pragma unroll
     for (int a = 0; a < TM; ++a)
@@ -325,6 +362,10 @@
           if (row_ok && co < ((p.Nout + 3) & ~3)) slice[(long long)m * p.ld_out + co] = acc[a][b][r];
         }
       }
+    if constexpr (FIN) {
+      if (splitk_arrive(g_tickets, lb, splits, tid, reinterpret_cast<int*>(smem)))
+        splitk_finish_tile<BM, BN>(p, splits, g_ws, m0, n0, 0, BM - 1, tid, g_bias, g_addend, g_mask, g_out, g_ohi, g_olo);
+    }
     return;
   }
   epilogue3<TM, TN, OP, PP_EPI_GF, SC, false, RL>(p, acc, smem, m0, n0, tid, wm, wn, il, h, g_bias, g_addend, g_mask, g_out, g_ohi, g_olo, rl_blk);
@@ -341,6 +382,18 @@
                                               g_mask, g_out, g_ohi, g_olo, w_rows, w_ld8, splits, g_ws, g_rl, g_srcflags);
 }
 
+template <int TM, int TN, bool AP>
+__global__ __launch_bounds__(256, (TM * TN >= 8) ? 2 : ((TM * TN == 4) ? 3 : 4)) void igemm3f_fin_kernel(
+    const IgemmParams p, const void* __restrict__ g_a0, const void* __restrict__ g_a1, unsigned a_bytes,
+    const void* __restrict__ g_whi, const void* __restrict__ g_wlo, unsigned w_bytes,
+    const float* __restrict__ g_bias, const float* __restrict__ g_addend, const float* __restrict__ g_mask,
+    float* __restrict__ g_out, uint2* __restrict__ g_ohi, uint2* __restrict__ g_olo, int w_rows, int w_ld8, int splits,
+    float* __restrict__ g_ws, int* g_tickets) {
+  igemm3f_body<TM, TN, AP, false, false, false, false, true>(p, (int)blockIdx.x, (int)gridDim.x, g_a0, g_a1, a_bytes, g_whi, g_wlo, w_bytes, g_bias,
+                                                             g_addend, g_mask, g_out, g_ohi, g_olo, w_rows, w_ld8, splits, g_ws, nullptr, nullptr,
+                                                             g_tickets);
+}
+
 template <int TM, int TN, bool AP, bool OP>
 __global__ __launch_bounds__(256, (TM * TN >= 8) ? 2 : ((TM * TN == 4) ? 3 : 4)) void igemm3m_kernel(
     const IgemmParams p0, const PpS2Merged g, const void* __restrict__ g_a0, const void* __restrict__ g_a1, unsigned a_bytes,
@@ -358,7 +411,7 @@
                                                   g_out, g_ohi, g_olo, w_rows, w_ld8, 1, nullptr, nullptr, nullptr);
 }
 
-template <int TM, int TN, bool CAP, bool AP = false, bool OP = false>
+template <int TM, int TN, bool CAP, bool AP = false, bool OP = false, bool FIN = false>
 __global__ __launch_bounds__(256, (TM * TN >= 8) ? 2 : ((TM * TN == 4) ? 3 : 4)) void igemm3x_kernel(
     const IgemmParams p, const void* __restrict__ g_a, const void* __restrict__ g_a1, unsigned a_bytes, const void* __restrict__ g_whi,
     const void* __restrict__ g_wlo, unsigned w_bytes, const float* __restrict__ g_bias, const float* __restrict__ g_addend,
@@ -366,6 +419,7 @@
     int splits, float* __restrict__ g_ws, void* __restrict__ g_chi, void* __restrict__ g_clo, const unsigned char* __restrict__ g_flags,
     int skip_halo) {
   static_assert(!(CAP && AP), "split capture is for f32 operands");
+  static_assert(!FIN || (!CAP && !OP), "the in-launch finish has no capture form and writes the planes itself");
   constexpr int ES = 4;
   constexpr int BM = 64 * TM, BN = 64 * TN, BK = 32, NO = BK / 8;
   constexpr int AP1 = NO * BM + 1;
@@ -585,7 +639,7 @@
     store_a();
     __syncthreads();
   }
-  if (splits > 1) {
+  if (FIN || splits > 1) {
     float* slice = g_ws + (long long)split * (p.M - p.m_off) * p.ld_out;
 #pragma unroll
     for (int a = 0; a < TM; ++a)
@@ -599,6 +653,10 @@
           if (row >= 1 && row <= BM - 2 && m < p.M && co < ((p.Nout + 3) & ~3)) slice[(long long)(m - p.m_off) * p.ld_out + co] = acc[a][b][r];
         }
       }
+    if constexpr (FIN) {
+      if (splitk_arrive(static_cast<int*>(g_chi), lb, splits, tid, reinterpret_cast<int*>(smem)))
+        splitk_finish_tile<BM, BN>(p, splits, g_ws, m0, n0, 1, BM - 2, tid, g_bias, g_addend, g_mask, g_out, g_ohi, g_olo);
+    }
     return;
   }
   epilogue3<TM, TN, OP, 4, false, true>(p, acc, smem, m0, n0, tid, wm, wn, il, h, g_bias, g_addend, g_mask, g_out, g_ohi, g_olo);
@@ -625,6 +683,20 @@
   if (g_ohi) planes_st4(g_ohi, g_olo, (mo * p.ld_out + co) >> 2, v);
 }
 
+__device__ __forceinline__ void splitk_finish4(const IgemmParams& p, int splits, const float* ws, long long slice, int mr, int co,
+                                               const float* __restrict__ g_bias, const float* __restrict__ g_addend, const float* __restrict__ g_mask,
+                                               float* __restrict__ g_out, void* __restrict__ g_ohi, void* __restrict__ g_olo) {
+  const int m = p.m_off + mr;
+  const float* w = ws + (long long)mr * p.ld_out + co;
+  float4 v = *reinterpret_cast<const float4*>(w);
+  for (int s = 1; s < splits; ++s) {
+    const float4 q = *reinterpret_cast<const float4*>(w + s * slice);
+    v.x += q.x; v.y += q.y; v.z += q.z; v.w += q.w;
+  }
+  if (g_bias) { const float4 b = *reinterpret_cast<const float4*>(g_bias + co); v.x += b.x; v.y += b.y; v.z += b.z; v.w += b.w; }
+  finish4(p, v, (long long)m, co, true, g_addend, g_mask, g_out, g_ohi, g_olo);
+}
+
 __global__ void class_fill_kernel(const IgemmParams p, const float* __restrict__ g_addend, const float* __restrict__ g_mask,
                                   float* __restrict__ g_out, void* __restrict__ g_ohi, void* __restrict__ g_olo) {
   const int n4 = (p.Nout + 3) >> 2;
@@ -646,15 +718,7 @@
   const long long total = (long long)rows * n4, slice = (long long)rows * p.ld_out;
   for (long long i = blockIdx.x * (long long)blockDim.x + threadIdx.x; i < total; i += (long long)gridDim.x * blockDim.x) {
     const int mr = (int)(i / n4), co = 4 * (int)(i - (long long)mr * n4);
-    const int m = p.m_off + mr;
-    const float* w = ws + (long long)mr * p.ld_out + co;
-    float4 v = *reinterpret_cast<const float4*>(w);
-    for (int s = 1; s < splits; ++s) {
-      const float4 q = *reinterpret_cast<const float4*>(w + s * slice);
-      v.x += q.x; v.y += q.y; v.z += q.z; v.w += q.w;
-    }
-    if (g_bias) { const float4 b = *reinterpret_cast<const float4*>(g_bias + co); v.x += b.x; v.y += b.y; v.z += b.z; v.w += b.w; }
-    finish4(p, v, (long long)m, co, true, g_addend, g_mask, g_out, g_ohi, g_olo);
+    splitk_finish4(p, splits, ws, slice, mr, co, g_bias, g_addend, g_mask, g_out, g_ohi, g_olo);
   }
 }
 
@@ -805,10 +869,19 @@
   if (pl.capture_first) PP_API(pp3_split_capture_pass)(st, p, a.chi, a.clo);
   auto go_x = [&](auto cap, auto ap, auto op, const IgemmParams& q, unsigned grid, int q_splits, float* q_ws, const unsigned char* flags) {
     constexpr bool CAP = decltype(cap)::value, AP = decltype(ap)::value, OP = decltype(op)::value;
-    if constexpr (AP || TM <= 2)
+    if constexpr (AP || TM <= 2) {
+      if constexpr (!CAP && !OP && TM <= 2) {
+        if (pl.finish_inline && q_splits > 1) {
+          hipLaunchKernelGGL((igemm3x_kernel<TM, TN, false, AP, false, true>), dim3(grid), wg, 0, st, q, AP ? a.ahi : (const void*)q.src,
+                             AP ? a.alo : nullptr, a_bytes, a.whi, a.wlo, w_bytes, q.bias, q.addend, q.mask_src, q.out, (uint2*)a.ohi, (uint2*)a.olo,
+                             a.w_rows, a.w_ld8, q_splits, q_ws, (void*)a.tickets, nullptr, flags, pl.skip_halo);
+          return;
+        }
+      }
       hipLaunchKernelGGL((igemm3x_kernel<TM, TN, CAP, AP, OP>), dim3(grid), wg, 0, st, q, AP ? a.ahi : (const void*)q.src, AP ? a.alo : nullptr, a_bytes,
                          a.whi, a.wlo, w_bytes, q.bias, q.addend, q.mask_src, q.out, OP ? (uint2*)a.ohi : no_hi, OP ? (uint2*)a.olo : no_lo, a.w_rows,
                          a.w_ld8, q_splits, q_ws, CAP ? a.chi : nullptr, CAP ? a.clo : nullptr, flags, pl.skip_halo);
+    }
   };
   switch (pl.family) {
     case PP_IGEMM3F_CLASS:
@@ -822,7 +895,7 @@
           IgemmParams q = p;
           q.m_off = pl.tail_m_off;
           go_x(no, yes, no, q, pl.tail_grid, pl.tail_splits, a.ws, nullptr);
-          launch_splitk_finish(st, q, pl.tail_splits, a.ws, pl.finish_blocks, a.ohi, a.olo);
+          if (pl.finish_blocks) launch_splitk_finish(st, q, pl.tail_splits, a.ws, pl.finish_blocks, a.ohi, a.olo);
         }
       }
       return;
@@ -842,7 +915,11 @@
       void *const ohi = splits > 1 ? nullptr : a.ohi, *const olo = splits > 1 ? nullptr : a.olo;
       auto go = [&](auto ap, auto op) {
         constexpr bool AP = decltype(ap)::value, OP = decltype(op)::value;
-        if (pl.family == PP_IGEMM3F)
+        if (pl.family == PP_IGEMM3F && pl.finish_inline && !OP)
+          hipLaunchKernelGGL((igemm3f_fin_kernel<TM, TN, AP>), dim3(pl.grid), wg, 0, st, p, AP ? a.ahi : (const void*)p.src, AP ? a.alo : nullptr, a_bytes,
+                             a.whi, a.wlo, w_bytes, p.bias, p.addend, p.mask_src, p.out, (uint2*)a.ohi, (uint2*)a.olo, a.w_rows, a.w_ld8, splits, ws,
+                             a.tickets);
+        else if (pl.family == PP_IGEMM3F)
           launch_igemm3f<TM, TN, AP, OP, false, false>(st, pl.grid, p, a, ohi, olo, splits, ws, nullptr, nullptr);
         else
           hipLaunchKernelGGL((igemm3_kernel<TM, TN, AP, OP>), dim3(pl.grid), wg, 0, st, p, p.src, (const uint4*)(AP ? a.ahi : nullptr),
diff --git a/pyrapose_amd/csrc/conv_plan.h b/pyrapose_amd/csrc/conv_plan.h
--- a/pyrapose_amd/csrc/conv_plan.h
+++ b/pyrapose_amd/csrc/conv_plan.h
@@ -51,6 +51,7 @@
 inline int pp_sw_dma_var() { return pp_env_int("PP_CONV3_DMA_VAR", 1); }
 inline bool pp_sw_dma2() { return pp_env_is1("PP_CONV3_DMA2"); }
 inline int pp_sw_dma2_min() { return pp_env_int("PP_CONV3_DMA2_MIN", 512); }
+inline bool pp_sw_splitk_inline() { return pp_env_not0("PP_CONV3_SPLITK_INLINE"); }
 inline bool pp_sw_conv4p() { return pp_env_is1("PP_CONV4P"); }
 inline int pp_sw_conv4p_nst() { const char* e = getenv("PP_CONV4P_NST"); return e && atoi(e) == 3 ? 3 : 4; }
 inline int pp_sw_conv4p_splits() { return pp_env_int("PP_CONV4P_SPLITS", 0); }
@@ -100,6 +101,7 @@
   int n_cu;
   bool ws;
   long long ws_bytes;
+  int tickets;
 };
 
 enum PpIgemmFamily {
@@ -122,6 +124,7 @@
   int stages;
   bool capture_first;
   unsigned finish_blocks;
+  bool finish_inline;
   long long ws_need;
   int n_steps;
   bool may_split;
@@ -201,6 +204,10 @@
   pl->grid = (unsigned)(((nb + BM / 32 - 1) / (BM / 32)) * pl->n_tiles_n * splits);
   pl->finish_blocks = splits > 1 ? (unsigned)nb : 0u;
   pl->ws_need = splits > 1 ? (long long)nb * 32 * f.ld_out * 4 * splits : 0;
+}
+
+inline bool pp_plan_finish_inline(const PpIgemmFacts& f, unsigned grid, int splits) {
+  return splits > 1 && pp_sw_splitk_inline() && (long long)(grid / (unsigned)splits) <= (long long)f.tickets;
 }
 
 inline PpIgemmPlan pp_plan_igemm(const PpIgemmFacts& f) {
@@ -297,7 +304,8 @@
           const int rem = f.M - full_rt * (BM4 - 2);
           pl.tail_m_off = full_rt * (BM4 - 2);
           pl.tail_grid = (unsigned)(((rem + BM - 3) / (BM - 2)) * ntn * tail_splits);
-          pl.finish_blocks = pp_finish_blocks(rem, f.Nout, n_cu);
+          pl.finish_inline = pp_plan_finish_inline(f, pl.tail_grid, tail_splits);
+          pl.finish_blocks = pl.finish_inline ? 0u : pp_finish_blocks(rem, f.Nout, n_cu);
           pl.ws_need = (long long)tail_splits * rem * f.ld_out * 4;
         }
         return pl;
@@ -310,10 +318,14 @@
       }
     }
     pl.family = f.planes_in ? (op ? PP_IGEMM3X_PP : PP_IGEMM3X_PF) : (op ? PP_IGEMM3X_FP : PP_IGEMM3X_FF);
+    pl.finish_inline = tm <= 2 && pp_plan_finish_inline(f, pl.grid, splits);
+    if (pl.finish_inline) pl.finish_blocks = 0;
     return pl;
   }
   pl.capture_first = f.capture;
   pl.family = fast ? PP_IGEMM3F : PP_IGEMM3;
+  pl.finish_inline = fast && pp_plan_finish_inline(f, pl.grid, splits);
+  if (pl.finish_inline) pl.finish_blocks = 0;
   return pl;
 }
 
@@ -556,6 +568,7 @@
                         "variant=%d stages=%d capture_first=%d finish_blocks=%u ws_need=%lld",
                         pl.grid, pl.n_tiles_n, pl.x_ty_inner, pl.skip_halo, pl.full_rt, pl.tail_splits, pl.tail_grid, pl.tail_m_off, pl.variant,
                         pl.stages, (int)pl.capture_first, pl.finish_blocks, pl.ws_need);
+  if (detail && pl.finish_inline) at = pp_plan_append(buf, cap, at, " finish_inline=1");
   return pp_plan_append(buf, cap, at, "\n");
 }
 inline int pp_plan_print(char* buf, int cap, int at, const PpWgradFacts& f, const PpWgradPlan& pl, bool detail) {
diff --git a/pyrapose_amd/csrc/ctx.hip b/pyrapose_amd/csrc/ctx.hip
--- a/pyrapose_amd/csrc/ctx.hip
+++ b/pyrapose_amd/csrc/ctx.hip
@@ -44,6 +44,32 @@
   return PP_OK;
 }
 
+extern "C" int pp_ctx_set_tickets(pp_ctx* ctx, int* zeroed, size_t count, int zero) {
+  PP_REQUIRE_CTX(ctx);
+  PP_CHECK_ARG(ctx, (zeroed == nullptr) == (count == 0) && pp_is_aligned16(zeroed) && count < (1u << 30), PP_ERR_ARG, "pp_ctx_set_tickets: bad buffer");
+  ctx->tickets = nullptr;
+  ctx->n_tickets = 0;
+  if (zeroed && zero) PP_HIP(ctx, hipMemsetAsync(zeroed, 0, count * sizeof(int), ctx->stream));
+  ctx->tickets = zeroed;
+  ctx->n_tickets = count;
+  return PP_OK;
+}
+
+extern "C" int pp_ctx_tickets_nonzero(pp_ctx* ctx, int* count) {
+  PP_REQUIRE_CTX(ctx);
+  PP_CHECK_ARG(ctx, count != nullptr, PP_ERR_ARG, "pp_ctx_tickets_nonzero: null count");
+  *count = 0;
+  if (!ctx->tickets) return PP_OK;
+  int* host = (int*)malloc(ctx->n_tickets * sizeof(int));
+  PP_CHECK_ARG(ctx, host != nullptr, PP_ERR_ARG, "pp_ctx_tickets_nonzero: out of memory");
+  hipError_t e = hipMemcpyAsync(host, ctx->tickets, ctx->n_tickets * sizeof(int), hipMemcpyDeviceToHost, ctx->stream);
+  if (e == hipSuccess) e = hipStreamSynchronize(ctx->stream);
+  for (size_t i = 0; e == hipSuccess && i < ctx->n_tickets; ++i) *count += host[i] != 0;
+  free(host);
+  if (e != hipSuccess) return pp_fail(ctx, (int)e, "pp_ctx_tickets_nonzero: %s", hipGetErrorString(e));
+  return PP_OK;
+}
+
 extern "C" int pp_ctx_set_planes_format(pp_ctx* ctx, int fmt) {
   PP_REQUIRE_CTX(ctx);
   PP_CHECK_ARG(ctx, fmt == 0 || fmt == 1, PP_ERR_ARG, "pp_ctx_set_planes_format: 0 (bf16 pairs) or 1 (P16)");
diff --git a/pyrapose_amd/csrc/pp_internal.h b/pyrapose_amd/csrc/pp_internal.h
--- a/pyrapose_amd/csrc/pp_internal.h
+++ b/pyrapose_amd/csrc/pp_internal.h
@@ -14,6 +14,8 @@
   char err[512];
   float* ws;
   size_t ws_bytes;
+  int* tickets;
+  size_t n_tickets;
   int planes_fmt;
   const float* grad_scale;
 };
diff --git a/pyrapose_amd/ops.py b/pyrapose_amd/ops.py
--- a/pyrapose_amd/ops.py
+++ b/pyrapose_amd/ops.py
@@ -13,6 +13,9 @@
         return None
     assert t.is_cuda, "pyrapose_amd ops need device tensors"
     return C.c_void_p(t.data_ptr())
+
+
+TICKETS_MIN = 16384
 
 
 class Context:
@@ -48,17 +51,31 @@
             t.workspace = ws
             if ws is not None:
                 check(lib.pp_ctx_set_workspace(t.handle, _ptr(ws), ws.numel() * 4), t.handle, "pp_ctx_set_workspace")
+            tk = getattr(self, "tickets", None)
+            t.tickets = tk
+            if tk is not None:
+                check(lib.pp_ctx_set_tickets(t.handle, _ptr(tk), tk.numel(), 0), t.handle, "pp_ctx_set_tickets")
             self._twin = t
         assert self._twin.planes_fmt == int(fmt)
         return self._twin
 
     def set_workspace(self, nbytes):
         self.workspace = torch.empty((int(nbytes) // 4,), dtype=torch.float32, device="cuda:%d" % self.device) if nbytes else None
+        self.tickets = (torch.empty((max(TICKETS_MIN, int(nbytes) // 16384),), dtype=torch.int32, device="cuda:%d" % self.device)
+                        if nbytes else None)
         for c in (self, self._twin):
             if c is not None:
                 c.workspace = self.workspace
                 check(lib.pp_ctx_set_workspace(c.handle, _ptr(self.workspace), (int(nbytes) // 4) * 4 if nbytes else 0), c.handle,
                       "pp_ctx_set_workspace")
+                c.tickets = self.tickets
+                check(lib.pp_ctx_set_tickets(c.handle, _ptr(self.tickets), self.tickets.numel() if nbytes else 0, int(c is self)), c.handle,
+                      "pp_ctx_set_tickets")
+
+    def tickets_nonzero(self):
+        n = C.c_int(0)
+        check(lib.pp_ctx_tickets_nonzero(self.handle, C.byref(n)), self.handle, "pp_ctx_tickets_nonzero")
+        return n.value
 
     def device_info(self):
         n = C.c_int(0)
@@ -87,6 +104,7 @@
 
 PLAN_FWD, PLAN_BWD_DATA, PLAN_BWD_WEIGHT, PLAN_BWD_DATA_S2 = 0, 1, 2, 3
 PLAN_PLANES_IN, PLAN_PLANES_OUT, PLAN_F32_OUT, PLAN_CAPTURE, PLAN_LIST, PLAN_LAZY_IN, PLAN_LAZY_OUT = 1, 2, 4, 8, 16, 32, 64
+PLAN_TICKETS = 128
 
 
 def conv_plan_text(d, pass_, forms=0, planes_fmt=1, n_cu=256, ws_bytes=0):
```

After: 580.0. 5.8% lower.
